# EryiXie/PlaneRecNet

Measured on AMD Instinct MI355X. Metric: img/s fwd+bwd @480×640 ResNet101-DCN, 1/2/4/8 MI355X + roofline %, higher is better.
Workload: dtype f32 (tensors and accumulation fp32; plain GEMMs and the tap-walked 4x4/s2, 1x1/s2 and sub-pixel convolutions >= 300 tiles: 2xfp16-piece split MFMA, fp32 accumulate; fp32-only rate in fp32_only_run)

## Files before the change

### include/prn.h

```cpp
#ifndef PRN_H
#define PRN_H
#include <stdint.h>
#ifdef __cplusplus
extern "C" {
#endif

#define PRN_BN_SPLITS 32

int prn_version(void);
const char* prn_last_error(void);

enum { PRN_IN_ZERO = 0, PRN_IN_REFLECT = 1, PRN_IN_UP2_REFLECT = 2, PRN_IN_DILATED = 3, PRN_IN_UP2_PHASE = 4,
       PRN_IN_EMBED1 = 5  };
enum { PRN_EPI_NONE = 0, PRN_EPI_RELU = 1, PRN_EPI_SIGMOID = 2 };

enum { PRN_SPLIT_OFF = 0, PRN_SPLIT_PLAN = 1, PRN_SPLIT_ALWAYS = 2 };
enum { PRN_PIECES_BF16 = 0, PRN_PIECES_F16 = 16 };
typedef struct prn_gemm_opts {
  int32_t split_mode;
  int32_t split_kind;
  int32_t split_products;
  int32_t split_min_tiles;
  float split_min_gflop;
  int32_t wgrad_wgs;
  int32_t wgrad_target;
  int32_t wgrad_split;
} prn_gemm_opts;
void prn_gemm_opts_default(prn_gemm_opts* o);

typedef struct prn_conv_desc {
  int32_t B, C, H, W;
  int32_t M;
  int32_t KH, KW;
  int32_t stride, pad;
  int32_t Ho, Wo;
  int32_t in_mode;
  int32_t dil;
  int32_t epilogue;
  int32_t ystride;
  int32_t yH, yW;
  int32_t reserved;
  prn_gemm_opts opts;
} prn_conv_desc;

int64_t prn_conv2d_fwd_ws_bytes(const prn_conv_desc* d);
int prn_conv2d_kernel_kind(const prn_conv_desc* d);
int prn_conv2d_fwd_partials(const prn_conv_desc* d, int64_t* offset_bytes);
int prn_gemm_pipe(int M, int K, int B, int HW, int nz, const prn_gemm_opts* opts);
int64_t prn_split_images_bytes(int M, int K, int nz);
int prn_split_prepare(const float* w, void* images, int M, int K, int nz, int kind, void* stream);
int prn_split_prepare_batched(const void* items_dev, int n_items, int64_t total_blocks, int64_t total_row_blocks, int kind, void* stream);
int prn_conv2d_fwd(const prn_conv_desc* d, const float* x, const float* w, const float* bias,
                   const float* addend, float* y, void* ws, void* stream);
#define PRN_TILE_COUNTERS 4096
int prn_conv2d_fwd_counted(const prn_conv_desc* d, const float* x, const float* w, const void* w_images, const float* bias, const float* addend, float* y,
                           void* ws, unsigned* counters, void* stream, int phase);
#define PRN_MAX_SEGMENTS 6
typedef struct prn_ragged {
  int32_t nseg;
  int32_t H[PRN_MAX_SEGMENTS], W[PRN_MAX_SEGMENTS];
} prn_ragged;
int prn_conv2d_fwd_ragged(const prn_conv_desc* d, const prn_ragged* rg, const float* x, const float* w, const float* bias,
                          const float* addend, float* y, void* stream);
int64_t prn_conv2d_wgrad_ragged_ws_bytes(const prn_conv_desc* d, const prn_ragged* rg);
int prn_conv2d_wgrad_ragged(const prn_conv_desc* d, const prn_ragged* rg, const float* x, const float* dy, float* dw, void* ws,
                            void* stream);

int prn_conv2d_fwd_phase(const prn_conv_desc* d, const float* x, const float* w, const float* bias,
                         const float* addend, float* y, void* ws, void* stream, int phase);

int prn_weight_flip_transpose(const float* w, float* wt, int M, int C, int KH, int KW, void* stream);

typedef struct prn_flip_item {
  const float* src;
  float* dst;
  int M, C, KH, KW;
  int64_t first;
} prn_flip_item;
int prn_weight_flip_transpose_batched(const prn_flip_item* items_dev, int n_items, int64_t total_blocks, void* stream);

int64_t prn_winograd_tiles(int B, int H, int W);
typedef struct prn_winograd_item {
  const float* src;
  float* u;
  float* ut;
  int M, C;
  int64_t first;
} prn_winograd_item;
int prn_winograd_weights_batched(const prn_winograd_item* items_dev, int n_items, int64_t total_blocks, void* stream);
int prn_winograd_input(const float* x, float* V, int B, int C, int H, int W, int in_mode, void* stream);
int64_t prn_gemm_batched_ws_bytes(int M, int C, int P, int nb, const prn_gemm_opts* opts);
int prn_gemm_batched(int M, int C, int P, int nb, const float* U, const void* u_images, const float* V, float* Y, void* ws, const prn_gemm_opts* opts,
                     void* stream);
int prn_winograd_output(const float* Y, const float* bias, const float* addend, float* y, int B, int M, int H, int W, int epilogue, void* stream);
int prn_winograd_output_bn_fwd(const float* Yt, float* x_out, float* stats, const float* gamma, const float* beta, float* y, float* running_mean,
                               float* running_var, int B, int M, int H, int W, float eps, float momentum, int relu, void* stream);
int prn_winograd_output_bn_bwd(const float* Yt, const float* x, const float* stats, const float* gamma, const float* beta, float* dx, float* dgamma,
                               float* dbeta, int B, int M, int H, int W, int relu, void* stream);
int64_t prn_winograd_wgrad_ws_bytes(int B, int C, int H, int W, int M, const prn_gemm_opts* opts);
int prn_winograd_dy(const float* dy, float* Y, int B, int M, int H, int W, void* stream);
int prn_gemm_batched_nt_splits(int M, int C, int P, int nb, const prn_gemm_opts* opts);
int prn_gemm_batched_nt_kind(int M, int C, int P, int nb, const prn_gemm_opts* opts);
int prn_gemm_batched_nt(int M, int C, int P, int nb, const float* A, const float* Bm, float* ws, const prn_gemm_opts* opts, void* stream);
int prn_winograd_dw(const float* partials, float* dw, int M, int C, int splits, void* stream);
int prn_conv3x3_winograd_wgrad(const float* x, const float* dy, float* dw, void* ws, int B, int C, int H, int W, int M, int in_mode, const prn_gemm_opts* opts,
                               void* stream, int phase);
int prn_conv3x3_winograd_wgrad_v(const float* V, const float* dy, float* dw, void* ws, int B, int C, int H, int W, int M, const prn_gemm_opts* opts, void* stream);
int64_t prn_winograd_tiles_ragged(const prn_ragged* rg, int B);
int64_t prn_conv3x3_winograd_ragged_ws_bytes(const prn_ragged* rg, int B, int C, int M, const prn_gemm_opts* opts);
int prn_conv3x3_winograd_ragged(const float* x, const float* U, const void* u_images, const float* bias, const float* addend, float* y, void* ws,
                                const prn_ragged* rg, int B, int C, int M, int epilogue, const prn_gemm_opts* opts, void* stream);
int64_t prn_winograd_wgrad_ragged_ws_bytes(const prn_ragged* rg, int B, int C, int M, const prn_gemm_opts* opts);
int prn_conv3x3_winograd_wgrad_ragged(const float* x, const float* dy, float* dw, void* ws, const prn_ragged* rg, int B, int C, int M, const prn_gemm_opts* opts,
                                      void* stream);
// ... 20 lines not shown

int prn_channel_sum(const float* x, float* out, double* ws, int B, int C, int HW, void* stream);

int prn_dcn_sample(const float* x, const float* om, float* cols, int B, int C, int H, int W, int Ho, int Wo,
                   int stride, float max_offset, void* stream);
int64_t prn_dcn_sample_bwd_ws_bytes(int B, int C, int H, int W, int Ho, int Wo);
int prn_dcn_sample_bwd(const float* x, const float* om, const float* dcols, float* dx, float* d_om, void* ws,
                       int B, int C, int H, int W, int Ho, int Wo, int stride, float max_offset, void* stream);

typedef struct prn_dcn_desc {
  int32_t B, C, H, W;
  int32_t M;
  int32_t stride, pad;
  int32_t Ho, Wo;
  int32_t raw;
  float max_offset;
  int32_t epilogue;
  prn_gemm_opts opts;
} prn_dcn_desc;
int64_t prn_dcnv2_table_bytes(const prn_dcn_desc* d);
int prn_dcnv2_table(const prn_dcn_desc* d, const float* offset, const float* mask, void* table, void* stream);
int64_t prn_dcnv2_fwd_ws_bytes(const prn_dcn_desc* d);
int prn_dcnv2_fwd(const prn_dcn_desc* d, const float* x, const void* table, const float* w, const float* bias, float* y, void* ws, void* stream);
int prn_dcnv2_fwd_phase(const prn_dcn_desc* d, const float* x, const void* table, const float* w, const float* bias, float* y, void* ws, void* stream,
                        int phase);
int64_t prn_dcnv2_bwd_weight_ws_bytes(const prn_dcn_desc* d);
int prn_dcnv2_bwd_weight(const prn_dcn_desc* d, const float* x, const void* table, const float* dy, float* dw, void* ws, void* stream);
int prn_dcnv2_bwd_weight_phase(const prn_dcn_desc* d, const float* x, const void* table, const float* dy, float* dw, void* ws, void* stream, int phase);
int64_t prn_dcnv2_bwd_ws_bytes(const prn_dcn_desc* d);
int prn_dcnv2_bwd_input(const prn_dcn_desc* d, const float* dy, const float* wt, const void* wt_images, const float* offset, const float* mask, float* dx,
                        void* ws, void* stream);
int prn_dcnv2_bwd_input_phase(const prn_dcn_desc* d, const float* dy, const float* wt, const void* wt_images, const float* offset, const float* mask,
                              float* dx, void* ws, void* stream, int phase);
int prn_dcnv2_bwd_offset_mask(const prn_dcn_desc* d, const float* x, const float* offset, const float* mask, float* d_offset, float* d_mask,
                              void* ws, void* stream);

int prn_bn_stats(const float* x, float* stats, float* running_mean, float* running_var, double* ws,
                 int B, int C, int HW, float eps, float momentum, void* stream);
int prn_bn_apply(const float* x, const float* stats, const float* gamma, const float* beta, const float* residual,
                 float* y, int B, int C, int HW, int relu, void* stream);
int prn_bn_kernel_kind(int B, int HW);
int prn_bn_train_fwd(const float* x, float* stats, const float* gamma, const float* beta, const float* residual, float* y,
                     float* running_mean, float* running_var, double* ws, int B, int C, int HW, float eps, float momentum,
                     int relu, void* stream);
int prn_bn_bwd(const float* dy, const float* x, const float* y, const float* stats, const float* gamma, const float* beta,
               float* dx, float* dres, float* dgamma, float* dbeta, double* ws,
               int B, int C, int HW, int relu, int frozen, void* stream);
int prn_bn_train_fwd_into(const float* x, float* stats, const float* gamma, const float* beta, const float* residual, float* y,
                          int64_t y_batch_stride, float* running_mean, float* running_var, double* ws, int B, int C, int HW, float eps,
                          float momentum, int relu, void* stream);
int prn_bn_bwd_from(const float* dy, int64_t dy_batch_stride, const float* x, const float* y, const float* stats, const float* gamma,
                    const float* beta, float* dx, float* dres, float* dgamma, float* dbeta, double* ws,
                    int B, int C, int HW, int relu, int frozen, void* stream);

int prn_bn_train_fwd_partials(const float* parts, int nparts, int64_t part_stride, float* x_out, float* stats, const float* gamma, const float* beta,
                              const float* residual, float* y, float* running_mean, float* running_var, int B, int C, int HW, float eps, float momentum,
                              int relu, void* stream);
int prn_bn_bwd_partials(const float* dparts, int nparts, int64_t part_stride, const float* x, const float* y, const float* stats, const float* gamma,
                        const float* beta, float* dx, float* dres, float* dgamma, float* dbeta, int B, int C, int HW, int relu, int frozen, void* stream);
int prn_bn_train_fwd_winograd(const float* parts, int nparts, int64_t part_stride, float* x_out, float* stats, const float* gamma, const float* beta,
                              const float* residual, float* y, float* running_mean, float* running_var, float* V, int B, int C, int H, int W, float eps,
                              float momentum, int relu, void* stream);
int prn_bn_bwd_winograd(const float* dparts, int nparts, int64_t part_stride, const float* x, const float* y, const float* stats, const float* gamma,
                        const float* beta, float* dx, float* dres, float* dgamma, float* dbeta, float* V, int B, int C, int H, int W, int relu, int frozen,
                        void* stream);

int prn_gn_relu_fwd(const float* x, const float* gamma, const float* beta, float* y, float* stats ,
                    int B, int C, int HW, int G, float eps, void* stream);
int prn_gn_relu_bwd(const float* dy, const float* x, const float* beta, const float* stats, const float* gamma,
                    float* dx, float* dgamma_part , float* dbeta_part ,
                    int B, int C, int HW, int G, void* stream);
int prn_gn_relu_fwd_ragged(const float* x, const float* gamma, const float* beta, float* y, float* stats,
                           int B, int C, int nseg, const int* hw, int G, float eps, void* stream);
int prn_gn_relu_bwd_ragged(const float* dy, const float* x, const float* beta, const float* stats, const float* gamma,
                           float* dx, float* dgamma_part, float* dbeta_part, int B, int C, int nseg, const int* hw, int G,
                           void* stream);

int prn_sum_rows(const float* in, float* out, int nb, int R, int N, void* stream);

int prn_debug_skip_launches(int mask);

int prn_resize_bilinear_fwd(const float* x, float* y, int BC, int H, int W, int Ho, int Wo, void* stream);
int prn_resize_bilinear_bwd(const float* dy, float* dx, int BC, int H, int W, int Ho, int Wo, void* stream);
int prn_resize_bilinear_add_fwd(const float* x, const float* addend, float* y, int BC, int H, int W, int Ho, int Wo, void* stream);
int prn_resize_bilinear_bwd_add(const float* dy, const float* addend, float* dx, int BC, int H, int W, int Ho, int Wo, void* stream);
int prn_maxpool3s2_fwd(const float* x, float* y, unsigned char* arg, int BC, int H, int W, int Ho, int Wo, void* stream);
int prn_maxpool3s2_bwd(const unsigned char* arg, const float* dy, float* dx, int BC, int H, int W, int Ho, int Wo, void* stream);

int64_t prn_plane_prior_ws_bytes(int B, int E, int h, int w, int NK, int F, const prn_gemm_opts* opts);
int prn_plane_prior_fwd(const float* seg, const float* kernels, const float* w1, const float* b1, float* pooled, float* out, void* ws, int B, int E,
                        int h, int w, int NK, int F, const prn_gemm_opts* opts, void* stream);
int prn_plane_prior_fwd_phase(const float* seg, const float* kernels, const float* w1, const float* b1, float* pooled, float* out, void* ws, int B, int E,
                        int h, int w, int NK, int F, const prn_gemm_opts* opts, void* stream, int phase);
int64_t prn_plane_prior_wgrad_ws_bytes(int B, int h, int w, int NK, int F, const prn_gemm_opts* opts);
int prn_plane_prior_wgrad(const float* pooled, const float* d_out, float* dw1, void* ws, int B, int h, int w, int NK, int F, const prn_gemm_opts* opts,
                          void* stream);
int64_t prn_fpn_level_ws_bytes(int B, int C, int H, int W, int F, int relu, int has_prev, int have_u, const prn_gemm_opts* opts);
int prn_fpn_level_fwd(const float* x, const float* w_lat, const float* b_lat, const float* prev, int Hp, int Wp, const float* w_out, const float* u_out,
                      const float* b_out, float* lateral, float* p_out, void* ws, int B, int C, int H, int W, int F, int relu, const prn_gemm_opts* opts,
                      void* stream);

enum { PRN_BLK_WINOGRAD = 1,
       PRN_BLK_HANDOVER = 2,
       PRN_BLK_KEEP_V = 4,
       PRN_BLK_SCATTER_ACC = 8 };
enum { PRN_BLK_CONV2_DIRECT = 0, PRN_BLK_CONV2_WINOGRAD = 1, PRN_BLK_CONV2_DCN = 2 };
typedef struct prn_bottleneck_desc {
  int32_t B, C, H, W;
  int32_t planes;
  int32_t stride;
  int32_t dcn;
  int32_t downsample;
  int32_t flags;
  float eps[4], momentum[4];
  float max_offset;
  int32_t reserved;
  prn_gemm_opts opts;
} prn_bottleneck_desc;
typedef struct prn_bottleneck_params {
  const float *w1, *w2, *w3, *wd;
  const float *b2;
  const void *w1_img, *w3_img, *wd_img;
  const float* u2; const void* u2_img;
  const float *w1_t, *w2_t, *w3_t, *wd_t;
  const void *w1_t_img, *w3_t_img, *wd_t_img;
  const float* ut2; const void* ut2_img;
  const float *w27, *b27, *w27_t;
  const float* w2_cols_t; const void* w2_cols_t_img;
  const float *gamma[4], *beta[4];
  float *running_mean[4], *running_var[4];
} prn_bottleneck_params;
enum { PRN_BLK_SAVE_BYTES = 0, PRN_BLK_GSAVE_BYTES, PRN_BLK_FWD_WS_BYTES, PRN_BLK_BWD_WS_BYTES, PRN_BLK_HO, PRN_BLK_WO, PRN_BLK_CONV2_PATH, PRN_BLK_KEEPS_V,
       PRN_BLK_OFF_A1, PRN_BLK_OFF_V, PRN_BLK_OFF_A2, PRN_BLK_OFF_OM, PRN_BLK_OFF_TABLE,
       PRN_BLK_OFF_D1, PRN_BLK_OFF_D2, PRN_BLK_OFF_D3, PRN_BLK_OFF_DD, PRN_BLK_OFF_DOM,
       PRN_BLK_BN_GRAD_FLOATS,
       PRN_BLK_HANDOVERS,
       PRN_BLK_NEEDS_W1_IMG, PRN_BLK_NEEDS_W3_IMG, PRN_BLK_NEEDS_WD_IMG, PRN_BLK_NEEDS_W1T_IMG, PRN_BLK_NEEDS_W3T_IMG, PRN_BLK_NEEDS_WDT_IMG, PRN_BLK_NEEDS_U_IMG,
       PRN_BLK_NEEDS_COLT_IMG, PRN_BLK_INFO_COUNT };
int64_t prn_bottleneck_plan_bytes(void);
int64_t prn_bottleneck_params_bytes(void);
int prn_bottleneck_plan(const prn_bottleneck_desc* d, void* plan);
int prn_bottleneck_plan_info(const void* plan, int64_t* out, int n);
int prn_bottleneck_train_fwd(const void* plan, const prn_bottleneck_params* p, const float* x, float* y, void* save, void* ws, void* stream);
int prn_bottleneck_train_bwd(const void* plan, const prn_bottleneck_params* p, const float* x, const float* y, const float* dy, float* dx, int dx_accumulate,
                             const void* save, void* gsave, float* bn_grads, void* ws, void* stream);

int prn_frame_to_input(const unsigned char* src, int Hs, int Ws, int Hr, int Wr, int Hp, int Wp, const float* mean_bgr, const float* std_bgr, int mode,
                       float* dst, float* frame_bgr, void* stream);

int prn_mask_loss_ws_floats(int P);
int prn_mask_loss_fwd(const float* logits, const unsigned char* labels, const float* adj, const int64_t* img, const float* gsum, const float* npos,
                      float* out2, float* coef, float* ws, int P, int HW, int B, float w_ins, float w_lav, void* stream);
int prn_mask_loss_bwd(const float* logits, const unsigned char* labels, const float* adj, const int64_t* img, const float* coef, const float* g_ins,
                      const float* g_lav, float* dlogits, int P, int HW, void* stream);

int prn_lava_gt_weights(const float* gt, float* out, int B, int H, int W, float depth_resolution, void* stream);

int prn_vnl_triplets(const float* pred, const float* gt, const int* gid, const int64_t* seg, const unsigned char* seg_is_plane, const double* seg_normal,
                     const int64_t* seg_img, const double* fx, const double* fy, double* loss, unsigned char* valid, float* g3, int n, int H, int W,
                     float delta_z, void* stream);
int prn_vnl_scatter(const double* g_loss, const float* g3, const int64_t* order, const int64_t* start, float* d_depth, int npts, int n, void* stream);

int prn_loss_ws_doubles(int B);
int prn_focal_sum_fwd(const float* x, const int64_t* labels, float* out, double* ws, int64_t rows, int C, float alpha, float gamma, void* stream);
int prn_focal_sum_bwd(const float* x, const int64_t* labels, const float* g_out, float* dx, int64_t rows, int C, float alpha, float gamma, void* stream);
int prn_rmse_log_fwd(const float* pred, const float* gt, float* out, float* coef, double* ws, int B, int HW, float min_depth, float clamp, void* stream);
int prn_rmse_log_bwd(const float* pred, const float* gt, const float* coef, const float* g_out, float* dpred, int B, int HW, float min_depth, float clamp,
                     void* stream);

int prn_vnl_trim_key(const double* loss, const unsigned char* valid, const int64_t* seg, double* key, int n, void* stream);
int prn_vnl_trim_fwd(const double* loss, const unsigned char* valid, const int64_t* order, const int64_t* seg_start, const unsigned char* seg_is_plane,
                     const int64_t* seg_img, const double* nplanes, int nseg, int n, int B, double* out, double* seg_sum, int* seg_m, double* seg_coef,
                     void* ws, void* stream);
int64_t prn_vnl_trim_ws_bytes(int nseg);
int prn_vnl_trim_bwd(const double* loss, const int64_t* order, const int64_t* seg_start, const int* seg_m, const double* seg_coef, const int64_t* seg_img,
                     const double* g_out, int nseg, int n, double* dloss, void* stream);

int prn_depth_metrics_ws_doubles(void);
int prn_depth_metrics(const float* pred, const float* gt, double* out, double* ws, int64_t n, float min_depth, float max_depth, void* stream);

int64_t prn_pairwise_iou_ws_bytes(int A, int B, int64_t HW);
int prn_pairwise_iou(const unsigned char* masks_a, const unsigned char* masks_b, const float* boxes_a, const float* boxes_b, int A, int B, int64_t HW,
                     float* mask_iou, float* box_iou, void* ws, void* stream);
int prn_mask_boxes(const unsigned char* masks, int n, int H, int W, float* boxes, void* stream);
int prn_mask_stats(const float* seg, int n, int64_t HW, float thr, float* count, float* msum, void* stream);
int prn_sigmoid_point_nms(const float* x, float* out, int B, int C, int S, int64_t out_batch_stride, void* stream);
int prn_matrix_nms(const float* iou, const int64_t* labels, const float* scores, int n, float sigma, int gaussian, float* out, float* ws, void* stream);
#define PRN_MASK_NMS_MAX 4096
int64_t prn_mask_nms_ws_bytes(int n_total, int n_max, int64_t HW);
int prn_mask_nms(const unsigned char* masks, const int64_t* labels, const float* sum_masks, const int* seg, int n_img, int n_max, int64_t HW, float thr,
                 unsigned char* keep, void* ws, void* stream);
// ... 71 lines not shown
```

### planerecnet_amd/_lib.py

```python
import ctypes
import os

_HERE = os.path.dirname(os.path.abspath(__file__))
LIB_PATH = os.environ.get("PRN_LIB") or os.path.join(_HERE, "libprn_hip.so")

c_int, c_float, c_void_p, c_i64 = ctypes.c_int, ctypes.c_float, ctypes.c_void_p, ctypes.c_int64


class GemmOpts(ctypes.Structure):
    _fields_ = [("split_mode", ctypes.c_int32), ("split_kind", ctypes.c_int32), ("split_products", ctypes.c_int32), ("split_min_tiles", ctypes.c_int32),
                ("split_min_gflop", ctypes.c_float), ("wgrad_wgs", ctypes.c_int32), ("wgrad_target", ctypes.c_int32), ("wgrad_split", ctypes.c_int32)]

    def key(self):
        return (self.split_mode, self.split_kind, self.split_products, self.split_min_tiles, self.split_min_gflop, self.wgrad_wgs, self.wgrad_target, self.wgrad_split)


SPLIT_OFF, SPLIT_PLAN, SPLIT_ALWAYS = 0, 1, 2
PIECES_BF16, PIECES_F16 = 0, 16


class ConvDesc(ctypes.Structure):
    _fields_ = [(n, ctypes.c_int32) for n in
                ("B", "C", "H", "W", "M", "KH", "KW", "stride", "pad", "Ho", "Wo", "in_mode", "dil", "epilogue", "ystride", "yH", "yW", "reserved")] + [
                    ("opts", GemmOpts)]


class Ragged(ctypes.Structure):
    _fields_ = [("nseg", ctypes.c_int32), ("H", ctypes.c_int32 * 6), ("W", ctypes.c_int32 * 6)]


class DcnDesc(ctypes.Structure):
    _fields_ = [(n, ctypes.c_int32) for n in ("B", "C", "H", "W", "M", "stride", "pad", "Ho", "Wo", "raw")] + [("max_offset", ctypes.c_float),
                                                                                                              ("epilogue", ctypes.c_int32),
                                                                                                              ("opts", GemmOpts)]


class BottleneckDesc(ctypes.Structure):
    _fields_ = [(n, ctypes.c_int32) for n in ("B", "C", "H", "W", "planes", "stride", "dcn", "downsample", "flags")] + [
        ("eps", ctypes.c_float * 4), ("momentum", ctypes.c_float * 4), ("max_offset", ctypes.c_float), ("reserved", ctypes.c_int32), ("opts", GemmOpts)]


class BottleneckParams(ctypes.Structure):
    _fields_ = [(n, ctypes.c_void_p) for n in (
        "w1", "w2", "w3", "wd", "b2", "w1_img", "w3_img", "wd_img", "u2", "u2_img", "w1_t", "w2_t", "w3_t", "wd_t", "w1_t_img", "w3_t_img", "wd_t_img", "ut2", "ut2_img",
        "w27", "b27", "w27_t", "w2_cols_t", "w2_cols_t_img")] + [(n, ctypes.c_void_p * 4) for n in ("gamma", "beta", "running_mean", "running_var")]


IN_ZERO, IN_REFLECT, IN_UP2_REFLECT, IN_DILATED, IN_UP2_PHASE, IN_EMBED1 = 0, 1, 2, 3, 4, 5
EPI_NONE, EPI_RELU, EPI_SIGMOID = 0, 1, 2
BN_SPLITS = 32

P = c_void_p
_DP = ctypes.POINTER(ConvDesc)
_OP = ctypes.POINTER(GemmOpts)
SIGNATURES = {
    "prn_version": (c_int, []),
    "prn_last_error": (ctypes.c_char_p, []),
    "prn_conv2d_fwd_ws_bytes": (c_i64, [_DP]),
    "prn_conv2d_kernel_kind": (c_int, [_DP]),
    "prn_conv2d_fwd_partials": (c_int, [_DP, ctypes.POINTER(c_i64)]),
    "prn_gemm_opts_default": (None, [_OP]),
    "prn_gemm_pipe": (c_int, [c_int, c_int, c_int, c_int, c_int, _OP]),
    "prn_split_images_bytes": (c_i64, [c_int, c_int, c_int]),
    "prn_split_prepare": (c_int, [P, P, c_int, c_int, c_int, c_int, P]),
    "prn_split_prepare_batched": (c_int, [P, c_int, c_i64, c_i64, c_int, P]),
    "prn_conv2d_fwd": (c_int, [_DP, P, P, P, P, P, P, P]),
    "prn_conv2d_fwd_ragged": (c_int, [_DP, P, P, P, P, P, P, P]),
    "prn_conv2d_wgrad_ragged_ws_bytes": (c_i64, [_DP, P]),
    "prn_conv2d_wgrad_ragged": (c_int, [_DP, P, P, P, P, P, P]),
    "prn_gn_relu_fwd_ragged": (c_int, [P, P, P, P, P, c_int, c_int, c_int, P, c_int, c_float, P]),
    "prn_gn_relu_bwd_ragged": (c_int, [P, P, P, P, P, P, P, P, c_int, c_int, c_int, P, c_int, P]),
    "prn_conv2d_fwd_phase": (c_int, [_DP, P, P, P, P, P, P, P, c_int]),
    "prn_conv2d_fwd_counted": (c_int, [_DP, P, P, P, P, P, P, P, P, P, c_int]),
    "prn_conv2d_wgrad_phase": (c_int, [_DP, P, P, P, P, P, c_int]),
    "prn_weight_flip_transpose": (c_int, [P, P, c_int, c_int, c_int, c_int, P]),
    "prn_weight_flip_transpose_batched": (c_int, [P, c_int, c_i64, P]),
    "prn_winograd_tiles": (c_i64, [c_int, c_int, c_int]),
    "prn_winograd_weights_batched": (c_int, [P, c_int, c_i64, P]),
    "prn_winograd_input": (c_int, [P, P, c_int, c_int, c_int, c_int, c_int, P]),
    "prn_gemm_batched_ws_bytes": (c_i64, [c_int, c_int, c_int, c_int, _OP]),
    "prn_gemm_batched": (c_int, [c_int, c_int, c_int, c_int, P, P, P, P, P, _OP, P]),
    "prn_winograd_output": (c_int, [P, P, P, P, c_int, c_int, c_int, c_int, c_int, P]),
    "prn_winograd_output_bn_fwd": (c_int, [P] * 8 + [c_int] * 4 + [c_float, c_float, c_int, P]),
    "prn_winograd_output_bn_bwd": (c_int, [P] * 8 + [c_int] * 5 + [P]),
    "prn_winograd_wgrad_ws_bytes": (c_i64, [c_int] * 5 + [_OP]),
    "prn_winograd_dy": (c_int, [P, P, c_int, c_int, c_int, c_int, P]),
    "prn_gemm_batched_nt_splits": (c_int, [c_int] * 4 + [_OP]),
    "prn_gemm_batched_nt_kind": (c_int, [c_int] * 4 + [_OP]),
    "prn_conv2d_wgrad_kernel_kind": (c_int, [_DP, c_int]),
    "prn_gemm_batched_nt": (c_int, [c_int, c_int, c_int, c_int, P, P, P, _OP, P]),
    "prn_winograd_dw": (c_int, [P, P, c_int, c_int, c_int, P]),
    "prn_conv3x3_winograd_wgrad": (c_int, [P, P, P, P, c_int, c_int, c_int, c_int, c_int, c_int, _OP, P, c_int]),
    "prn_winograd_tiles_ragged": (c_i64, [P, c_int]),
    "prn_conv3x3_winograd_ragged_ws_bytes": (c_i64, [P, c_int, c_int, c_int, _OP]),
    "prn_conv3x3_winograd_ragged": (c_int, [P, P, P, P, P, P, P, P, c_int, c_int, c_int, c_int, _OP, P]),
    "prn_winograd_wgrad_ragged_ws_bytes": (c_i64, [P, c_int, c_int, c_int, _OP]),
    "prn_conv3x3_winograd_wgrad_ragged": (c_int, [P, P, P, P, P, c_int, c_int, c_int, _OP, P]),
    "prn_conv3x3_winograd_wgrad_v": (c_int, [P, P, P, P, c_int, c_int, c_int, c_int, c_int, _OP, P]),
    "prn_conv3x3_winograd_ws_bytes": (c_i64, [c_int] * 5 + [_OP]),
    "prn_conv3x3_winograd": (c_int, [P, P, P, P, P, P, P, c_int, c_int, c_int, c_int, c_int, c_int, c_int, _OP, P]),
    "prn_conv2d_wgrad_ws_bytes": (c_i64, [_DP]),
    "prn_conv2d_wgrad_grouped_ws_bytes": (c_i64, [_DP, c_int]),
    "prn_conv2d_wgrad_grouped": (c_int, [_DP, c_int, P, P, P, P, P]),
    "prn_conv2d_wgrad": (c_int, [_DP, P, P, P, P, P]),
    "prn_pad_fold": (c_int, [P, P, c_int, c_int, c_int, c_int, c_int, P]),
    "prn_pad_fold_pitched": (c_int, [P, P, c_int, c_int, c_int, c_int, c_int, P]),
    "prn_up2_phase_weights": (c_int, [P, P, c_int, c_int, P]),
    "prn_up2_dgrad_weights": (c_int, [P, P, c_int, c_int, P]),
    "prn_up2_wgrad_combine": (c_int, [P, P, c_int, c_int, P]),
    "prn_space_to_depth2": (c_int, [P, P, c_int, c_int, c_int, c_int, P]),
    "prn_replicate_fold": (c_int, [P, P, c_int, c_int, c_int, c_int, P]),
    "prn_channel_sum": (c_int, [P, P, P, c_int, c_int, c_int, P]),
    "prn_dcn_sample": (c_int, [P, P, P] + [c_int] * 7 + [c_float, P]),
    "prn_dcn_sample_bwd_ws_bytes": (c_i64, [c_int] * 6),
    "prn_dcn_sample_bwd": (c_int, [P, P, P, P, P, P] + [c_int] * 7 + [c_float, P]),
    "prn_dcnv2_table_bytes": (c_i64, [P]),
    "prn_dcnv2_table": (c_int, [P, P, P, P, P]),
    "prn_dcnv2_fwd_ws_bytes": (c_i64, [P]),
    "prn_dcnv2_fwd": (c_int, [P] * 8),
    "prn_dcnv2_fwd_phase": (c_int, [P] * 8 + [c_int]),
    "prn_dcnv2_bwd_weight_ws_bytes": (c_i64, [P]),
    "prn_dcnv2_bwd_weight": (c_int, [P] * 7),
    "prn_dcnv2_bwd_weight_phase": (c_int, [P] * 7 + [c_int]),
    "prn_dcnv2_bwd_ws_bytes": (c_i64, [P]),
    "prn_dcnv2_bwd_input": (c_int, [P] * 9),
    "prn_dcnv2_bwd_input_phase": (c_int, [P] * 9 + [c_int]),
    "prn_bn_kernel_kind": (c_int, [c_int, c_int]),
    "prn_dcnv2_bwd_offset_mask": (c_int, [P] * 8),
    "prn_plane_prior_ws_bytes": (c_i64, [c_int] * 6 + [_OP]),
    "prn_plane_prior_fwd": (c_int, [P] * 7 + [c_int] * 6 + [_OP, P]),
    "prn_plane_prior_fwd_phase": (c_int, [P] * 7 + [c_int] * 6 + [_OP, P, c_int]),
    "prn_plane_prior_wgrad_ws_bytes": (c_i64, [c_int] * 5 + [_OP]),
    "prn_plane_prior_wgrad": (c_int, [P] * 4 + [c_int] * 5 + [_OP, P]),
    "prn_fpn_level_ws_bytes": (c_i64, [c_int] * 8 + [_OP]),
    "prn_fpn_level_fwd": (c_int, [P, P, P, P, c_int, c_int, P, P, P, P, P, P] + [c_int] * 6 + [_OP, P]),
    "prn_frame_to_input": (c_int, [P] + [c_int] * 6 + [P, P, c_int, P, P, P]),
    "prn_mask_loss_ws_floats": (c_int, [c_int]),
    "prn_mask_loss_fwd": (c_int, [P] * 9 + [c_int, c_int, c_int, c_float, c_float, P]),
    "prn_mask_loss_bwd": (c_int, [P] * 8 + [c_int, c_int, P]),
    "prn_vnl_triplets": (c_int, [P] * 12 + [c_int, c_int, c_int, c_float, P]),
    "prn_vnl_scatter": (c_int, [P] * 5 + [c_int, c_int, P]),
    "prn_depth_metrics_ws_doubles": (c_int, []),
    "prn_depth_metrics": (c_int, [P, P, P, P, c_i64, c_float, c_float, P]),
    "prn_vnl_trim_key": (c_int, [P, P, P, P, c_int, P]),
    "prn_vnl_trim_fwd": (c_int, [P, P, P, P, P, P, P, c_int, c_int, c_int, P, P, P, P, P, P]),
    "prn_vnl_trim_ws_bytes": (c_i64, [c_int]),
    "prn_vnl_trim_bwd": (c_int, [P, P, P, P, P, P, P, c_int, c_int, P, P]),
    "prn_loss_ws_doubles": (c_int, [c_int]),
    "prn_focal_sum_fwd": (c_int, [P, P, P, P, c_i64, c_int, c_float, c_float, P]),
    "prn_focal_sum_bwd": (c_int, [P, P, P, P, c_i64, c_int, c_float, c_float, P]),
    "prn_rmse_log_fwd": (c_int, [P, P, P, P, P, c_int, c_int, c_float, c_float, P]),
    "prn_rmse_log_bwd": (c_int, [P, P, P, P, P, c_int, c_int, c_float, c_float, P]),
    "prn_gt_segments": (c_i64, [c_int, c_int]),
    "prn_gt_mask_stats": (c_int, [P, P, c_int, c_int, c_int, c_int, P, P, P, P]),
    "prn_gt_quarter_masks": (c_int, [P, P, c_int, c_int, c_int, P]),
    "prn_gt_sample_triplets": (c_int, [P, P, c_int, c_int, c_int, c_int, P, P, P, P, P, ctypes.c_uint64, ctypes.c_uint64, c_i64, P, P]),
    "prn_adam_chunk_elems": (c_int, []),
    "prn_adam_step": (c_int, [P, c_int, c_int, P, P, P, P, P, P, P, P, P, ctypes.c_double, ctypes.c_double, c_float, P]),
    "prn_adam_step_masked": (c_int, [P, c_int, c_int, P, P, P, P, P, P, P, P, P, ctypes.c_double, ctypes.c_double, c_float, P, P, P]),
    "prn_pairwise_iou_ws_bytes": (c_i64, [c_int, c_int, c_i64]),
    "prn_pairwise_iou": (c_int, [P, P, P, P, c_int, c_int, c_i64, P, P, P, P]),
    "prn_mask_boxes": (c_int, [P, c_int, c_int, c_int, P, P]),
    "prn_mask_stats": (c_int, [P, c_int, c_i64, c_float, P, P, P]),
    "prn_sigmoid_point_nms": (c_int, [P, P, c_int, c_int, c_int, c_i64, P]),
    "prn_matrix_nms": (c_int, [P, P, P, c_int, c_float, c_int, P, P, P]),
    "prn_mask_nms_ws_bytes": (c_i64, [c_int, c_int, c_i64]),
    "prn_mask_nms": (c_int, [P, P, P, P, c_int, c_int, c_i64, c_float, P, P, P]),
    "prn_bn_stats": (c_int, [P, P, P, P, P, c_int, c_int, c_int, c_float, c_float, P]),
    "prn_bn_apply": (c_int, [P, P, P, P, P, P, c_int, c_int, c_int, c_int, P]),
    "prn_bn_train_fwd": (c_int, [P] * 9 + [c_int, c_int, c_int, c_float, c_float, c_int, P]),
    "prn_bn_bwd": (c_int, [P] * 11 + [c_int] * 5 + [P]),
    "prn_bn_train_fwd_into": (c_int, [P] * 6 + [c_i64] + [P] * 3 + [c_int, c_int, c_int, c_float, c_float, c_int, P]),
    "prn_bn_bwd_from": (c_int, [P, c_i64] + [P] * 10 + [c_int] * 5 + [P]),
    "prn_bn_train_fwd_partials": (c_int, [P, c_int, c_i64] + [P] * 8 + [c_int, c_int, c_int, c_float, c_float, c_int, P]),
    "prn_bn_bwd_partials": (c_int, [P, c_int, c_i64] + [P] * 9 + [c_int] * 5 + [P]),
    "prn_bn_train_fwd_winograd": (c_int, [P, c_int, c_i64] + [P] * 9 + [c_int] * 4 + [c_float, c_float, c_int, P]),
    "prn_bn_bwd_winograd": (c_int, [P, c_int, c_i64] + [P] * 10 + [c_int] * 6 + [P]),
    "prn_gn_relu_fwd": (c_int, [P, P, P, P, P, c_int, c_int, c_int, c_int, c_float, P]),
    "prn_gn_relu_bwd": (c_int, [P] * 8 + [c_int] * 4 + [P]),
    "prn_resize_bilinear_fwd": (c_int, [P, P] + [c_int] * 5 + [P]),
    "prn_resize_bilinear_bwd": (c_int, [P, P] + [c_int] * 5 + [P]),
    "prn_resize_bilinear_add_fwd": (c_int, [P, P, P] + [c_int] * 5 + [P]),
    "prn_resize_bilinear_bwd_add": (c_int, [P, P, P] + [c_int] * 5 + [P]),
    "prn_maxpool3s2_fwd": (c_int, [P, P, P] + [c_int] * 5 + [P]),
    "prn_maxpool3s2_bwd": (c_int, [P, P, P] + [c_int] * 5 + [P]),
    "prn_sum_rows": (c_int, [P, P, c_int, c_int, c_int, P]),
    "prn_lava_gt_weights": (c_int, [P, P, c_int, c_int, c_int, c_float, P]),
    "prn_debug_skip_launches": (c_int, [c_int]),
    "prn_bottleneck_plan_bytes": (c_i64, []),
    "prn_bottleneck_params_bytes": (c_i64, []),
    "prn_bottleneck_plan": (c_int, [ctypes.POINTER(BottleneckDesc), P]),
    "prn_bottleneck_plan_info": (c_int, [P, ctypes.POINTER(c_i64), c_int]),
    "prn_bottleneck_train_fwd": (c_int, [P, ctypes.POINTER(BottleneckParams), P, P, P, P, P]),
    "prn_bottleneck_train_bwd": (c_int, [P, ctypes.POINTER(BottleneckParams), P, P, P, P, c_int, P, P, P, P, P]),
    "prn_planes_ws_bytes": (c_i64, [c_int] * 4),
    "prn_planes_fit": (c_int, [P] * 4 + [c_int] * 4 + [P] * 6),
    "prn_planes_render": (c_int, [P] * 6 + [c_int] * 5 + [c_float, c_float, P, P, P]),
    "prn_planes_ransac_ws_bytes": (c_i64, [c_int] * 5),
    "prn_planes_ransac_fit": (c_int, [P] * 4 + [c_int] * 4 + [ctypes.c_double, c_int, c_int, c_int, ctypes.c_uint64] + [P] * 9),
    "prn_render_overlay": (c_int, [P] * 4 + [c_int] * 3 + [c_float, c_float, c_int, P, P]),
    "prn_render_limits_ws_bytes": (c_i64, []),
    "prn_render_depth_limits": (c_int, [P, c_i64, ctypes.c_double, ctypes.c_double, P, P, P]),
    "prn_render_depth_colors": (c_int, [P, c_i64, P, P, P, P]),
    "prn_render_depth_gray": (c_int, [P, c_i64, c_float, P, P]),
    "prn_rle_ws_bytes": (c_i64, [c_int] * 3),
    "prn_rle_count": (c_int, [P, P] + [c_int] * 4 + [P, P, P]),
    "prn_rle_fill": (c_int, [P, P] + [c_int] * 4 + [P, P, P, P]),
    "prn_rle_string_lengths": (c_int, [P, P] + [c_int] * 3 + [P, P]),
    "prn_rle_strings": (c_int, [P, P, P] + [c_int] * 3 + [P, P]),
    "prn_rle_paint": (c_int, [P, P] + [c_int] * 3 + [P, P]),
    "prn_ccl_ws_bytes": (c_i64, [c_int] * 3),
    "prn_ccl_label": (c_int, [P, P] + [c_int] * 5 + [P, P, P, P]),
    "prn_ccl_clean": (c_int, [P, P] + [c_int] * 8 + [P] * 7),
    "prn_morph_ws_bytes": (c_i64, [c_int] * 4),
    "prn_morph": (c_int, [P, P] + [c_int] * 7 + [P] * 4),
    "prn_boundary_iou_ws_bytes": (c_i64, [c_int] * 4),
    "prn_boundary_iou": (c_int, [P, P] + [c_int] * 5 + [P] * 4),
}


def load():
    if not os.path.exists(LIB_PATH):
        raise ImportError(f"{LIB_PATH} is missing: run `python -c 'import __graft_entry__ as g; g.build()'` "
                          "(hipcc --offload-arch=gfx950). There is no fallback path.")
# ... 17 lines not shown
```

### planerecnet_amd/blocks.py

```python
import ctypes
import os
import sys

import torch

from . import _lib, ops, profiling
from ._lib import lib, check

ENABLED = os.environ.get("PRN_BLOCKS", "1") == "1"
HANDOVER = os.environ.get("PRN_BLOCK_HANDOVER", "1") == "1"
SCATTER_ACCUMULATE = os.environ.get("PRN_SCATTER_ACC", "1") == "1"
STATS = {"fwd": 0, "bwd": 0, "resolved": 0, "vouched": 0, "scatter_acc": 0}

BLK_WINOGRAD, BLK_HANDOVER, BLK_KEEP_V, BLK_SCATTER_ACC = 1, 2, 4, 8
CONV2_DIRECT, CONV2_WINOGRAD, CONV2_DCN = 0, 1, 2
(I_SAVE, I_GSAVE, I_FWD_WS, I_BWD_WS, I_HO, I_WO, I_CONV2, I_KEEPS_V, I_A1, I_V, I_A2, I_OM, I_TABLE, I_D1, I_D2, I_D3, I_DD, I_DOM, I_BN_FLOATS, I_HANDOVERS,
 I_W1_IMG, I_W3_IMG, I_WD_IMG, I_W1T_IMG, I_W3T_IMG, I_WDT_IMG, I_U_IMG, I_COLT_IMG, INFO_COUNT) = range(29)

_SCRATCH = {}
_F32 = torch.float32
_empty = torch.empty


def scratch(nbytes, dev):
    key = (dev.index, ops._raw_stream(dev.index))
    t = _SCRATCH.get(key)
    if t is None or t.numel() * 4 < nbytes:
        t = _SCRATCH[key] = torch.empty((int(nbytes * 1.25) + 1023) // 4, device=dev, dtype=torch.float32)
    return t


class _Ref:
    __slots__ = ("ptr", "shape", "device")

    def __init__(self, ptr, shape, device):
        self.ptr, self.shape, self.device = ptr, shape, device

    def data_ptr(self):
        return self.ptr

    def numel(self):
        n = 1
        for s in self.shape:
            n *= s
        return n


class _State:
    __slots__ = ("plan", "plan_ref", "info", "params", "params_ref", "convw", "wver", "epoch", "batched", "keep", "hb", "bn_sizes", "out_shape", "Ho", "Wo", "conv2",
                 "dims", "wino_wgrad", "g_keys", "max_offset", "ps", "bns", "stat_bufs", "save_n", "gsave_n", "bn_n", "fwd_ws", "bwd_ws", "stride", "dcn", "ds",
                 "shapes")


def _flags():
    f = BLK_SCATTER_ACC if SCATTER_ACCUMULATE else 0
    if ops.WINOGRAD:
        f |= BLK_WINOGRAD
    if ops.WINOGRAD and ops.WINOGRAD_WGRAD:
        f |= BLK_KEEP_V
    if HANDOVER:
        f |= BLK_HANDOVER
    return f


def supported(blk):
    from .dcn import DeformableConv2d
    c2 = blk.conv2
    if blk.downsample is not None:
        dc = blk.downsample[0]
        if dc.kernel_size != (1, 1) or dc.stride[0] != blk.stride or dc.bias is not None:
            return False
    elif blk.stride != 1 or blk.conv1.weight.shape[1] != blk.conv3.weight.shape[0]:
        return False
    if isinstance(c2, DeformableConv2d):
        if c2.stride != blk.stride:
            return False
    elif c2.bias is not None or c2.kernel_size != (3, 3) or c2.padding != (1, 1) or c2.stride[0] != blk.stride:
        return False
    bns = [blk.bn1, blk.bn2, blk.bn3] + ([blk.downsample[1]] if blk.downsample is not None else [])
    return (blk.stride in (1, 2) and ops.WINOGRAD_MIN_TILES == 128 and blk.conv1.bias is None and blk.conv3.bias is None and blk.conv1.kernel_size == (1, 1)
            and blk.conv3.kernel_size == (1, 1) and all(isinstance(m, torch.nn.BatchNorm2d) and m.affine and m.track_running_stats and m.momentum is not None for m in bns))


def _param_list(blk):
    from .dcn import DeformableConv2d
    c2 = blk.conv2
    ps = [blk.conv1.weight, blk.bn1.weight, blk.bn1.bias]
    if isinstance(c2, DeformableConv2d):
        ps += [c2.offset_conv.weight, c2.modulator_conv.weight, c2.offset_conv.bias, c2.modulator_conv.bias, c2.regular_conv.weight, c2.regular_conv.bias]
    else:
        ps += [c2.weight]
    ps += [blk.bn2.weight, blk.bn2.bias, blk.conv3.weight, blk.bn3.weight, blk.bn3.bias]
    if blk.downsample is not None:
        ps += [blk.downsample[0].weight, blk.downsample[1].weight, blk.downsample[1].bias]
    return tuple(ps)


def _state(blk, x, key):
    from .dcn import DeformableConv2d
    oe = ops._opts_entry()
    B, C, H, W = x.shape
    dcn = isinstance(blk.conv2, DeformableConv2d)
    bns = (blk.bn1, blk.bn2, blk.bn3) + ((blk.downsample[1],) if blk.downsample is not None else ())
    eps = [float(m.eps) for m in bns] + [0.0] * (4 - len(bns))
    mom = [float(m.momentum) for m in bns] + [0.0] * (4 - len(bns))
    P = blk.conv1.weight.shape[0]
    d = _lib.BottleneckDesc(B, C, H, W, P, blk.stride, int(dcn), int(blk.downsample is not None), key[2], (ctypes.c_float * 4)(*eps), (ctypes.c_float * 4)(*mom),
                            max(H, W) / 4.0 if dcn else 0.0, 0, oe[0])
    st = _State()
    st.plan = ctypes.create_string_buffer(int(lib.prn_bottleneck_plan_bytes()) + 64)
    st.plan_ref = (ctypes.addressof(st.plan) + 63) & ~63
    check(lib.prn_bottleneck_plan(ctypes.byref(d), st.plan_ref), "prn_bottleneck_plan")
    info = (ctypes.c_int64 * INFO_COUNT)()
    check(lib.prn_bottleneck_plan_info(st.plan_ref, info, INFO_COUNT), "prn_bottleneck_plan_info")
# ... 276 lines not shown
```

### planerecnet_amd/csrc/prn_bottleneck.hip

```cpp
#include "prn_common.h"
#include <string.h>

namespace {

constexpr int32_t PLAN_MAGIC = 0x424c4b36;
constexpr int64_t WINOGRAD_MIN_TILES = 128;

inline int64_t up256(int64_t v) { return (v + 255) & ~255LL; }

struct Plan {
  int32_t magic, pad_;
  prn_bottleneck_desc d;
  int32_t Ho, Wo, P4, conv2_path;
  int32_t small1, small2;
  int32_t lazy1, parts1;
  int32_t v1, lazy2, keep_v;
  int32_t lazy3g, parts3g;
  int32_t v2g, lazy2g;
  int32_t pad2_;
  int64_t parts1_off, parts3g_off;
  prn_conv_desc c1, c2, c3, cd, c27, g1, g2, g3, gd, g27;
  prn_dcn_desc dcn;
  int64_t s_c1, s_a1, s_v, s_c2, s_a2, s_c3, s_cd, s_om, s_table, s_stats[4], save_bytes;
  int64_t q_d3, q_dd, q_d2, q_d1, q_dom, q_bn, gsave_bytes;
  int64_t f_c1, f_bn, f_v, f_yt, f_gemm, f_c2, f_c27, f_dcn, f_c3, f_cd, f_res, fwd_ws_bytes;
  int64_t b_bn, b_dres, b_g3, b_g3ws, b_v, b_yt, b_gemm, b_g2, b_g2ws, b_dcn, b_dx1, b_g27ws, b_g1ws, b_gdtmp, b_gdws, bwd_ws_bytes;
};

prn_conv_desc conv_desc(int B, int C, int H, int W, int M, int K, int stride, int pad, int Ho, int Wo, int mode, int dil, int ystride, int yH, int yW,
                        const prn_gemm_opts& o) {
  prn_conv_desc d;
  d.B = B; d.C = C; d.H = H; d.W = W; d.M = M; d.KH = d.KW = K; d.stride = stride; d.pad = pad; d.Ho = Ho; d.Wo = Wo;
  d.in_mode = mode; d.dil = dil; d.epilogue = PRN_EPI_NONE; d.ystride = ystride; d.yH = yH; d.yW = yW; d.reserved = 0;
  d.opts = o;
  return d;
}

bool winograd_ok(const prn_bottleneck_desc& d, int B, int C, int H, int W, int M) {
  return (d.flags & PRN_BLK_WINOGRAD) && (W % 4) == 0 && H >= 8 && C >= 64 && M >= 64 && (int64_t)B * ((H + 3) / 4) * (W / 4) >= WINOGRAD_MIN_TILES;
}

int make_plan(const prn_bottleneck_desc* dp, Plan& L) {
  PRN_REQUIRE(dp != nullptr, "prn_bottleneck_plan: null descriptor");
  const prn_bottleneck_desc& d = *dp;
  PRN_REQUIRE(d.B > 0 && d.C > 0 && d.H > 0 && d.W > 0 && d.planes > 0, "prn_bottleneck_plan: empty dimension");
  PRN_REQUIRE(d.stride == 1 || d.stride == 2, "prn_bottleneck_plan: stride %d (1 or 2)", d.stride);
  PRN_REQUIRE(d.downsample || (d.stride == 1 && d.C == 4 * d.planes), "prn_bottleneck_plan: without a downsample branch the block must keep its shape (C = 4 * planes, stride 1)");
  PRN_REQUIRE(!d.dcn || d.max_offset > 0.f, "prn_bottleneck_plan: the deformable variant needs max_offset (max(h, w) / 4)");
  memset(&L, 0, sizeof(L));
  L.magic = PLAN_MAGIC;
  L.d = d;
  const int B = d.B, C = d.C, H = d.H, W = d.W, P = d.planes, s = d.stride, Q = 4 * d.planes;
  const int Ho = (H + 2 - 3) / s + 1, Wo = (W + 2 - 3) / s + 1;
  L.Ho = Ho; L.Wo = Wo;
  const prn_gemm_opts& o = d.opts;
  const bool ho = (d.flags & PRN_BLK_HANDOVER) != 0;
  L.small1 = prn_bn_kernel_kind(B, H * W);
  L.small2 = prn_bn_kernel_kind(B, Ho * Wo);
  L.c1 = conv_desc(B, C, H, W, P, 1, 1, 0, H, W, PRN_IN_ZERO, 1, 0, 0, 0, o);
  L.c3 = conv_desc(B, P, Ho, Wo, Q, 1, 1, 0, Ho, Wo, PRN_IN_ZERO, 1, 0, 0, 0, o);
  if (d.downsample) L.cd = conv_desc(B, C, H, W, Q, 1, s, 0, Ho, Wo, PRN_IN_ZERO, 1, 0, 0, 0, o);
  const bool wino = !d.dcn && s == 1 && winograd_ok(d, B, P, H, W, P);
  L.conv2_path = d.dcn ? PRN_BLK_CONV2_DCN : (wino ? PRN_BLK_CONV2_WINOGRAD : PRN_BLK_CONV2_DIRECT);
  if (d.dcn) {
    L.c27 = conv_desc(B, P, H, W, 27, 3, s, 1, Ho, Wo, PRN_IN_ZERO, 1, 0, 0, 0, o);
    prn_dcn_desc& q = L.dcn;
    q.B = B; q.C = P; q.H = H; q.W = W; q.M = P; q.stride = s; q.pad = 1; q.Ho = Ho; q.Wo = Wo; q.raw = 1; q.max_offset = d.max_offset; q.epilogue = PRN_EPI_NONE;
    q.opts = o;
  } else if (!wino) {
    L.c2 = conv_desc(B, P, H, W, P, 3, s, 1, Ho, Wo, PRN_IN_ZERO, 1, 0, 0, 0, o);
  }
  if (wino) L.P4 = (int)prn_winograd_tiles(B, H, W);
  L.g3 = conv_desc(B, Q, Ho, Wo, P, 1, 1, 0, Ho, Wo, PRN_IN_ZERO, 1, 0, 0, 0, o);
  L.g1 = conv_desc(B, P, H, W, C, 1, 1, 0, H, W, PRN_IN_ZERO, 1, 0, 0, 0, o);
  if (!d.dcn && !wino)
    L.g2 = s == 1 ? conv_desc(B, P, Ho, Wo, P, 3, 1, 1, H, W, PRN_IN_ZERO, 1, 0, 0, 0, o) : conv_desc(B, P, Ho, Wo, P, 3, 1, 1, H, W, PRN_IN_DILATED, 2, 0, 0, 0, o);
  if (d.dcn)
    L.g27 = s == 1 ? conv_desc(B, 27, Ho, Wo, P, 3, 1, 1, H, W, PRN_IN_ZERO, 1, 0, 0, 0, o) : conv_desc(B, 27, Ho, Wo, P, 3, 1, 1, H, W, PRN_IN_DILATED, 2, 0, 0, 0, o);
  if (d.downsample)
    L.gd = s == 1 ? conv_desc(B, Q, Ho, Wo, C, 1, 1, 0, H, W, PRN_IN_ZERO, 1, 0, 0, 0, o) : conv_desc(B, Q, Ho, Wo, C, 1, 1, 0, Ho, Wo, PRN_IN_ZERO, 1, 2, H, W, o);
  int64_t off = 0;
  const int p1 = prn_conv2d_fwd_partials(&L.c1, &off);
  if (p1 < 0) return 2;
  L.lazy1 = ho && L.small1 && p1 > 1 && (((int64_t)B * P * H * W) & 3) == 0;
  L.parts1 = L.lazy1 ? p1 : 0; L.parts1_off = L.lazy1 ? off : 0;
  L.v1 = ho && wino && L.small1;
  L.lazy2 = ho && wino && L.small2 && L.P4 <= 768;
  L.keep_v = wino && (d.flags & PRN_BLK_KEEP_V) && 4LL * 36 * P * L.P4 <= (128LL << 20);
  const int p3 = prn_conv2d_fwd_partials(&L.g3, &off);
  if (p3 < 0) return 2;
  L.lazy3g = ho && L.small2 && p3 > 1 && (((int64_t)B * P * Ho * Wo) & 3) == 0;
  L.parts3g = L.lazy3g ? p3 : 0; L.parts3g_off = L.lazy3g ? off : 0;
  L.v2g = ho && wino && L.small2;
  L.lazy2g = ho && wino && L.small1 && L.P4 <= 768;
  const int64_t n1 = (int64_t)B * P * H * W * 4, n2 = (int64_t)B * P * Ho * Wo * 4, n3 = (int64_t)B * Q * Ho * Wo * 4, nx = (int64_t)B * C * H * W * 4;
  const int64_t nv = wino ? 4LL * 36 * P * L.P4 : 0, nom = (int64_t)B * 27 * Ho * Wo * 4;
  const int Cmax = Q > C ? Q : C;
  const int64_t bnws = 2LL * Cmax * PRN_BN_SPLITS * 8;
#define PRN_WS(expr_, name_) const int64_t name_ = (expr_); if (name_ < 0) return 2
  PRN_WS(prn_conv2d_fwd_ws_bytes(&L.c1), w_c1);
  PRN_WS(prn_conv2d_fwd_ws_bytes(&L.c3), w_c3);
  PRN_WS(d.downsample ? prn_conv2d_fwd_ws_bytes(&L.cd) : 0, w_cd);
  PRN_WS(L.conv2_path == PRN_BLK_CONV2_DIRECT ? prn_conv2d_fwd_ws_bytes(&L.c2) : 0, w_c2);
  PRN_WS(d.dcn ? prn_conv2d_fwd_ws_bytes(&L.c27) : 0, w_c27);
  PRN_WS(d.dcn ? prn_dcnv2_fwd_ws_bytes(&L.dcn) : 0, w_dcnf);
  PRN_WS(d.dcn ? prn_dcnv2_table_bytes(&L.dcn) : 0, n_table);
  PRN_WS(d.dcn ? prn_dcnv2_bwd_ws_bytes(&L.dcn) : 0, w_dcnb);
  PRN_WS(wino ? prn_gemm_batched_ws_bytes(P, P, L.P4, 36, &o) : 0, w_gemm);
  PRN_WS(prn_conv2d_fwd_ws_bytes(&L.g3), w_g3);
  PRN_WS(prn_conv2d_fwd_ws_bytes(&L.g1), w_g1);
  PRN_WS(L.conv2_path == PRN_BLK_CONV2_DIRECT ? prn_conv2d_fwd_ws_bytes(&L.g2) : 0, w_g2);
  PRN_WS(d.dcn ? prn_conv2d_fwd_ws_bytes(&L.g27) : 0, w_g27);
  PRN_WS(d.downsample ? prn_conv2d_fwd_ws_bytes(&L.gd) : 0, w_gd);
#undef PRN_WS
  int64_t at = 0;
  auto put = [&at](int64_t& slot, int64_t bytes) { slot = at; at += up256(bytes); };
  put(L.s_c1, n1); put(L.s_a1, n1);
  put(L.s_v, L.keep_v ? nv : 0);
  put(L.s_c2, n2); put(L.s_a2, n2); put(L.s_c3, n3);
  put(L.s_cd, d.downsample ? n3 : 0);
  put(L.s_om, d.dcn ? nom : 0); put(L.s_table, n_table);
  put(L.s_stats[0], 8LL * P); put(L.s_stats[1], 8LL * P); put(L.s_stats[2], 8LL * Q); put(L.s_stats[3], d.downsample ? 8LL * Q : 0);
  L.save_bytes = at;
  at = 0;
  put(L.q_d3, n3); put(L.q_dd, d.downsample ? n3 : 0); put(L.q_d2, n2); put(L.q_d1, n1); put(L.q_dom, d.dcn ? nom : 0);
  L.q_bn = 2 * P + 2 * P + 2 * Q + (d.downsample ? 2 * Q : 0);
  L.gsave_bytes = at;
  at = 0;
  put(L.f_c1, w_c1); put(L.f_bn, bnws);
  put(L.f_v, (wino && !L.keep_v) ? nv : 0); put(L.f_yt, nv); put(L.f_gemm, w_gemm);
  put(L.f_c2, w_c2); put(L.f_c27, w_c27); put(L.f_dcn, w_dcnf); put(L.f_c3, w_c3); put(L.f_cd, w_cd);
  put(L.f_res, d.downsample ? n3 : 0);
  L.fwd_ws_bytes = at;
  at = 0;
  put(L.b_bn, bnws); put(L.b_dres, n3);
  put(L.b_g3, n2); put(L.b_g3ws, w_g3);
  put(L.b_v, nv); put(L.b_yt, nv); put(L.b_gemm, w_gemm);
  put(L.b_g2, n1); put(L.b_g2ws, w_g2);
  put(L.b_dcn, w_dcnb); put(L.b_dx1, d.dcn ? n1 : 0); put(L.b_g27ws, w_g27);
  put(L.b_g1ws, w_g1);
  put(L.b_gdtmp, d.downsample ? nx : 0); put(L.b_gdws, w_gd);
  L.bwd_ws_bytes = at;
  return 0;
}

const Plan* plan_of(const void* plan, const char* who) {
  const Plan* L = (const Plan*)plan;
  if (L == nullptr || L->magic != PLAN_MAGIC) { prn_set_error("%s: not a plan filled by prn_bottleneck_plan", who); return nullptr; }
  return L;
}

inline float* f32(void* base, int64_t off) { return (float*)((char*)base + off); }
inline void* raw(void* base, int64_t off, int64_t used = 1) { return used ? (void*)((char*)base + off) : nullptr; }

#define PRN_TRY(call_) do { if (int e_ = (call_)) return e_; } while (0)

}

extern "C" int64_t prn_bottleneck_plan_bytes(void) { return (int64_t)sizeof(Plan); }
extern "C" int64_t prn_bottleneck_params_bytes(void) { return (int64_t)sizeof(prn_bottleneck_params); }

extern "C" int prn_bottleneck_plan(const prn_bottleneck_desc* d, void* plan) {
  PRN_REQUIRE(plan != nullptr, "prn_bottleneck_plan: null plan buffer (prn_bottleneck_plan_bytes() bytes, caller-owned)");
  Plan L;
  if (int e = make_plan(d, L)) { memset(plan, 0, sizeof(int32_t)); return e; }
  memcpy(plan, &L, sizeof(L));
  return 0;
}

extern "C" int prn_bottleneck_plan_info(const void* plan, int64_t* out, int n) {
  const Plan* L = plan_of(plan, "prn_bottleneck_plan_info");
  if (!L) return 2;
  PRN_REQUIRE(out != nullptr && n >= PRN_BLK_INFO_COUNT, "prn_bottleneck_plan_info: out must hold PRN_BLK_INFO_COUNT (%d) values", PRN_BLK_INFO_COUNT);
  out[PRN_BLK_SAVE_BYTES] = L->save_bytes; out[PRN_BLK_GSAVE_BYTES] = L->gsave_bytes;
  out[PRN_BLK_FWD_WS_BYTES] = L->fwd_ws_bytes; out[PRN_BLK_BWD_WS_BYTES] = L->bwd_ws_bytes;
  out[PRN_BLK_HO] = L->Ho; out[PRN_BLK_WO] = L->Wo; out[PRN_BLK_CONV2_PATH] = L->conv2_path; out[PRN_BLK_KEEPS_V] = L->keep_v;
  out[PRN_BLK_OFF_A1] = L->s_a1; out[PRN_BLK_OFF_V] = L->s_v; out[PRN_BLK_OFF_A2] = L->s_a2; out[PRN_BLK_OFF_OM] = L->s_om; out[PRN_BLK_OFF_TABLE] = L->s_table;
  out[PRN_BLK_OFF_D1] = L->q_d1; out[PRN_BLK_OFF_D2] = L->q_d2; out[PRN_BLK_OFF_D3] = L->q_d3; out[PRN_BLK_OFF_DD] = L->q_dd; out[PRN_BLK_OFF_DOM] = L->q_dom;
  out[PRN_BLK_BN_GRAD_FLOATS] = L->q_bn;
  out[PRN_BLK_HANDOVERS] = L->lazy1 | (L->v1 << 1) | (L->lazy2 << 2) | (L->lazy3g << 3) | (L->v2g << 4) | (L->lazy2g << 5);
  out[PRN_BLK_NEEDS_W1_IMG] = prn_conv2d_kernel_kind(&L->c1) >= 2; out[PRN_BLK_NEEDS_W3_IMG] = prn_conv2d_kernel_kind(&L->c3) >= 2;
  out[PRN_BLK_NEEDS_WD_IMG] = (L->d.downsample && L->d.stride == 1 && prn_conv2d_kernel_kind(&L->cd) >= 2) ? 1 : 0;
  out[PRN_BLK_NEEDS_W1T_IMG] = prn_conv2d_kernel_kind(&L->g1) >= 2; out[PRN_BLK_NEEDS_W3T_IMG] = prn_conv2d_kernel_kind(&L->g3) >= 2;
  out[PRN_BLK_NEEDS_WDT_IMG] = (L->d.downsample && L->d.stride == 1 && prn_conv2d_kernel_kind(&L->gd) >= 2) ? 1 : 0;
  out[PRN_BLK_NEEDS_U_IMG] = (L->conv2_path == PRN_BLK_CONV2_WINOGRAD && prn_gemm_pipe(L->d.planes, L->d.planes, 1, L->P4, 36, &L->d.opts) >= 1) ? 1 : 0;
  out[PRN_BLK_NEEDS_COLT_IMG] = (L->d.dcn && prn_gemm_pipe(9 * L->d.planes, L->d.planes, L->d.B, L->Ho * L->Wo, 1, &L->d.opts) >= 1) ? 1 : 0;
  return 0;
}

extern "C" int prn_bottleneck_train_fwd(const void* plan, const prn_bottleneck_params* p, const float* x, float* y, void* save, void* ws, void* stream) {
  const Plan* Lp = plan_of(plan, "prn_bottleneck_train_fwd");
  if (!Lp) return 2;
  const Plan& L = *Lp;
  const prn_bottleneck_desc& d = L.d;
  PRN_REQUIRE(p && x && y && save && (ws || L.fwd_ws_bytes == 0), "prn_bottleneck_train_fwd: null tensor / buffer");
  PRN_REQUIRE(p->w1 && p->w3 && (p->w2 || L.conv2_path == PRN_BLK_CONV2_WINOGRAD) && (p->u2 || L.conv2_path != PRN_BLK_CONV2_WINOGRAD) && (!d.downsample || p->wd),
              "prn_bottleneck_train_fwd: a weight operand the plan reads is null");
  PRN_REQUIRE(!d.dcn || (p->w27 && p->b27), "prn_bottleneck_train_fwd: the deformable variant needs the merged offset | modulator weights");
  for (int i = 0; i < (d.downsample ? 4 : 3); ++i)
    PRN_REQUIRE(p->gamma[i] && p->beta[i] && p->running_mean[i] && p->running_var[i], "prn_bottleneck_train_fwd: null BatchNorm parameter (layer %d)", i);
  PRN_REQUIRE(((reinterpret_cast<uintptr_t>(save) | reinterpret_cast<uintptr_t>(ws)) & 255) == 0, "prn_bottleneck_train_fwd: save / ws must be 256-byte aligned");
  const int B = d.B, H = d.H, W = d.W, P = d.planes, Q = 4 * P, Ho = L.Ho, Wo = L.Wo;
  float* c1 = f32(save, L.s_c1); float* a1 = f32(save, L.s_a1); float* c2 = f32(save, L.s_c2); float* a2 = f32(save, L.s_a2); float* c3 = f32(save, L.s_c3);
  float* st1 = f32(save, L.s_stats[0]); float* st2 = f32(save, L.s_stats[1]); float* st3 = f32(save, L.s_stats[2]); float* std_ = f32(save, L.s_stats[3]);
  double* bnws = (double*)raw(ws, L.f_bn);
  const int64_t n1 = (int64_t)B * P * H * W;
  const prn_gemm_opts* o = &d.opts;
  PRN_TRY(prn_conv2d_fwd_counted(&L.c1, x, p->w1, p->w1_img, nullptr, nullptr, c1, raw(ws, L.f_c1, L.f_bn - L.f_c1), nullptr, stream, L.lazy1 ? 1 : 0));
  float* V = L.conv2_path == PRN_BLK_CONV2_WINOGRAD ? (L.keep_v ? f32(save, L.s_v) : f32(ws, L.f_v)) : nullptr;
  const float* in1 = L.lazy1 ? f32(ws, L.f_c1 + L.parts1_off) : c1;
  if (L.v1)
    PRN_TRY(prn_bn_train_fwd_winograd(in1, L.lazy1 ? L.parts1 : 1, L.lazy1 ? n1 : 0, L.lazy1 ? c1 : nullptr, st1, p->gamma[0], p->beta[0], nullptr, a1, p->running_mean[0],
                                      p->running_var[0], V, B, P, H, W, d.eps[0], d.momentum[0], 1, stream));
  else if (L.lazy1)
    PRN_TRY(prn_bn_train_fwd_partials(in1, L.parts1, n1, c1, st1, p->gamma[0], p->beta[0], nullptr, a1, p->running_mean[0], p->running_var[0], B, P, H * W, d.eps[0],
                                      d.momentum[0], 1, stream));
  else
    PRN_TRY(prn_bn_train_fwd(c1, st1, p->gamma[0], p->beta[0], nullptr, a1, p->running_mean[0], p->running_var[0], L.small1 ? nullptr : bnws, B, P, H * W, d.eps[0],
                             d.momentum[0], 1, stream));
  float* Yt = f32(ws, L.f_yt);
  if (L.conv2_path == PRN_BLK_CONV2_WINOGRAD) {
    if (!L.v1) PRN_TRY(prn_winograd_input(a1, V, B, P, H, W, PRN_IN_ZERO, stream));
    PRN_TRY(prn_gemm_batched(P, P, L.P4, 36, p->u2, p->u2_img, V, Yt, raw(ws, L.f_gemm, L.f_c2 - L.f_gemm), o, stream));
    if (!L.lazy2) PRN_TRY(prn_winograd_output(Yt, nullptr, nullptr, c2, B, P, H, W, PRN_EPI_NONE, stream));
  } else if (L.conv2_path == PRN_BLK_CONV2_DCN) {
    float* om = f32(save, L.s_om);
    void* table = raw(save, L.s_table);
    PRN_TRY(prn_conv2d_fwd_counted(&L.c27, a1, p->w27, nullptr, p->b27, nullptr, om, raw(ws, L.f_c27, L.f_dcn - L.f_c27), nullptr, stream, 0));
    PRN_TRY(prn_dcnv2_table(&L.dcn, om, nullptr, table, stream));
    PRN_TRY(prn_dcnv2_fwd(&L.dcn, a1, table, p->w2, p->b2, c2, raw(ws, L.f_dcn, L.f_c3 - L.f_dcn), stream));
  } else {
    PRN_TRY(prn_conv2d_fwd_counted(&L.c2, a1, p->w2, nullptr, nullptr, nullptr, c2, raw(ws, L.f_c2, L.f_c27 - L.f_c2), nullptr, stream, 0));
  }
  if (L.conv2_path == PRN_BLK_CONV2_WINOGRAD && L.lazy2)
    PRN_TRY(prn_winograd_output_bn_fwd(Yt, c2, st2, p->gamma[1], p->beta[1], a2, p->running_mean[1], p->running_var[1], B, P, Ho, Wo, d.eps[1], d.momentum[1], 1, stream));
  else
    PRN_TRY(prn_bn_train_fwd(c2, st2, p->gamma[1], p->beta[1], nullptr, a2, p->running_mean[1], p->running_var[1], L.small2 ? nullptr : bnws, B, P, Ho * Wo, d.eps[1],
                             d.momentum[1], 1, stream));
  PRN_TRY(prn_conv2d_fwd_counted(&L.c3, a2, p->w3, p->w3_img, nullptr, nullptr, c3, raw(ws, L.f_c3, L.f_cd - L.f_c3), nullptr, stream, 0));
  const float* res = x;
  if (d.downsample) {
    float* cd = f32(save, L.s_cd);
    float* rd = f32(ws, L.f_res);
    PRN_TRY(prn_conv2d_fwd_counted(&L.cd, x, p->wd, d.stride == 1 ? p->wd_img : nullptr, nullptr, nullptr, cd, raw(ws, L.f_cd, L.f_res - L.f_cd), nullptr, stream, 0));
    PRN_TRY(prn_bn_train_fwd(cd, std_, p->gamma[3], p->beta[3], nullptr, rd, p->running_mean[3], p->running_var[3], L.small2 ? nullptr : bnws, B, Q, Ho * Wo, d.eps[3],
                             d.momentum[3], 0, stream));
    res = rd;
  }
  return prn_bn_train_fwd(c3, st3, p->gamma[2], p->beta[2], res, y, p->running_mean[2], p->running_var[2], L.small2 ? nullptr : bnws, B, Q, Ho * Wo, d.eps[2], d.momentum[2],
                          1, stream);
}

extern "C" int prn_bottleneck_train_bwd(const void* plan, const prn_bottleneck_params* p, const float* x, const float* y, const float* dy, float* dx,
                                        int dx_accumulate, const void* save_, void* gsave, float* bn_grads, void* ws, void* stream) {
  const Plan* Lp = plan_of(plan, "prn_bottleneck_train_bwd");
  if (!Lp) return 2;
  const Plan& L = *Lp;
  const prn_bottleneck_desc& d = L.d;
  PRN_REQUIRE(p && x && y && dy && dx && save_ && gsave && bn_grads && ws, "prn_bottleneck_train_bwd: null tensor / buffer");
  PRN_REQUIRE(p->w1_t && p->w3_t && (!d.downsample || p->wd_t), "prn_bottleneck_train_bwd: an input-gradient weight layout the plan reads is null");
  PRN_REQUIRE(L.conv2_path != PRN_BLK_CONV2_WINOGRAD || p->ut2, "prn_bottleneck_train_bwd: conv2's Winograd-domain input-gradient operand is null");
  PRN_REQUIRE(L.conv2_path != PRN_BLK_CONV2_DIRECT || p->w2_t, "prn_bottleneck_train_bwd: conv2's input-gradient layout is null");
  PRN_REQUIRE(!d.dcn || (p->w27_t && p->w2_cols_t), "prn_bottleneck_train_bwd: the deformable variant needs the input-gradient layouts of both convolutions");
  PRN_REQUIRE(!dx_accumulate || (d.downsample && d.stride == 2 && (d.flags & PRN_BLK_SCATTER_ACC)),
              "prn_bottleneck_train_bwd: dx_accumulate only for stride-2 downsample blocks planned with PRN_BLK_SCATTER_ACC");
  PRN_REQUIRE(((reinterpret_cast<uintptr_t>(save_) | reinterpret_cast<uintptr_t>(gsave) | reinterpret_cast<uintptr_t>(ws)) & 255) == 0,
              "prn_bottleneck_train_bwd: save / gsave / ws must be 256-byte aligned");
  void* save = const_cast<void*>(save_);
  const int B = d.B, C = d.C, H = d.H, W = d.W, P = d.planes, Q = 4 * P, Ho = L.Ho, Wo = L.Wo;
  const float* c1 = f32(save, L.s_c1); const float* a1 = f32(save, L.s_a1); const float* c2 = f32(save, L.s_c2); const float* c3 = f32(save, L.s_c3);
  const float* st1 = f32(save, L.s_stats[0]); const float* st2 = f32(save, L.s_stats[1]); const float* st3 = f32(save, L.s_stats[2]); const float* std_ = f32(save, L.s_stats[3]);
  float* d3 = f32(gsave, L.q_d3); float* d2 = f32(gsave, L.q_d2); float* d1 = f32(gsave, L.q_d1);
  float* dg1 = bn_grads; float* db1 = dg1 + P; float* dg2 = db1 + P; float* db2 = dg2 + P; float* dg3 = db2 + P; float* db3 = dg3 + Q; float* dgd = db3 + Q; float* dbd = dgd + Q;
  double* bnws = (double*)raw(ws, L.b_bn);
  float* dres = f32(ws, L.b_dres);
  const prn_gemm_opts* o = &d.opts;
  hipStream_t st = (hipStream_t)stream;
  PRN_TRY(prn_bn_bwd(dy, c3, y, st3, p->gamma[2], p->beta[2], d3, dres, dg3, db3, L.small2 ? nullptr : bnws, B, Q, Ho * Wo, 1, 0, stream));
  const float* addx = dres;
  if (d.downsample) {
    float* dd = f32(gsave, L.q_dd);
    PRN_TRY(prn_bn_bwd(dres, f32(save, L.s_cd), nullptr, std_, p->gamma[3], p->beta[3], dd, nullptr, dgd, dbd, L.small2 ? nullptr : bnws, B, Q, Ho * Wo, 0, 0, stream));
    void* gws = raw(ws, L.b_gdws, L.bwd_ws_bytes - L.b_gdws);
    if (d.stride == 1) {
      float* tmp = f32(ws, L.b_gdtmp);
      PRN_TRY(prn_conv2d_fwd_counted(&L.gd, dd, p->wd_t, p->wd_t_img, nullptr, nullptr, tmp, gws, nullptr, stream, 0));
      addx = tmp;
    } else if (dx_accumulate) {
      PRN_TRY(prn_conv2d_fwd_counted(&L.gd, dd, p->wd_t, nullptr, nullptr, dx, dx, gws, nullptr, stream, 0));
      addx = dx;
    } else {
      float* tmp = f32(ws, L.b_gdtmp);
      const hipError_t e = hipMemsetAsync(tmp, 0, (size_t)B * C * H * W * 4, st);
      PRN_REQUIRE(e == hipSuccess, "prn_bottleneck_train_bwd: clearing the strided input gradient failed: %s", hipGetErrorString(e));
      PRN_TRY(prn_conv2d_fwd_counted(&L.gd, dd, p->wd_t, nullptr, nullptr, nullptr, tmp, gws, nullptr, stream, 0));
      addx = tmp;
    }
  }
  float* g3 = f32(ws, L.b_g3);
  PRN_TRY(prn_conv2d_fwd_counted(&L.g3, d3, p->w3_t, p->w3_t_img, nullptr, nullptr, g3, raw(ws, L.b_g3ws, L.b_v - L.b_g3ws), nullptr, stream, L.lazy3g ? 1 : 0));
  const float* in2 = L.lazy3g ? f32(ws, L.b_g3ws + L.parts3g_off) : g3;
  const int64_t n2 = (int64_t)B * P * Ho * Wo;
  float* Vg = f32(ws, L.b_v);
  if (L.v2g)
    PRN_TRY(prn_bn_bwd_winograd(in2, L.lazy3g ? L.parts3g : 1, L.lazy3g ? n2 : 0, c2, nullptr, st2, p->gamma[1], p->beta[1], d2, nullptr, dg2, db2, Vg, B, P, Ho, Wo, 1, 0, stream));
  else if (L.lazy3g)
    PRN_TRY(prn_bn_bwd_partials(in2, L.parts3g, n2, c2, nullptr, st2, p->gamma[1], p->beta[1], d2, nullptr, dg2, db2, B, P, Ho * Wo, 1, 0, stream));
  else
    PRN_TRY(prn_bn_bwd(g3, c2, nullptr, st2, p->gamma[1], p->beta[1], d2, nullptr, dg2, db2, L.small2 ? nullptr : bnws, B, P, Ho * Wo, 1, 0, stream));
  float* g2 = f32(ws, L.b_g2);
  float* Ytg = f32(ws, L.b_yt);
  if (L.conv2_path == PRN_BLK_CONV2_WINOGRAD) {
    if (!L.v2g) PRN_TRY(prn_winograd_input(d2, Vg, B, P, H, W, PRN_IN_ZERO, stream));
    PRN_TRY(prn_gemm_batched(P, P, L.P4, 36, p->ut2, p->ut2_img, Vg, Ytg, raw(ws, L.b_gemm, L.b_g2 - L.b_gemm), o, stream));
    if (!L.lazy2g) PRN_TRY(prn_winograd_output(Ytg, nullptr, nullptr, g2, B, P, H, W, PRN_EPI_NONE, stream));
  } else if (L.conv2_path == PRN_BLK_CONV2_DCN) {
    const float* om = f32(save, L.s_om);
    float* dom = f32(gsave, L.q_dom);
    float* dx1 = f32(ws, L.b_dx1);
    void* cws = raw(ws, L.b_dcn);
    PRN_TRY(prn_dcnv2_bwd_input(&L.dcn, d2, p->w2_cols_t, p->w2_cols_t_img, om, nullptr, dx1, cws, stream));
    PRN_TRY(prn_dcnv2_bwd_offset_mask(&L.dcn, a1, om, nullptr, dom, nullptr, cws, stream));
    PRN_TRY(prn_conv2d_fwd_counted(&L.g27, dom, p->w27_t, nullptr, nullptr, dx1, g2, raw(ws, L.b_g27ws, L.b_g1ws - L.b_g27ws), nullptr, stream, 0));
  } else {
    PRN_TRY(prn_conv2d_fwd_counted(&L.g2, d2, p->w2_t, nullptr, nullptr, nullptr, g2, raw(ws, L.b_g2ws, L.b_dcn - L.b_g2ws), nullptr, stream, 0));
  }
  if (L.conv2_path == PRN_BLK_CONV2_WINOGRAD && L.lazy2g)
    PRN_TRY(prn_winograd_output_bn_bwd(Ytg, c1, st1, p->gamma[0], p->beta[0], d1, dg1, db1, B, P, H, W, 1, stream));
  else
    PRN_TRY(prn_bn_bwd(g2, c1, nullptr, st1, p->gamma[0], p->beta[0], d1, nullptr, dg1, db1, L.small1 ? nullptr : bnws, B, P, H * W, 1, 0, stream));
  return prn_conv2d_fwd_counted(&L.g1, d1, p->w1_t, p->w1_t_img, nullptr, addx, dx, raw(ws, L.b_g1ws, L.b_gdtmp - L.b_g1ws), nullptr, stream, 0);
}
```

### planerecnet_amd/csrc/prn_common.h

```cpp
#pragma once
#include <hip/hip_runtime.h>
#include <stdint.h>
#include <stdio.h>
#include "../../include/prn.h"

#define PRN_WAVE 64

void prn_set_error(const char* fmt, ...);

#include <stdlib.h>
static inline int prn_env_int(const char* name, int dflt) {
  const char* e = getenv(name);
  return e ? atoi(e) : dflt;
}
struct prn_env4 { int v[4]; };
static inline prn_env4 prn_env_ints(const char* name) {
  prn_env4 r = {{0, 0, 0, 0}};
  if (const char* e = getenv(name)) sscanf(e, "%d,%d,%d,%d", &r.v[0], &r.v[1], &r.v[2], &r.v[3]);
  return r;
}

extern int prn_skip_mask;
#define PRN_SKIPPED(bit) (__builtin_expect(prn_skip_mask & (bit), 0))
#define PRN_REPS(bit) (__builtin_expect(prn_skip_mask & ((bit) | ((bit) << 8)), 0) ? ((prn_skip_mask & (bit)) ? 0 : 2) : 1)
// ... 37 lines not shown
  const int64_t T_ = (int64_t)gridDim.x * 256, i0_ = (int64_t)blockIdx.x * 256 + threadIdx.x; \
  float v_[PRN_EPT]; \
  _Pragma("unroll") for (int k_ = 0; k_ < PRN_EPT; ++k_) { \
    const int64_t i = (i0_ + k_ * T_ < (total_)) ? i0_ + k_ * T_ : (total_) - 1;
#define PRN_EPT_END(total_, out_) \
  } \
  _Pragma("unroll") for (int k_ = 0; k_ < PRN_EPT; ++k_) if (i0_ + k_ * T_ < (total_)) (out_)[i0_ + k_ * T_] = v_[k_];


__device__ __forceinline__ float wave_sum(float v) {
#pragma unroll
  for (int o = 32; o > 0; o >>= 1) v += __shfl_xor(v, o, 64);
  return v;
}
__device__ __forceinline__ double wave_sum_d(double v) {
#pragma unroll
  for (int o = 32; o > 0; o >>= 1) v += __shfl_xor(v, o, 64);
  return v;
}
__device__ __forceinline__ int wave_sum_i(int v) {
#pragma unroll
  for (int o = 32; o > 0; o >>= 1) v += __shfl_xor(v, o, 64);
  return v;
}

__device__ __forceinline__ void block_sum2(double& a, double& b, double* sm) {
  a = wave_sum_d(a);
  b = wave_sum_d(b);
  const int w = threadIdx.x >> 6, nw = blockDim.x >> 6;
  __syncthreads();
  if ((threadIdx.x & 63) == 0) { sm[w] = a; sm[nw + w] = b; }
  __syncthreads();
  double ra = 0.0, rb = 0.0;
  for (int i = 0; i < nw; ++i) { ra += sm[i]; rb += sm[nw + i]; }
  a = ra; b = rb;
}

__device__ __forceinline__ void bt6(const float* v, float* o) {
  o[0] = 4.f * v[0] - 5.f * v[2] + v[4];
  o[1] = -4.f * (v[1] + v[2]) + v[3] + v[4];
  o[2] = 4.f * (v[1] - v[2]) - v[3] + v[4];
  o[3] = -2.f * v[1] - v[2] + 2.f * v[3] + v[4];
  o[4] = 2.f * v[1] - v[2] - 2.f * v[3] + v[4];
  o[5] = 4.f * v[1] - 5.f * v[3] + v[5];
}
__device__ __forceinline__ void at6(const float* m, float* o) {
  const float s12 = m[1] + m[2], d12 = m[1] - m[2], s34 = m[3] + m[4], d34 = m[3] - m[4];
  o[0] = m[0] + s12 + s34;
  o[1] = d12 + 2.f * d34;
  o[2] = s12 + 4.f * s34;
  o[3] = d12 + 8.f * d34 + m[5];
}

static inline int cdiv(int64_t a, int64_t b) { return (int)((a + b - 1) / b); }
__host__ __device__ inline size_t prn_align256(size_t v) { return (v + 255) & ~(size_t)255; }

int prn_launch_reduce_epilogue(const float* ws, const float* bias, const float* addend, float* y, int64_t total, int M, int HoWo, int splits,
                               int epi, hipStream_t st);
int prn_launch_reduce_splits(const float* ws, float* out, int64_t n, int splits, hipStream_t st);
int prn_quantise_splits(int64_t tiles, int splits);
int prn_gemm_batched_epi(int M, int C, int P, int nb, const float* U, const void* u_images, const float* V, float* Y, void* ws, const prn_gemm_opts* opts, int epi,
                         void* stream);

int prn_split_gemm_plan(int M, int K, int B, int HW, int nz, const prn_gemm_opts* opts);
int64_t prn_split_gemm_image_bytes(int M, int K, int nz);
int64_t prn_split_gemm_partial_bytes(int M, int B, int HW, int nz, int splits);
int prn_split_gemm(const float* w, const void* w_images, const float* x, const float* bias, const float* addend, float* y, void* images_ws, float* partial, int M,
                   int K, int B, int HW, int nz, int64_t zw, int64_t zx, int64_t zy, int epi, int splits, const prn_gemm_opts* opts, hipStream_t st, int phase);
int prn_split_conv_taps(const float* w, const float* x, const float* bias, const float* addend, float* y, void* images_ws, float* partial, int M, int C, int B, int XH,
                        int XW, int Ho, int Wo, int KH, int KW, int stride, int pad, int epi, int splits, const prn_gemm_opts* o, hipStream_t st, int phase);
int prn_split_conv_up2(const float* wp, const float* x, const float* bias, float* y, void* images_ws, int M, int C, int B, int H, int W, int epi, const prn_gemm_opts* o,
                       hipStream_t st);
static inline prn_gemm_opts prn_opts_or_zero(const prn_gemm_opts* o) {
  prn_gemm_opts z;
  if (o) return *o;
  z.split_mode = 0; z.split_kind = 0; z.split_products = 0; z.split_min_tiles = 0; z.split_min_gflop = 0.f; z.wgrad_wgs = 0; z.wgrad_target = 0; z.wgrad_split = 0;
  return z;
}

int prn_wgrad16_plan(int M, int C, int64_t N, int HW, int nz, const prn_gemm_opts* opts);
int prn_wgrad16_launch(const float* dy, const float* x, const float* const* gdy, const float* const* gx, int ngroup, float* out, int M, int C, int B, int HW, int nz,
                       int64_t zdy, int64_t zx, int splits, const prn_gemm_opts* opts, hipStream_t st);
```

### planerecnet_amd/csrc/prn_conv.hip

```cpp
#include <stddef.h>
#include <stdlib.h>
#include <type_traits>
#include "prn_common.h"

typedef float f32x16 __attribute__((ext_vector_type(16)));

namespace {

constexpr int MAX_SEG = 6;
struct Seg {
  int nseg;
  int n0[MAX_SEG + 1];
  int H[MAX_SEG], W[MAX_SEG];
  int x0[MAX_SEG], y0[MAX_SEG];
};
__device__ __forceinline__ int seg_find(const Seg& g, int n) {
  int s = 0;
#pragma unroll
  for (int t = 1; t < MAX_SEG; ++t)
    if (t < g.nseg && n >= g.n0[t]) s = t;
  return s;
}
template <class Args>
__device__ __forceinline__ int seg_read(size_t member_offset, int s) {
// ... 1427 lines not shown
    xo += (int64_t)d->B * d->C * H * W;
    yo += (int64_t)d->B * d->M * H * W;
  }
  PRN_REQUIRE(n % align == 0 && n < (1LL << 31) && xo < (1LL << 29) && yo < (1LL << 29), "%s: ragged batch too large or unaligned", who);
  for (int s = rg->nseg; s <= MAX_SEG; ++s) sg.n0[s] = (int)n;
  sg.nseg = rg->nseg;
  return 0;
}
int64_t seg_pixels(const prn_ragged* rg, int B) {
  int64_t n = 0;
  for (int s = 0; s < rg->nseg; ++s) n += (int64_t)B * rg->H[s] * rg->W[s];
  return n;
}
int conv_fwd_impl(const prn_conv_desc* d, const prn_ragged* rg, const float* x, const float* w, const float* bias, const float* addend, float* y,
                  void* ws, void* stream, int phase, unsigned* counters = nullptr, const void* w_images = nullptr);
int conv_wgrad_impl(const prn_conv_desc* d, const prn_ragged* rg, const float* x, const float* dy, float* dw, void* ws, void* stream, int phase);
}

extern "C" int prn_conv2d_kernel_kind(const prn_conv_desc* d) {
  if (check_desc(d, "prn_conv2d_kernel_kind")) return -1;
  if (direct_small_m(d) || direct_one_c(d)) return 1;
  int ss = split_plan_of(d);
  if (ss == 0) ss = taps_plan_of(d);
  if (ss == 0) ss = up2_plan_of(d);
  return ss == 0 ? 0 : (ss == 1 ? 2 : 3);
}

extern "C" int prn_conv2d_fwd_partials(const prn_conv_desc* d, int64_t* offset_bytes) {
  if (check_desc(d, "prn_conv2d_fwd_partials")) return -1;
  PRN_REQUIRE(offset_bytes != nullptr, "prn_conv2d_fwd_partials: null offset");
  *offset_bytes = 0;
  if (direct_small_m(d) || direct_one_c(d)) return 0;
  if (const int ss = split_plan_of(d)) {
    *offset_bytes = (prn_split_gemm_image_bytes(d->M, d->C, 1) + 255) & ~255LL;
    return ss > 1 ? ss : 0;
  }
  if (taps_plan_of(d) || up2_plan_of(d)) return 0;
  const Geo g = geo_of(d);
  const FwdPlan p = plan_fwd(d->M, (int64_t)d->B * g.gH * g.gW, d->C * d->KH * d->KW, narrow_available(d->KH, d->in_mode), g.phases, g.nosplit,
                             wide_ks(d->KH, d->in_mode));
  return p.splits > 1 ? p.splits : 0;
}

extern "C" int prn_conv2d_fwd_phase(const prn_conv_desc* d, const float* x, const float* w, const float* bias,
                                    const float* addend, float* y, void* ws, void* stream, int phase) {
  return conv_fwd_impl(d, nullptr, x, w, bias, addend, y, ws, stream, phase);
}

extern "C" int prn_conv2d_fwd_counted(const prn_conv_desc* d, const float* x, const float* w, const void* w_images, const float* bias, const float* addend,
                                      float* y, void* ws, unsigned* counters, void* stream, int phase) {
  return conv_fwd_impl(d, nullptr, x, w, bias, addend, y, ws, stream, phase, counters, w_images);
}

extern "C" int prn_conv2d_fwd_ragged(const prn_conv_desc* d, const prn_ragged* rg, const float* x, const float* w, const float* bias,
                                     const float* addend, float* y, void* stream) {
  PRN_REQUIRE(rg != nullptr, "prn_conv2d_fwd_ragged: null segment list");
  return conv_fwd_impl(d, rg, x, w, bias, addend, y, nullptr, stream, 0);
}

namespace {
int conv_fwd_impl(const prn_conv_desc* d0, const prn_ragged* rg, const float* x, const float* w, const float* bias, const float* addend, float* y,
                  void* ws, void* stream, int phase, unsigned* counters, const void* w_images) {
  prn_conv_desc dd;
  const prn_conv_desc* d = d0;
  if (rg && d0) {
    dd = *d0; dd.H = dd.Ho = rg->H[0]; dd.W = dd.Wo = rg->W[0]; d = &dd;
  }
  if (int e = check_desc(d, "prn_conv2d_fwd")) return e;
  PRN_REQUIRE(x && w && y, "prn_conv2d_fwd: null tensor");
  if (rg == nullptr && (direct_small_m(d) || direct_one_c(d))) {
    if (phase == 2) return 0;
    hipStream_t sd = (hipStream_t)stream;
    if (direct_small_m(d)) {
      const dim3 grid(cdiv((int64_t)d->B * d->H * d->W, 256)), block(256);
#define PRN_SMALL_M(MODE_, MM_) hipLaunchKernelGGL((conv3x3_small_m_kernel<MODE_, MM_>), grid, block, 0, sd, x, w, bias, addend, y, d->B, d->C, d->H, d->W, \
                                                   d->pad, d->epilogue)
      if (d->in_mode == PRN_IN_ZERO) { if (d->M == 1) PRN_SMALL_M(PRN_IN_ZERO, 1); else PRN_SMALL_M(PRN_IN_ZERO, 2); }
      else { if (d->M == 1) PRN_SMALL_M(PRN_IN_REFLECT, 1); else PRN_SMALL_M(PRN_IN_REFLECT, 2); }
#undef PRN_SMALL_M
    } else {
      hipLaunchKernelGGL(conv3x3_one_c_kernel, dim3(cdiv((int64_t)d->B * d->Ho * d->Wo, 256)), dim3(256), 0, sd, x, w, bias, addend, y, d->B, d->H, d->W,
                         d->M, d->pad, d->Ho, d->Wo, d->epilogue);
    }
    PRN_CHECK_LAUNCH("prn_conv2d_fwd/direct");
    return 0;
  }
  if (rg == nullptr && ws != nullptr) {
    if (const int ss = split_plan_of(d)) {
      const int64_t ib = (prn_split_gemm_image_bytes(d->M, d->C, 1) + 255) & ~255LL;
      return prn_split_gemm(w, w_images, x, bias, addend, y, ws, (float*)((char*)ws + ib), d->M, d->C, d->B, d->H * d->W, 1, 0, 0, 0, d->epilogue, ss, &d->opts,
                            (hipStream_t)stream, phase);
    }
    if (up2_plan_of(d) && addend == nullptr && (reinterpret_cast<uintptr_t>(y) & 15) == 0) {
      if (phase == 2) return 0;
      return prn_split_conv_up2(w, x, bias, y, ws, d->M, d->C, d->B, d->H, d->W, d->epilogue, &d->opts, (hipStream_t)stream);
    }
    if (const int st = taps_plan_of(d)) {
      const int64_t ib = (prn_split_gemm_image_bytes(d->M, d->C * d->KH * d->KW, 1) + 255) & ~255LL;
      return prn_split_conv_taps(w, x, bias, addend, y, ws, (float*)((char*)ws + ib), d->M, d->C, d->B, d->H, d->W, d->Ho, d->Wo, d->KH, d->KW, d->stride, d->pad, d->epilogue,
                                 st, &d->opts, (hipStream_t)stream, phase);
    }
  }
  ConvArgs a;
  a.x = x; a.w = w; a.bias = bias; a.addend = addend; a.y = y; a.ws = (float*)ws;
  a.B = d->B; a.C = d->C; a.H = d->H; a.W = d->W; a.M = d->M; a.stride = d->stride; a.pad = d->pad;
  const Geo g = geo_of(d);
// ... 370 lines not shown
```

### planerecnet_amd/csrc/prn_gemm_split.hip

```cpp
#include "prn_common.h"
#include <stdlib.h>

namespace {

typedef __attribute__((ext_vector_type(8))) __bf16 bf16x8_t;
typedef __attribute__((ext_vector_type(16))) float f32x16_t;
typedef int i32x4_t __attribute__((ext_vector_type(4)));
typedef float f32x4_t __attribute__((ext_vector_type(4)));

constexpr int BM = 128, BK = 32;
constexpr int IMG_U4 = 1536;

__device__ __forceinline__ void split2(float x0, float x1, unsigned& h, unsigned& m, unsigned& l) {
  const unsigned u0 = __float_as_uint(x0), u1 = __float_as_uint(x1);
  const float r0 = x0 - __uint_as_float(u0 & 0xffff0000u), r1 = x1 - __uint_as_float(u1 & 0xffff0000u);
  const unsigned v0 = __float_as_uint(r0), v1 = __float_as_uint(r1);
  const float s0 = r0 - __uint_as_float(v0 & 0xffff0000u), s1 = r1 - __uint_as_float(v1 & 0xffff0000u);
  h = __builtin_amdgcn_perm(u1, u0, 0x07060302u);
  m = __builtin_amdgcn_perm(v1, v0, 0x07060302u);
  l = __builtin_amdgcn_perm(__float_as_uint(s1), __float_as_uint(s0), 0x07060302u);
}

__global__ void split_prepare_kernel(const float* __restrict__ w, uint4* __restrict__ img, int M, int K, long long zw, int mtiles, int kslices, long long total) {
  const long long i = (long long)blockIdx.x * 256 + threadIdx.x;
// ... 176 lines not shown
}

__global__ void split16_prepare_kernel(const float* __restrict__ w, uint4* __restrict__ img, const int* __restrict__ ex, int M, int K, long long zw, int mtiles, int kslices,
                                       long long total, int taps = 1) {
  const long long i = (long long)blockIdx.x * 256 + threadIdx.x;
  if (i >= total) return;
  const int g = i % 4; const int r = (i / 4) % 128; const long long t = i / 512;
  const int ks = t % kslices; const long long zm = t / kslices; const int mt = zm % mtiles; const long long z = zm / mtiles;
  const int m = mt * 128 + r, k0 = ks * 32 + g * 8;
  const int sh = 14 - ex[z * (mtiles * 128) + m];
  float v[8];
  const int C = K / taps;
#pragma unroll
  for (int j = 0; j < 8; ++j) {
    const int kp = k0 + j;
    const int ksrc = taps > 1 ? (kp % C) * taps + kp / C : kp;
    v[j] = (m < M && kp < K) ? ldexpf(w[z * zw + (long long)m * K + ksrc], sh) : 0.f;
  }
  uint4 h, l;
  split2_f16(v[0], v[1], h.x, l.x); split2_f16(v[2], v[3], h.y, l.y); split2_f16(v[4], v[5], h.z, l.z); split2_f16(v[6], v[7], h.w, l.w);
  uint4* o = img + t * IMG16_U4;
  o[g * 128 + r] = h; o[(4 + g) * 128 + r] = l;
}

#ifdef PRN_S16_TIMING
__device__ long long prn_s16_dbg[8192 * 6];
#define S16_T(slot_) do { if (t == 0 && blockIdx.x + gridDim.x * blockIdx.y < 8192) prn_s16_dbg[(blockIdx.x + gridDim.x * blockIdx.y) * 6 + (slot_)] = (long long)wall_clock64(); } while (0)
__device__ long long prn_s16_it[64 * 4 * 4];
#define S16_IT(slot_) do { if (t == 0 && (blockIdx.x == 0 || blockIdx.x == gridDim.x / 2) && blockIdx.y == 0 && ks - ks0 < 64) { \
    if ((slot_) == 2) asm volatile("s_waitcnt vmcnt(0)" ::: "memory"); \
    prn_s16_it[((blockIdx.x ? 1 : 0) * 64 + (ks - ks0)) * 4 + (slot_)] = (long long)wall_clock64(); } } while (0)
extern "C" int prn_debug_s16_iter(long long* host, int n) { return (int)hipMemcpyFromSymbol(host, HIP_SYMBOL(prn_s16_it), sizeof(long long) * (size_t)n); }
extern "C" int prn_debug_s16_timing(long long* host, int n) { return (int)hipMemcpyFromSymbol(host, HIP_SYMBOL(prn_s16_dbg), sizeof(long long) * (size_t)n); }
#else
#define S16_T(slot_) do { } while (0)
#define S16_IT(slot_) do { } while (0)
#endif

__device__ __forceinline__ void store4_policy(float* p, float4 v, int pol) {
  const f32x4_t q = {v.x, v.y, v.z, v.w};
  if (pol == 0) *reinterpret_cast<float4*>(p) = v;
  else if (pol == 1) asm volatile("global_store_dwordx4 %0, %1, off sc1" ::"v"(p), "v"(q) : "memory");
  else if (pol == 2) asm volatile("global_store_dwordx4 %0, %1, off nt" ::"v"(p), "v"(q) : "memory");
  else if (pol == 3) asm volatile("global_store_dwordx4 %0, %1, off sc0 sc1" ::"v"(p), "v"(q) : "memory");
  else asm volatile("global_store_dwordx4 %0, %1, off sc1 nt" ::"v"(p), "v"(q) : "memory");
}

struct Split16Args {
  const uint4* img; const int* ex; const float* x; const float* bias; const float* addend; float* y; float* partial;
  int M, K, B, HW, epi, mtiles, kslices, ptiles, total, splits;
  int wide;
  int store_policy;
  long long zx, zy, slice;
  int C, XH, XW, Wo, KW, stride, pad;
};

template <int NP, int TAPS = 0>
__global__ __launch_bounds__(256) __attribute__((amdgpu_waves_per_eu(3, 3))) void split16_gemm_kernel(const Split16Args a) {
  __shared__ uint4 lds[2 * IMG16_U4];
  const int t = threadIdx.x, lane = t & 63, wave = __builtin_amdgcn_readfirstlane(t >> 6);
  const int id = prn_xcd_remap(blockIdx.x, a.total);
  const int mt = id % a.mtiles; const int rest = id / a.mtiles;
  const int pt = rest % a.ptiles; const int zb = rest / a.ptiles; const int b = zb % a.B, z = zb / a.B;
  const int sp = blockIdx.y;
  const int ks0 = (int)((long long)a.kslices * sp / a.splits), ks1 = (int)((long long)a.kslices * (sp + 1) / a.splits);
  const int HW = a.HW, M = a.M;
  const int r = lane & 31, gs = lane >> 5;
  S16_T(0);
#ifdef PRN_S16_TIMING
  if (t == 0 && blockIdx.x + gridDim.x * blockIdx.y < 8192) {
    unsigned hw, xcc; asm volatile("s_getreg_b32 %0, hwreg(HW_REG_HW_ID)" : "=s"(hw)); asm volatile("s_getreg_b32 %0, hwreg(HW_REG_XCC_ID)" : "=s"(xcc));
    prn_s16_dbg[(blockIdx.x + gridDim.x * blockIdx.y) * 6 + 4] = ((long long)(xcc & 15) << 32) | hw;
  }
#endif
  const int px = pt * 128 + wave * 32 + r;
  const int pxc = px < HW ? px : HW - 1;
  const int XHW = TAPS ? a.XH * a.XW : HW;
  const int XK = TAPS ? a.C : a.K;
  const float* xb = a.x + (long long)z * a.zx + (long long)b * XK * XHW;
  const __amdgpu_buffer_rsrc_t xrs = __builtin_amdgcn_make_buffer_rsrc(const_cast<float*>(xb), 0, XK * XHW * 4, 0x00020000);
  const int xoff = (pxc + gs * 8 * HW) * 4;
  int choff[16];
#pragma unroll
  for (int j = 0; j < 16; ++j) choff[j] = __builtin_amdgcn_readfirstlane(min(((j >> 3) * 16 + (j & 7)) * XHW * 4, XK * XHW * 4));
  const int t_oi = TAPS ? pxc / a.Wo : 0, t_oj = TAPS ? pxc - t_oi * a.Wo : 0;
  const int t_iy0 = t_oi * a.stride - a.pad, t_ix0 = t_oj * a.stride - a.pad;
  auto tap_vo = [&](int ks_) -> int {
    const int k0 = ks_ * BK, tp = __builtin_amdgcn_readfirstlane(k0 / a.C), c0 = __builtin_amdgcn_readfirstlane(k0 - tp * a.C);
    const int ty = __builtin_amdgcn_readfirstlane(tp / a.KW), tx = __builtin_amdgcn_readfirstlane(tp - ty * a.KW);
    int iy = t_iy0 + ty, ix = t_ix0 + tx;
    bool ok = (unsigned)iy < (unsigned)a.XH && (unsigned)ix < (unsigned)a.XW && k0 < a.K;
    if (TAPS == 2) {
      iy = min(max(t_oi + (z >> 1) - 1 + ty, 0), a.XH - 1); ix = min(max(t_oj + (z & 1) - 1 + tx, 0), a.XW - 1);
      ok = k0 < a.K;
    }
    return ok ? (iy * a.XW + ix + (c0 + gs * 8) * XHW) * 4 : (int)0x80000000u;
  };
  const uint4* ag = a.img + ((long long)(z * a.mtiles + mt) * a.kslices) * IMG16_U4;
  const i32x4_t adesc = make_desc(ag, (unsigned)a.kslices * IMG16_U4 * 16u);
  const unsigned lds0 = (unsigned)(unsigned long long)(void*)lds;
  float rn[16];
  f16x8_t bp[2][2];
  int erun = -1000, de = 0;
  const unsigned podd = (unsigned)__builtin_popcount((unsigned)px) & 1u;
  const unsigned sflip16 = podd ? 0x80008000u : 0u, sflip32 = podd ? 0x80000000u : 0u;
#define S16_DMA(ks_, st_) do { \
// ... 74 lines not shown
    __builtin_amdgcn_sched_barrier(0);
    S16_STEP(1);
    S16_IT(1);
    S16_IT(2);
    if (more) S16_PIECES(); else de = 0;
    __builtin_amdgcn_sched_barrier(0);
    S16_LOADB(ks + 2);
    S16_IT(3);
  }
#undef S16_DMA
#undef S16_LOADB
#undef S16_PIECES
#undef S16_STEP
  S16_T(2);
  const bool cok = px < HW;
  const int* exm = a.ex + (long long)z * a.mtiles * 128 + mt * 128;
  float* yb = a.y + (long long)z * a.zy + (long long)b * M * HW;
  const float* ab = a.addend ? a.addend + (long long)z * a.zy + (long long)b * M * HW : nullptr;
  float* pb = a.splits > 1 ? a.partial + (long long)sp * a.slice + ((long long)z * a.B + b) * (long long)M * HW : nullptr;
  if (a.wide) {
    __syncthreads();
    float* cw = reinterpret_cast<float*>(lds) + wave * (32 * 36);
    int* exl = reinterpret_cast<int*>(lds) + 4 * (32 * 36);
    if (t < 128) exl[t] = exm[t];
    __syncthreads();
    const int crow = lane >> 3, ccol = (lane & 7) * 4;
    const int px4 = pt * 128 + wave * 32 + ccol;
    const bool pok = px4 < HW;
    const bool fin = a.splits == 1;
#pragma unroll
    for (int i = 0; i < 4; ++i) {
#pragma unroll
      for (int e = 0; e < 16; ++e) {
        const int ro = (e >> 2) * 8 + (e & 3) + gs * 4;
        cw[ro * 36 + r] = __uint_as_float(__float_as_uint(ldexpf(acc[i][e], erun + exl[i * 32 + ro] - 28)) ^ sflip32);
      }
      __builtin_amdgcn_wave_barrier();
#pragma unroll
      for (int q = 0; q < 4; ++q) {
        const int rl = crow + 8 * q, row = mt * BM + i * 32 + rl;
        float4 v = *reinterpret_cast<const float4*>(&cw[rl * 36 + ccol]);
        if (!pok || row >= M) continue;
        const long long idx = (long long)row * HW + px4;
        if (TAPS == 2) {
          if (a.bias) { const float bm = a.bias[row]; v.x += bm; v.y += bm; v.z += bm; v.w += bm; }
          if (a.epi == PRN_EPI_RELU) { v.x = fmaxf(v.x, 0.f); v.y = fmaxf(v.y, 0.f); v.z = fmaxf(v.z, 0.f); v.w = fmaxf(v.w, 0.f); }
          const int oi4 = px4 / a.Wo, oj4 = px4 - oi4 * a.Wo;
          float* yp = a.y + (((long long)b * M + row) * (2 * a.XH) + 2 * oi4 + (z >> 1)) * (2 * a.XW) + 2 * oj4 + (z & 1);
          yp[0] = v.x; yp[2] = v.y; yp[4] = v.z; yp[6] = v.w;
          continue;
        }
        if (fin) {
          if (a.bias) { const float bm = a.bias[row]; v.x += bm; v.y += bm; v.z += bm; v.w += bm; }
          if (ab) { const float4 t4 = *reinterpret_cast<const float4*>(ab + idx); v.x += t4.x; v.y += t4.y; v.z += t4.z; v.w += t4.w; }
          if (a.epi == PRN_EPI_RELU) { v.x = fmaxf(v.x, 0.f); v.y = fmaxf(v.y, 0.f); v.z = fmaxf(v.z, 0.f); v.w = fmaxf(v.w, 0.f); }
          else if (a.epi == PRN_EPI_SIGMOID) { v.x = 1.f / (1.f + expf(-v.x)); v.y = 1.f / (1.f + expf(-v.y)); v.z = 1.f / (1.f + expf(-v.z)); v.w = 1.f / (1.f + expf(-v.w)); }
          store4_policy(yb + idx, v, a.store_policy);
        } else {
          store4_policy(pb + idx, v, a.store_policy);
        }
      }
      __builtin_amdgcn_wave_barrier();
    }
#ifdef PRN_S16_TIMING
    asm volatile("s_waitcnt vmcnt(0)" ::: "memory");
#endif
    S16_T(3);
    return;
  }
  if (a.splits > 1) {
#pragma unroll
    for (int i = 0; i < 4; ++i)
#pragma unroll
      for (int e = 0; e < 16; ++e) {
        const int rl = i * 32 + gs * 4 + (e >> 2) * 8 + (e & 3), row = mt * BM + rl;
        if (cok && row < M) pb[(long long)row * HW + px] = __uint_as_float(__float_as_uint(ldexpf(acc[i][e], erun + exm[rl] - 28)) ^ sflip32);
      }
    return;
  }
#pragma unroll
  for (int i = 0; i < 4; ++i) {
    const int rl0 = i * 32 + gs * 4, rbase = mt * BM + rl0;
    float bv[16], av[16]; int ev[16];
#pragma unroll
    for (int e = 0; e < 16; ++e) {
      const int ro = (e >> 2) * 8 + (e & 3), row = rbase + ro; const int rc = row < M ? row : M - 1;
      bv[e] = a.bias ? a.bias[rc] : 0.f; av[e] = ab ? ab[(long long)rc * HW + pxc] : 0.f; ev[e] = exm[rl0 + ro];
    }
#pragma unroll
    for (int e = 0; e < 16; ++e) {
      const int row = rbase + (e >> 2) * 8 + (e & 3);
      float v = __uint_as_float(__float_as_uint(ldexpf(acc[i][e], erun + ev[e] - 28)) ^ sflip32) + bv[e] + av[e];
      if (a.epi == PRN_EPI_RELU) v = fmaxf(v, 0.f);
      else if (a.epi == PRN_EPI_SIGMOID) v = 1.f / (1.f + expf(-v));
      if (cok && row < M) yb[(long long)row * HW + px] = v;
    }
  }
}

struct PrepItem { const float* src; uint4* dst; int M, K, nz, pad; long long zw; long long first; };
__global__ void split_prepare_batched_kernel(const PrepItem* __restrict__ items, int n) {
  int lo = 0, hi = n - 1;
  const long long blk = blockIdx.x;
  while (lo < hi) { const int mid = (lo + hi + 1) >> 1; if (items[mid].first <= blk) lo = mid; else hi = mid - 1; }
  const PrepItem it = items[lo];
  const int mtiles = (it.M + 127) / 128, kslices = (it.K + 31) / 32;
  const long long total = (long long)it.nz * mtiles * kslices * 512;
// ... 93 lines not shown
}
extern "C" void prn_gemm_opts_default(prn_gemm_opts* o) {
  if (!o) return;
  o->split_mode = PRN_SPLIT_PLAN; o->split_kind = PRN_PIECES_F16; o->split_products = 3; o->split_min_tiles = 300; o->split_min_gflop = 4.0f;
  o->wgrad_wgs = 0; o->wgrad_target = 0; o->wgrad_split = PRN_SPLIT_PLAN;
}
extern "C" int64_t prn_split_images_bytes(int M, int K, int nz) {
  if (M <= 0 || K <= 0 || nz <= 0) return -1;
  return prn_split_gemm_image_bytes(M, K, nz);
}
extern "C" int prn_split_prepare_batched(const void* items_dev, int n_items, int64_t total_blocks, int64_t total_row_blocks, int kind, void* stream) {
  PRN_REQUIRE(items_dev && n_items > 0 && total_blocks > 0 && total_blocks < (1LL << 31), "prn_split_prepare_batched: bad arguments");
  PRN_REQUIRE(kind == PRN_PIECES_F16 || kind == PRN_PIECES_BF16, "prn_split_prepare_batched: kind is PRN_PIECES_F16 or PRN_PIECES_BF16");
  if (kind == PRN_PIECES_F16) {
    PRN_REQUIRE(total_row_blocks > 0 && total_row_blocks < (1LL << 31), "prn_split_prepare_batched: the fp16 piece format needs the row-block count");
    hipLaunchKernelGGL(split16_rowmax_batched_kernel, dim3((unsigned)total_row_blocks), dim3(256), 0, (hipStream_t)stream, (const PrepItem*)items_dev, n_items);
    hipLaunchKernelGGL(split16_prepare_batched_kernel, dim3((unsigned)total_blocks), dim3(256), 0, (hipStream_t)stream, (const PrepItem*)items_dev, n_items);
    PRN_CHECK_LAUNCH("prn_split_prepare_batched/f16");
    return 0;
  }
  hipLaunchKernelGGL(split_prepare_batched_kernel, dim3((unsigned)total_blocks), dim3(256), 0, (hipStream_t)stream, (const PrepItem*)items_dev, n_items);
  PRN_CHECK_LAUNCH("prn_split_prepare_batched");
  return 0;
}
namespace {
int cut_weight(const float* w, void* images, int M, int K, int nz, long long zw, int kind, hipStream_t st, const char* who, int taps = 1) {
  const int mtiles = cdiv(M, 128), kslices = cdiv(K, 32);
  const long long ptotal = (long long)nz * mtiles * kslices * 512;
  if (kind == PRN_PIECES_F16) {
    int* ex = (int*)((char*)images + (int64_t)nz * mtiles * kslices * IMG16_U4 * 16);
    const long long rows = (long long)nz * mtiles * 128;
    hipLaunchKernelGGL(split16_rowmax_kernel, dim3(cdiv(rows, 4)), dim3(256), 0, st, w, ex, M, K, zw, mtiles * 128, rows);
    hipLaunchKernelGGL(split16_prepare_kernel, dim3(cdiv(ptotal, 256)), dim3(256), 0, st, w, (uint4*)images, (const int*)ex, M, K, zw, mtiles, kslices, ptotal, taps);
  } else {
    hipLaunchKernelGGL(split_prepare_kernel, dim3(cdiv(ptotal, 256)), dim3(256), 0, st, w, (uint4*)images, M, K, zw, mtiles, kslices, ptotal);
  }
  PRN_CHECK_LAUNCH(who);
  return 0;
}
}
extern "C" int prn_split_prepare(const float* w, void* images, int M, int K, int nz, int kind, void* stream) {
  PRN_REQUIRE(w && images && M > 0 && K > 0 && nz > 0 && (reinterpret_cast<uintptr_t>(images) & 15) == 0, "prn_split_prepare: bad arguments");
  PRN_REQUIRE(kind == PRN_PIECES_F16 || kind == PRN_PIECES_BF16, "prn_split_prepare: kind is PRN_PIECES_F16 or PRN_PIECES_BF16");
  return cut_weight(w, images, M, K, nz, (long long)M * K, kind, (hipStream_t)stream, "prn_split_prepare");
}
extern "C" int prn_gemm_pipe(int M, int K, int B, int HW, int nz, const prn_gemm_opts* opts) {
  return prn_split_gemm_plan(M, K, B, HW, nz, opts);
}
int64_t prn_split_gemm_image_bytes(int M, int K, int nz) { return (int64_t)nz * cdiv(M, 128) * cdiv(K, 32) * IMG_U4 * 16 + (int64_t)nz * cdiv(M, 128) * 128 * 4; }
int64_t prn_split_gemm_partial_bytes(int M, int B, int HW, int nz, int splits) { return splits > 1 ? (int64_t)splits * nz * B * M * HW * 4 : 0; }

int prn_split_gemm(const float* w, const void* w_images, const float* x, const float* bias, const float* addend, float* y, void* images_ws, float* partial, int M,
                   int K, int B, int HW, int nz, int64_t zw, int64_t zx, int64_t zy, int epi, int splits, const prn_gemm_opts* o, hipStream_t st, int phase) {
  PRN_REQUIRE(o != nullptr && w && x && y && (splits == 1 || partial), "prn_split_gemm: null operand");
  const int mtiles = cdiv(M, 128), kslices = cdiv(K, 32), ptiles = cdiv(HW, 128);
  PRN_REQUIRE((int64_t)kslices * IMG_U4 * 16 < (1LL << 31) && (int64_t)K * HW < (1LL << 29), "prn_split_gemm: operand larger than a buffer descriptor");
  const int kind = o->split_kind;
  PRN_REQUIRE(kind == PRN_PIECES_F16 || kind == PRN_PIECES_BF16, "prn_split_gemm: unknown piece format %d", kind);
  {
    static const int dbg = prn_env_int("PRN_SPLIT_DEBUG", 0);
    if (dbg) fprintf(stderr, "prn_split_gemm M=%d K=%d B=%d HW=%d nz=%d splits=%d epi=%d addend=%d\n", M, K, B, HW, nz, splits, epi, addend != nullptr);
  }
  if (phase != 2) {
    const void* images = w_images;
    if (images == nullptr) {
      PRN_REQUIRE(images_ws != nullptr, "prn_split_gemm: no workspace for the weight images");
      if (int e = cut_weight(w, images_ws, M, K, nz, (long long)zw, kind, st, "prn_split_gemm/prepare")) return e;
      images = images_ws;
    }
    PRN_REQUIRE((reinterpret_cast<uintptr_t>(images) & 15) == 0, "prn_split_gemm: images must be 16-byte aligned");
    if (kind == PRN_PIECES_F16) {
      Split16Args a;
      a.img = (const uint4*)images; a.ex = (const int*)((const char*)images + (int64_t)nz * mtiles * kslices * IMG16_U4 * 16);
      a.x = x; a.bias = bias; a.addend = addend; a.y = y; a.partial = partial;
      a.M = M; a.K = K; a.B = B; a.HW = HW; a.epi = epi; a.mtiles = mtiles; a.kslices = kslices; a.ptiles = ptiles;
      a.total = mtiles * ptiles * B * nz; a.splits = splits; a.zx = zx; a.zy = zy; a.slice = (long long)nz * B * M * HW;
      a.C = K; a.XH = 1; a.XW = HW; a.Wo = HW; a.KW = 1; a.stride = 1; a.pad = 0;
      {
        auto al16 = [](const void* q) { return (reinterpret_cast<uintptr_t>(q) & 15) == 0; };
        static const int wide_on = prn_env_int("PRN_SPLIT_WIDE_STORE", 1);
        a.wide = wide_on && (HW & 3) == 0 && ((int64_t)M * HW & 3) == 0 && (zy & 3) == 0 && al16(y) && al16(addend) && al16(partial);
        static const int policy = prn_env_int("PRN_SPLIT_STORE_POLICY", 1);
        a.store_policy = policy;
      }
      if (o->split_products >= 4) hipLaunchKernelGGL(split16_gemm_kernel<4>, dim3(a.total, splits), dim3(256), 0, st, a);
      else hipLaunchKernelGGL(split16_gemm_kernel<3>, dim3(a.total, splits), dim3(256), 0, st, a);
      PRN_CHECK_LAUNCH("prn_split_gemm/f16");
    } else {
      SplitArgs a;
      a.img = (const uint4*)images; a.x = x; a.bias = bias; a.addend = addend; a.y = y; a.partial = partial;
      a.M = M; a.K = K; a.B = B; a.HW = HW; a.epi = epi; a.mtiles = mtiles; a.kslices = kslices; a.ptiles = ptiles;
      a.total = mtiles * ptiles * B * nz; a.splits = splits; a.zx = zx; a.zy = zy; a.slice = (long long)nz * B * M * HW;
      hipLaunchKernelGGL(split_gemm_kernel, dim3(a.total, splits), dim3(256), 0, st, a);
      PRN_CHECK_LAUNCH("prn_split_gemm");
    }
  }
  if (splits > 1 && phase != 1) {
    PRN_REQUIRE(nz == 1 || (zy == (int64_t)B * M * HW), "prn_split_gemm: K splits need a dense output");
    return prn_launch_reduce_epilogue(partial, bias, addend, y, (int64_t)nz * B * M * HW, M, HW, splits, epi, st);
  }
  return 0;
}

int prn_split_conv_taps(const float* w, const float* x, const float* bias, const float* addend, float* y, void* images_ws, float* partial, int M, int C, int B, int XH,
                        int XW, int Ho, int Wo, int KH, int KW, int stride, int pad, int epi, int splits, const prn_gemm_opts* o, hipStream_t st, int phase) {
  PRN_REQUIRE(o != nullptr && w && x && y && images_ws && (splits == 1 || partial), "prn_split_conv_taps: null operand");
  PRN_REQUIRE(o->split_kind == PRN_PIECES_F16 && (C & 31) == 0 && KH > 0 && KW > 0, "prn_split_conv_taps: fp16 pieces and C %% 32 == 0 only");
  const int K = KH * KW * C, HW = Ho * Wo;
  const int mtiles = cdiv(M, 128), kslices = K / 32, ptiles = cdiv(HW, 128);
  PRN_REQUIRE((int64_t)kslices * IMG_U4 * 16 < (1LL << 31) && (int64_t)C * XH * XW < (1LL << 29) && (int64_t)M * HW < (1LL << 29),
              "prn_split_conv_taps: operand larger than a buffer descriptor");
  if (phase != 2) {
    if (int e = cut_weight(w, images_ws, M, K, 1, (long long)M * K, PRN_PIECES_F16, st, "prn_split_conv_taps/prepare", KH * KW)) return e;
    Split16Args a;
    a.img = (const uint4*)images_ws; a.ex = (const int*)((const char*)images_ws + (int64_t)mtiles * kslices * IMG16_U4 * 16);
    a.x = x; a.bias = bias; a.addend = addend; a.y = y; a.partial = partial;
    a.M = M; a.K = K; a.B = B; a.HW = HW; a.epi = epi; a.mtiles = mtiles; a.kslices = kslices; a.ptiles = ptiles;
    a.total = mtiles * ptiles * B; a.splits = splits; a.zx = 0; a.zy = 0; a.slice = (long long)B * M * HW;
    a.C = C; a.XH = XH; a.XW = XW; a.Wo = Wo; a.KW = KW; a.stride = stride; a.pad = pad;
    auto al16 = [](const void* q) { return (reinterpret_cast<uintptr_t>(q) & 15) == 0; };
    a.wide = (HW & 3) == 0 && ((int64_t)M * HW & 3) == 0 && al16(y) && al16(addend) && al16(partial);
    a.store_policy = 1;
    if (o->split_products >= 4) hipLaunchKernelGGL((split16_gemm_kernel<4, 1>), dim3(a.total, splits), dim3(256), 0, st, a);
    else hipLaunchKernelGGL((split16_gemm_kernel<3, 1>), dim3(a.total, splits), dim3(256), 0, st, a);
    PRN_CHECK_LAUNCH("prn_split_conv_taps");
  }
  if (splits > 1 && phase != 1) return prn_launch_reduce_epilogue(partial, bias, addend, y, (int64_t)B * M * HW, M, HW, splits, epi, st);
  return 0;
}

int prn_split_conv_up2(const float* wp, const float* x, const float* bias, float* y, void* images_ws, int M, int C, int B, int H, int W, int epi, const prn_gemm_opts* o,
                       hipStream_t st) {
  PRN_REQUIRE(o != nullptr && wp && x && y && images_ws, "prn_split_conv_up2: null operand");
  PRN_REQUIRE(o->split_kind == PRN_PIECES_F16 && (C & 31) == 0 && (W & 3) == 0 && (reinterpret_cast<uintptr_t>(y) & 15) == 0, "prn_split_conv_up2: fp16 pieces, C %% 32 == 0, W %% 4 == 0");
  const int K = 4 * C, HW = H * W;
  const int mtiles = cdiv(M, 128), kslices = K / 32, ptiles = cdiv(HW, 128);
  PRN_REQUIRE((int64_t)kslices * IMG_U4 * 16 < (1LL << 31) && (int64_t)C * HW < (1LL << 29) && (int64_t)B * M * HW * 4 < (1LL << 31), "prn_split_conv_up2: operand too large");
  if (int e = cut_weight(wp, images_ws, M, K, 4, (long long)M * K, PRN_PIECES_F16, st, "prn_split_conv_up2/prepare", 4)) return e;
  Split16Args a;
  a.img = (const uint4*)images_ws; a.ex = (const int*)((const char*)images_ws + (int64_t)4 * mtiles * kslices * IMG16_U4 * 16);
  a.x = x; a.bias = bias; a.addend = nullptr; a.y = y; a.partial = nullptr;
  a.M = M; a.K = K; a.B = B; a.HW = HW; a.epi = epi; a.mtiles = mtiles; a.kslices = kslices; a.ptiles = ptiles;
  a.total = mtiles * ptiles * B * 4; a.splits = 1; a.zx = 0; a.zy = 0; a.slice = 0;
  a.C = C; a.XH = H; a.XW = W; a.Wo = W; a.KW = 2; a.stride = 1; a.pad = 0;
  a.wide = 1; a.store_policy = 1;
  if (o->split_products >= 4) hipLaunchKernelGGL((split16_gemm_kernel<4, 2>), dim3(a.total, 1), dim3(256), 0, st, a);
  else hipLaunchKernelGGL((split16_gemm_kernel<3, 2>), dim3(a.total, 1), dim3(256), 0, st, a);
  PRN_CHECK_LAUNCH("prn_split_conv_up2");
  return 0;
}
```

### planerecnet_amd/csrc/prn_norm.hip

```cpp
#include <stdlib.h>
#include "prn_common.h"

namespace {


__device__ __forceinline__ void slice_bounds(int HW, int s, int S, bool vec, int& beg, int& end) {
  if (vec) {
    const int n4 = HW >> 2;
    beg = (int)((int64_t)n4 * s / S) * 4;
    end = (int)((int64_t)n4 * (s + 1) / S) * 4;
  } else {
    beg = (int)((int64_t)HW * s / S);
    end = (int)((int64_t)HW * (s + 1) / S);
  }
}

__global__ __launch_bounds__(256) void bn_partial_kernel(const float* __restrict__ x, double* __restrict__ ws, int B, int C, int HW) {
  const int c = blockIdx.x, s = blockIdx.y, S = gridDim.y;
  const bool vec = (HW & 3) == 0;
  int beg, end;
  slice_bounds(HW, s, S, vec, beg, end);
  float s1 = 0.f, s2 = 0.f;
  for (int b = 0; b < B; ++b) {
    const float* xp = x + ((size_t)b * C + c) * HW;
    if (vec) {
      for (int p = beg + threadIdx.x * 4; p < end; p += 1024) {
        const float4 v = *reinterpret_cast<const float4*>(xp + p);
        s1 += (v.x + v.y) + (v.z + v.w);
        s2 += (v.x * v.x + v.y * v.y) + (v.z * v.z + v.w * v.w);
      }
    } else {
      for (int p = beg + threadIdx.x; p < end; p += 256) {
        const float v = xp[p];
        s1 += v; s2 += v * v;
      }
    }
  }
  __shared__ double sm[16];
  double d1 = s1, d2 = s2;
  block_sum2(d1, d2, sm);
  if (threadIdx.x == 0) { ws[((size_t)c * S + s) * 2] = d1; ws[((size_t)c * S + s) * 2 + 1] = d2; }
}

__global__ void bn_finalize_kernel(const double* __restrict__ ws, float* __restrict__ stats, float* __restrict__ rmean,
                                   float* __restrict__ rvar, int C, int S, double count, float eps, float momentum) {
  const int c = blockIdx.x * blockDim.x + threadIdx.x;
  if (c >= C) return;
  double s1 = 0.0, s2 = 0.0;
  for (int s = 0; s < S; ++s) { s1 += ws[((size_t)c * S + s) * 2]; s2 += ws[((size_t)c * S + s) * 2 + 1]; }
  const double mean = s1 / count;
  double var = s2 / count - mean * mean;
  if (var < 0.0) var = 0.0;
  stats[c] = (float)mean;
  stats[C + c] = (float)(1.0 / sqrt(var + (double)eps));
  if (rmean) {
    const double unbiased = count > 1.0 ? var * count / (count - 1.0) : var;
    rmean[c] = (1.f - momentum) * rmean[c] + momentum * (float)mean;
    rvar[c] = (1.f - momentum) * rvar[c] + momentum * (float)unbiased;
  }
}

template <bool FIN>
__global__ __launch_bounds__(256) void bn_apply_kernel(const float* __restrict__ x, float* __restrict__ stats,
                                                       const float* __restrict__ gamma, const float* __restrict__ beta,
                                                       const float* __restrict__ res, float* __restrict__ y, int C, int HW, int relu,
                                                       const double* __restrict__ ws, float* __restrict__ rmean, float* __restrict__ rvar,
                                                       int S, double count, float eps, float momentum, int64_t ybs) {
  const int bc = blockIdx.y, c = bc % C;
  float mean_f, istd_f;
  if (FIN) {
    double s1 = 0.0, s2 = 0.0;
    for (int s = 0; s < S; ++s) { s1 += ws[((size_t)c * S + s) * 2]; s2 += ws[((size_t)c * S + s) * 2 + 1]; }
    const double mean = s1 / count;
    double var = s2 / count - mean * mean;
    if (var < 0.0) var = 0.0;
    mean_f = (float)mean;
    istd_f = (float)(1.0 / sqrt(var + (double)eps));
    if (blockIdx.x == 0 && bc == c && threadIdx.x == 0) {
      stats[c] = mean_f;
      stats[C + c] = istd_f;
      if (rmean) {
        const double unbiased = count > 1.0 ? var * count / (count - 1.0) : var;
        rmean[c] = (1.f - momentum) * rmean[c] + momentum * mean_f;
        rvar[c] = (1.f - momentum) * rvar[c] + momentum * (float)unbiased;
      }
    }
  } else {
    mean_f = stats[c];
    istd_f = stats[C + c];
  }
  const float sc = istd_f * gamma[c], sh = beta[c] - mean_f * sc;
  const size_t base = (size_t)bc * HW;
  y += (size_t)(bc / C) * ybs + (size_t)c * HW - base;
  if ((HW & 3) == 0) {
    const int n4 = HW >> 2;
    const float4* xp = reinterpret_cast<const float4*>(x + base);
    const float4* rp = res ? reinterpret_cast<const float4*>(res + base) : nullptr;
    float4* yp = reinterpret_cast<float4*>(y + base);
    for (int i = blockIdx.x * 256 + threadIdx.x; i < n4; i += gridDim.x * 256) {
      float4 v = xp[i];
      v.x = fmaf(v.x, sc, sh); v.y = fmaf(v.y, sc, sh); v.z = fmaf(v.z, sc, sh); v.w = fmaf(v.w, sc, sh);
      if (rp) { const float4 r = rp[i]; v.x += r.x; v.y += r.y; v.z += r.z; v.w += r.w; }
      if (relu) { v.x = fmaxf(v.x, 0.f); v.y = fmaxf(v.y, 0.f); v.z = fmaxf(v.z, 0.f); v.w = fmaxf(v.w, 0.f); }
      yp[i] = v;
    }
  } else {
    for (int i = blockIdx.x * 256 + threadIdx.x; i < HW; i += gridDim.x * 256) {
      float v = fmaf(x[base + i], sc, sh);
      if (res) v += res[base + i];
      if (relu) v = fmaxf(v, 0.f);
      y[base + i] = v;
    }
  }
}

__global__ __launch_bounds__(256) void bn_bwd_partial_kernel(const float* __restrict__ dy, const float* __restrict__ x,
                                                             const float* __restrict__ y, const float* __restrict__ stats,
                                                             double* __restrict__ ws, int B, int C, int HW, int relu, const float* __restrict__ gamma,
                                                             const float* __restrict__ beta, int64_t dbs) {
  const int c = blockIdx.x, s = blockIdx.y, S = gridDim.y;
  const bool vec = (HW & 3) == 0;
  int beg, end;
  slice_bounds(HW, s, S, vec, beg, end);
  const float mean = stats[c], istd = stats[C + c];
  const float sc = relu == 2 ? istd * gamma[c] : 0.f, sh = relu == 2 ? beta[c] - mean * sc : 0.f;
  float s1 = 0.f, s2 = 0.f;
  for (int b = 0; b < B; ++b) {
    const size_t base = ((size_t)b * C + c) * HW;
    const float* dyb = dy + (size_t)b * dbs + (size_t)c * HW;
    if (vec) {
      for (int p = beg + threadIdx.x * 4; p < end; p += 1024) {
        float4 g = *reinterpret_cast<const float4*>(dyb + p);
        const float4 xv = *reinterpret_cast<const float4*>(x + base + p);
        if (relu == 1) {
          const float4 yv = *reinterpret_cast<const float4*>(y + base + p);
          g.x = yv.x > 0.f ? g.x : 0.f; g.y = yv.y > 0.f ? g.y : 0.f; g.z = yv.z > 0.f ? g.z : 0.f; g.w = yv.w > 0.f ? g.w : 0.f;
        } else if (relu == 2) {
          g.x = fmaf(xv.x, sc, sh) > 0.f ? g.x : 0.f; g.y = fmaf(xv.y, sc, sh) > 0.f ? g.y : 0.f;
          g.z = fmaf(xv.z, sc, sh) > 0.f ? g.z : 0.f; g.w = fmaf(xv.w, sc, sh) > 0.f ? g.w : 0.f;
        }
        s1 += (g.x + g.y) + (g.z + g.w);
        s2 += (g.x * (xv.x - mean) + g.y * (xv.y - mean)) + (g.z * (xv.z - mean) + g.w * (xv.w - mean));
      }
    } else {
      for (int p = beg + threadIdx.x; p < end; p += 256) {
        float g = dyb[p];
        if (relu == 1 && !(y[base + p] > 0.f)) g = 0.f;
        if (relu == 2 && !(fmaf(x[base + p], sc, sh) > 0.f)) g = 0.f;
        s1 += g; s2 += g * (x[base + p] - mean);
      }
    }
  }
  s2 *= istd;
  __shared__ double sm[16];
  double d1 = s1, d2 = s2;
  block_sum2(d1, d2, sm);
  if (threadIdx.x == 0) { ws[((size_t)c * S + s) * 2] = d1; ws[((size_t)c * S + s) * 2 + 1] = d2; }
}

__global__ __launch_bounds__(256) void bn_bwd_apply_kernel(const float* __restrict__ dy, const float* __restrict__ x,
                                                           const float* __restrict__ y, const float* __restrict__ stats,
                                                           const float* __restrict__ gamma, const double* __restrict__ ws,
                                                           float* __restrict__ dx, float* __restrict__ dres, int C, int HW,
                                                           int S, float inv_count, int relu, int frozen, int have_partials,
                                                           float* __restrict__ dgamma, float* __restrict__ dbeta,
                                                           const float* __restrict__ beta, int64_t dbs) {
  const int bc = blockIdx.y, c = bc % C;
  const float mean = stats[c], istd = stats[C + c], gi = gamma[c] * istd;
  const float sc = relu == 2 ? gi : 0.f, sh = relu == 2 ? beta[c] - mean * sc : 0.f;
  double t1 = 0.0, t2 = 0.0;
  if (have_partials)
    for (int s = 0; s < S; ++s) { t1 += ws[((size_t)c * S + s) * 2]; t2 += ws[((size_t)c * S + s) * 2 + 1]; }
  if (have_partials && blockIdx.x == 0 && bc == c && threadIdx.x == 0) {
    if (dbeta) dbeta[c] = (float)t1;
    if (dgamma) dgamma[c] = (float)t2;
  }
  const float m1 = frozen ? 0.f : (float)t1 * inv_count;
  const float m2 = frozen ? 0.f : (float)t2 * inv_count;
  const size_t base = (size_t)bc * HW;
  dy += (size_t)(bc / C) * dbs + (size_t)c * HW - base;
  if ((HW & 3) == 0) {
    const int n4 = HW >> 2;
    for (int i = blockIdx.x * 256 + threadIdx.x; i < n4; i += gridDim.x * 256) {
      float4 g = reinterpret_cast<const float4*>(dy + base)[i];
      const float4 xv = reinterpret_cast<const float4*>(x + base)[i];
      if (relu == 1) {
        const float4 yv = reinterpret_cast<const float4*>(y + base)[i];
        g.x = yv.x > 0.f ? g.x : 0.f; g.y = yv.y > 0.f ? g.y : 0.f; g.z = yv.z > 0.f ? g.z : 0.f; g.w = yv.w > 0.f ? g.w : 0.f;
      } else if (relu == 2) {
        g.x = fmaf(xv.x, sc, sh) > 0.f ? g.x : 0.f; g.y = fmaf(xv.y, sc, sh) > 0.f ? g.y : 0.f;
        g.z = fmaf(xv.z, sc, sh) > 0.f ? g.z : 0.f; g.w = fmaf(xv.w, sc, sh) > 0.f ? g.w : 0.f;
      }
      if (dres) reinterpret_cast<float4*>(dres + base)[i] = g;
      float4 o;
      o.x = gi * (g.x - m1 - (xv.x - mean) * istd * m2); o.y = gi * (g.y - m1 - (xv.y - mean) * istd * m2);
      o.z = gi * (g.z - m1 - (xv.z - mean) * istd * m2); o.w = gi * (g.w - m1 - (xv.w - mean) * istd * m2);
      reinterpret_cast<float4*>(dx + base)[i] = o;
    }
    return;
  }
  for (int i = blockIdx.x * 256 + threadIdx.x; i < HW; i += gridDim.x * 256) {
    float g = dy[base + i];
    if (relu == 1 && !(y[base + i] > 0.f)) g = 0.f;
    if (relu == 2 && !(fmaf(x[base + i], sc, sh) > 0.f)) g = 0.f;
    if (dres) dres[base + i] = g;
    const float xh = (x[base + i] - mean) * istd;
    dx[base + i] = gi * (g - m1 - xh * m2);
  }
}

constexpr int BN_SMALL_MAX = 12288;

__device__ __forceinline__ void plane_to_winograd_v(const float* __restrict__ plane, float* __restrict__ V, int c, int C, int B, int H, int W) {
  const int TW = W >> 2, TH = (H + 3) >> 2, P = B * TH * TW, P4 = (P + 3) & ~3, HW = H * W;
  const size_t zs = (size_t)C * P4;
  for (int p = threadIdx.x; p < P; p += 256) {
    const int tx = p % TW, ty = (p / TW) % TH, b = p / (TW * TH);
    const float* pb = plane + b * HW;
    const int w0 = 4 * tx;
    float d[6][6];
#pragma unroll
    for (int i = 0; i < 6; ++i) {
      const int ih = 4 * ty - 1 + i;
      const bool ok = (unsigned)ih < (unsigned)H;
      const float* row = pb + (ok ? ih : 0) * W;
      const float4 q = *reinterpret_cast<const float4*>(row + w0);
      const bool okl = w0 > 0, okr = w0 + 4 < W;
      const float l = row[okl ? w0 - 1 : 0], r = row[okr ? w0 + 4 : 0];
      d[i][0] = (ok && okl) ? l : 0.f;
      d[i][1] = ok ? q.x : 0.f; d[i][2] = ok ? q.y : 0.f; d[i][3] = ok ? q.z : 0.f; d[i][4] = ok ? q.w : 0.f;
      d[i][5] = (ok && okr) ? r : 0.f;
    }
    float t[6][6];
#pragma unroll
    for (int j = 0; j < 6; ++j) {
      float v[6], o[6];
#pragma unroll
      for (int i = 0; i < 6; ++i) v[i] = d[i][j];
      bt6(v, o);
#pragma unroll
      for (int i = 0; i < 6; ++i) t[i][j] = o[i];
    }
    float* out = V + (size_t)c * P4 + p;
#pragma unroll
    for (int i = 0; i < 6; ++i) {
      float o[6];
      bt6(t[i], o);
#pragma unroll
      for (int j = 0; j < 6; ++j) out[(size_t)(i * 6 + j) * zs] = o[j];
    }
  }
}

template <int NV, bool WINO = false>
__global__ __launch_bounds__(256) void bn_small_fwd_kernel(const float* __restrict__ x, float* __restrict__ stats, const float* __restrict__ gamma,
                                                           const float* __restrict__ beta, const float* __restrict__ res, float* __restrict__ y,
                                                           float* __restrict__ rmean, float* __restrict__ rvar, int B, int C, int HW, float eps,
                                                           float momentum, int relu, int64_t ybs, int nparts, int64_t pstride, float* __restrict__ xsum,
                                                           float* __restrict__ V = nullptr, int H = 0, int W = 0) {
  __shared__ float wino_plane[WINO ? BN_SMALL_MAX : 4];
  const int c = blockIdx.x, n4 = (B * HW) >> 2;
  const int64_t ydelta = ybs - (int64_t)C * HW;
  float4 v[NV];
  size_t off[NV];
  float s1 = 0.f, s2 = 0.f;
#pragma unroll
  for (int i = 0; i < NV; ++i) {
    const int q = threadIdx.x + i * 256;
    const int e = q < n4 ? q * 4 : 0, b = e / HW, p = e - b * HW;
    off[i] = ((size_t)b * C + c) * HW + p;
  }
#pragma unroll
  for (int i = 0; i < NV; ++i) v[i] = *reinterpret_cast<const float4*>(x + off[i]);
  __builtin_amdgcn_sched_barrier(0);
  for (int s = 1; s < nparts; ++s) {
    float4 t[NV];
#pragma unroll
    for (int i = 0; i < NV; ++i) t[i] = *reinterpret_cast<const float4*>(x + (size_t)s * pstride + off[i]);
    __builtin_amdgcn_sched_barrier(0);
#pragma unroll
    for (int i = 0; i < NV; ++i) { v[i].x += t[i].x; v[i].y += t[i].y; v[i].z += t[i].z; v[i].w += t[i].w; }
  }
  if (xsum) {
#pragma unroll
    for (int i = 0; i < NV; ++i)
      if (threadIdx.x + i * 256 < n4) *reinterpret_cast<float4*>(xsum + off[i]) = v[i];
  }
#pragma unroll
  for (int i = 0; i < NV; ++i) {
    if (threadIdx.x + i * 256 >= n4) v[i] = make_float4(0.f, 0.f, 0.f, 0.f);
    s1 += (v[i].x + v[i].y) + (v[i].z + v[i].w);
    s2 += (v[i].x * v[i].x + v[i].y * v[i].y) + (v[i].z * v[i].z + v[i].w * v[i].w);
  }
  __shared__ double sm[16];
  double d1 = s1, d2 = s2;
  block_sum2(d1, d2, sm);
  const double count = (double)B * HW, mean = d1 / count;
  double var = d2 / count - mean * mean;
  if (var < 0.0) var = 0.0;
  const float mean_f = (float)mean, istd_f = (float)(1.0 / sqrt(var + (double)eps));
  if (threadIdx.x == 0) {
    stats[c] = mean_f;
    stats[C + c] = istd_f;
    if (rmean) {
      const double unbiased = count > 1.0 ? var * count / (count - 1.0) : var;
      rmean[c] = (1.f - momentum) * rmean[c] + momentum * mean_f;
      rvar[c] = (1.f - momentum) * rvar[c] + momentum * (float)unbiased;
    }
  }
  const float sc = istd_f * gamma[c], sh = beta[c] - mean_f * sc;
  float4 r[NV];
  if (res) {
#pragma unroll
    for (int i = 0; i < NV; ++i) r[i] = *reinterpret_cast<const float4*>(res + off[i]);
    __builtin_amdgcn_sched_barrier(0);
  } else {
#pragma unroll
    for (int i = 0; i < NV; ++i) r[i] = make_float4(0.f, 0.f, 0.f, 0.f);
  }
#pragma unroll
  for (int i = 0; i < NV; ++i) {
    if (threadIdx.x + i * 256 >= n4) continue;
    float4 o = v[i];
    o.x = fmaf(o.x, sc, sh) + r[i].x; o.y = fmaf(o.y, sc, sh) + r[i].y; o.z = fmaf(o.z, sc, sh) + r[i].z; o.w = fmaf(o.w, sc, sh) + r[i].w;
    if (relu) { o.x = fmaxf(o.x, 0.f); o.y = fmaxf(o.y, 0.f); o.z = fmaxf(o.z, 0.f); o.w = fmaxf(o.w, 0.f); }
    size_t oy = off[i];
    if (ydelta) oy += (size_t)(((threadIdx.x + i * 256) * 4) / HW) * ydelta;
    *reinterpret_cast<float4*>(y + oy) = o;
    if constexpr (WINO) *reinterpret_cast<float4*>(&wino_plane[(threadIdx.x + i * 256) * 4]) = o;
  }
  if constexpr (WINO) {
    __syncthreads();
    plane_to_winograd_v(wino_plane, V, c, C, B, H, W);
  }
}

template <int NV, bool WINO = false>
__global__ __launch_bounds__(256) void bn_small_bwd_kernel(const float* __restrict__ dy, const float* __restrict__ x, const float* __restrict__ y,
                                                           const float* __restrict__ stats, const float* __restrict__ gamma,
                                                           const float* __restrict__ beta, float* __restrict__ dx, float* __restrict__ dres,
                                                           float* __restrict__ dgamma, float* __restrict__ dbeta, int B, int C, int HW, int relu,
                                                           int frozen, int64_t dbs, int nparts, int64_t pstride, float* __restrict__ V = nullptr, int H = 0,
                                                           int W = 0) {
  __shared__ float wino_plane[WINO ? BN_SMALL_MAX : 4];
  const int c = blockIdx.x, n4 = (B * HW) >> 2;
  const int64_t ddelta = dbs - (int64_t)C * HW;
  const float mean = stats[c], istd = stats[C + c], gi = gamma[c] * istd;
  const float sc = relu == 2 ? gi : 0.f, sh = relu == 2 ? beta[c] - mean * sc : 0.f;
  float4 g[NV], xv[NV];
  size_t off[NV];
  float s1 = 0.f, s2 = 0.f;
#pragma unroll
  for (int i = 0; i < NV; ++i) {
    const int q = threadIdx.x + i * 256;
    const int e = q < n4 ? q * 4 : 0, b = e / HW, p = e - b * HW;
    off[i] = ((size_t)b * C + c) * HW + p;
  }
#pragma unroll
  for (int i = 0; i < NV; ++i) {
    const int q = threadIdx.x + i * 256;
    g[i] = *reinterpret_cast<const float4*>(dy + off[i] + (ddelta ? (size_t)((q < n4 ? q * 4 : 0) / HW) * ddelta : 0));
    xv[i] = *reinterpret_cast<const float4*>(x + off[i]);
  }
  __builtin_amdgcn_sched_barrier(0);
  for (int s = 1; s < nparts; ++s) {
    float4 t[NV];
#pragma unroll
    for (int i = 0; i < NV; ++i) t[i] = *reinterpret_cast<const float4*>(dy + (size_t)s * pstride + off[i]);
    __builtin_amdgcn_sched_barrier(0);
#pragma unroll
    for (int i = 0; i < NV; ++i) { g[i].x += t[i].x; g[i].y += t[i].y; g[i].z += t[i].z; g[i].w += t[i].w; }
  }
  if (relu == 1) {
    float4 yv[NV];
#pragma unroll
    for (int i = 0; i < NV; ++i) yv[i] = *reinterpret_cast<const float4*>(y + off[i]);
    __builtin_amdgcn_sched_barrier(0);
#pragma unroll
    for (int i = 0; i < NV; ++i) {
      g[i].x = yv[i].x > 0.f ? g[i].x : 0.f; g[i].y = yv[i].y > 0.f ? g[i].y : 0.f;
      g[i].z = yv[i].z > 0.f ? g[i].z : 0.f; g[i].w = yv[i].w > 0.f ? g[i].w : 0.f;
    }
  } else if (relu == 2) {
#pragma unroll
    for (int i = 0; i < NV; ++i) {
      g[i].x = fmaf(xv[i].x, sc, sh) > 0.f ? g[i].x : 0.f; g[i].y = fmaf(xv[i].y, sc, sh) > 0.f ? g[i].y : 0.f;
      g[i].z = fmaf(xv[i].z, sc, sh) > 0.f ? g[i].z : 0.f; g[i].w = fmaf(xv[i].w, sc, sh) > 0.f ? g[i].w : 0.f;
    }
  }
#pragma unroll
  for (int i = 0; i < NV; ++i) {
    if (threadIdx.x + i * 256 >= n4) { g[i] = make_float4(0.f, 0.f, 0.f, 0.f); xv[i] = g[i]; }
    s1 += (g[i].x + g[i].y) + (g[i].z + g[i].w);
    s2 += (g[i].x * (xv[i].x - mean) + g[i].y * (xv[i].y - mean)) + (g[i].z * (xv[i].z - mean) + g[i].w * (xv[i].w - mean));
  }
  s2 *= istd;
  __shared__ double sm[16];
  double t1 = s1, t2 = s2;
  block_sum2(t1, t2, sm);
  if (threadIdx.x == 0) {
    if (dbeta) dbeta[c] = (float)t1;
    if (dgamma) dgamma[c] = (float)t2;
  }
  const float inv_count = 1.f / ((float)B * HW);
  const float m1 = frozen ? 0.f : (float)t1 * inv_count, m2 = frozen ? 0.f : (float)t2 * inv_count;
#pragma unroll
  for (int i = 0; i < NV; ++i) {
    if (threadIdx.x + i * 256 >= n4) continue;
    if (dres) *reinterpret_cast<float4*>(dres + off[i]) = g[i];
    float4 o;
    o.x = gi * (g[i].x - m1 - (xv[i].x - mean) * istd * m2); o.y = gi * (g[i].y - m1 - (xv[i].y - mean) * istd * m2);
    o.z = gi * (g[i].z - m1 - (xv[i].z - mean) * istd * m2); o.w = gi * (g[i].w - m1 - (xv[i].w - mean) * istd * m2);
    *reinterpret_cast<float4*>(dx + off[i]) = o;
    if constexpr (WINO) *reinterpret_cast<float4*>(&wino_plane[(threadIdx.x + i * 256) * 4]) = o;
  }
  if constexpr (WINO) {
    __syncthreads();
    plane_to_winograd_v(wino_plane, V, c, C, B, H, W);
  }
}

bool bn_small_ok(int B, int HW) {
  static const int on = prn_env_int("PRN_BN_SMALL", 1);
  return on && (HW & 3) == 0 && (int64_t)B * HW <= BN_SMALL_MAX;
}
}

extern "C" int prn_bn_kernel_kind(int B, int HW) { return bn_small_ok(B, HW) ? 1 : 0; }

namespace {

struct GnSeg { int nseg; int hw[6]; int off[6]; };
__device__ __forceinline__ int gn_seg_get(const int (&v)[6], int s) {
  int r = v[0];
#pragma unroll
  for (int t = 1; t < 6; ++t)
    if (s == t) r = v[t];
  return r;
}

// ... 125 lines not shown
    return;
  }
  for (int i = threadIdx.x; i < n; i += blockDim.x) {
    const int c = g * cpg + i / HW;
    float gg = dy[base + i];
    const float xh = (x[base + i] - mu) * istd;
    if (!(xh * gamma[c] + beta[c] > 0.f)) gg = 0.f;
    dx[base + i] = istd * (gamma[c] * gg - m1 - xh * m2);
  }
  (void)tot;
}

int bn_splits(int B, int HW) {
  int s = (int)(((int64_t)B * HW + 8191) / 8192);
  if (s > PRN_BN_SPLITS) s = PRN_BN_SPLITS;
  if (s < 1) s = 1;
  if (s > HW / 4 && HW >= 4) s = HW / 4;
  return s < 1 ? 1 : s;
}

}

extern "C" int prn_bn_stats(const float* x, float* stats, float* running_mean, float* running_var, double* ws,
                            int B, int C, int HW, float eps, float momentum, void* stream) {
  PRN_REQUIRE(x && stats && ws && B > 0 && C > 0 && HW > 0, "prn_bn_stats: bad arguments");
  hipStream_t st = (hipStream_t)stream;
  const int S = bn_splits(B, HW);
  hipLaunchKernelGGL(bn_partial_kernel, dim3(C, S), dim3(256), 0, st, x, ws, B, C, HW);
  PRN_CHECK_LAUNCH("prn_bn_stats/partial");
  hipLaunchKernelGGL(bn_finalize_kernel, dim3(cdiv(C, 128)), dim3(128), 0, st, (const double*)ws, stats, running_mean, running_var, C,
                     S, (double)B * HW, eps, momentum);
  PRN_CHECK_LAUNCH("prn_bn_stats/finalize");
  return 0;
}

extern "C" int prn_bn_apply(const float* x, const float* stats, const float* gamma, const float* beta, const float* residual,
                            float* y, int B, int C, int HW, int relu, void* stream) {
  PRN_REQUIRE(x && stats && gamma && beta && y && B > 0 && C > 0 && HW > 0, "prn_bn_apply: bad arguments");
  int gx = cdiv(HW, 256 * 8);
  if (gx < 1) gx = 1;
  PRN_REQUIRE((int64_t)B * C <= 65535, "prn_bn_apply: B*C too large for grid.y");
  hipLaunchKernelGGL((bn_apply_kernel<false>), dim3(gx, B * C), dim3(256), 0, (hipStream_t)stream, x, const_cast<float*>(stats), gamma, beta,
                     residual, y, C, HW, relu, (const double*)nullptr, (float*)nullptr, (float*)nullptr, 0, 0.0, 0.f, 0.f, (int64_t)C * HW);
  PRN_CHECK_LAUNCH("prn_bn_apply");
  return 0;
}

extern "C" int prn_bn_train_fwd(const float* x, float* stats, const float* gamma, const float* beta, const float* residual, float* y,
                                float* running_mean, float* running_var, double* ws, int B, int C, int HW, float eps, float momentum,
                                int relu, void* stream) {
  return prn_bn_train_fwd_into(x, stats, gamma, beta, residual, y, (int64_t)C * HW, running_mean, running_var, ws, B, C, HW, eps, momentum, relu, stream);
}

extern "C" int prn_bn_train_fwd_into(const float* x, float* stats, const float* gamma, const float* beta, const float* residual, float* y,
                                     int64_t y_batch_stride, float* running_mean, float* running_var, double* ws, int B, int C, int HW, float eps,
                                     float momentum, int relu, void* stream) {
  PRN_REQUIRE(x && stats && gamma && beta && y && B > 0 && C > 0 && HW > 0, "prn_bn_train_fwd: bad arguments");
  PRN_REQUIRE(ws || bn_small_ok(B, HW), "prn_bn_train_fwd: the two-launch path needs its workspace (prn_bn_kernel_kind(B, HW) == 0)");
  PRN_REQUIRE(y_batch_stride >= (int64_t)C * HW && ((HW & 3) || ((y_batch_stride & 3) == 0 && (reinterpret_cast<uintptr_t>(y) & 15) == 0)),
              "prn_bn_train_fwd_into: bad output batch stride / alignment");
  const int64_t ybs = y_batch_stride;
  PRN_REQUIRE((int64_t)B * C <= 65535, "prn_bn_train_fwd: B*C too large for grid.y");
  hipStream_t st = (hipStream_t)stream;
  if (bn_small_ok(B, HW)) {
    const int nv = cdiv(B * HW / 4, 256);
#define PRN_BN_SMALL_FWD(NV_) hipLaunchKernelGGL((bn_small_fwd_kernel<NV_>), dim3(C), dim3(256), 0, st, x, stats, gamma, beta, residual, y, \
                                                 running_mean, running_var, B, C, HW, eps, momentum, relu, ybs, 1, (int64_t)0, (float*)nullptr)
    if (nv <= 3) PRN_BN_SMALL_FWD(3); else if (nv <= 6) PRN_BN_SMALL_FWD(6); else if (nv <= 10) PRN_BN_SMALL_FWD(10); else PRN_BN_SMALL_FWD(12);
#undef PRN_BN_SMALL_FWD
    PRN_CHECK_LAUNCH("prn_bn_train_fwd/small");
    return 0;
  }
  const int S = bn_splits(B, HW);
  for (int r = PRN_REPS(1); r > 0; --r) hipLaunchKernelGGL(bn_partial_kernel, dim3(C, S), dim3(256), 0, st, x, ws, B, C, HW);
  PRN_CHECK_LAUNCH("prn_bn_train_fwd/partial");
  int gx = cdiv(HW, 256 * 8);
  if (gx < 1) gx = 1;
  hipLaunchKernelGGL((bn_apply_kernel<true>), dim3(gx, B * C), dim3(256), 0, st, x, stats, gamma, beta, residual, y, C, HW, relu,
                     (const double*)ws, running_mean, running_var, S, (double)B * HW, eps, momentum, ybs);
  PRN_CHECK_LAUNCH("prn_bn_train_fwd/apply");
  return 0;
}

extern "C" int prn_bn_bwd(const float* dy, const float* x, const float* y, const float* stats, const float* gamma, const float* beta,
                          float* dx, float* dres, float* dgamma, float* dbeta, double* ws,
                          int B, int C, int HW, int relu, int frozen, void* stream) {
  return prn_bn_bwd_from(dy, (int64_t)C * HW, x, y, stats, gamma, beta, dx, dres, dgamma, dbeta, ws, B, C, HW, relu, frozen, stream);
}

extern "C" int prn_bn_bwd_from(const float* dy, int64_t dy_batch_stride, const float* x, const float* y, const float* stats, const float* gamma,
                               const float* beta, float* dx, float* dres, float* dgamma, float* dbeta, double* ws,
                               int B, int C, int HW, int relu, int frozen, void* stream) {
  PRN_REQUIRE(dy && x && stats && gamma && dx && B > 0 && C > 0 && HW > 0, "prn_bn_bwd: bad arguments");
  PRN_REQUIRE(ws || bn_small_ok(B, HW), "prn_bn_bwd: the two-launch path needs its workspace (prn_bn_kernel_kind(B, HW) == 0)");
  PRN_REQUIRE(dy_batch_stride >= (int64_t)C * HW && ((HW & 3) || ((dy_batch_stride & 3) == 0 && (reinterpret_cast<uintptr_t>(dy) & 15) == 0)),
              "prn_bn_bwd_from: bad gradient batch stride / alignment");
  const int64_t dbs = dy_batch_stride;
  PRN_REQUIRE(!relu || y || (beta && !dres), "prn_bn_bwd: relu needs the forward output, or beta (and no residual) to recompute its sign");
  if (relu) relu = y ? 1 : 2;
  PRN_REQUIRE((int64_t)B * C <= 65535, "prn_bn_bwd: B*C too large for grid.y");
  hipStream_t st = (hipStream_t)stream;
  if (bn_small_ok(B, HW)) {
    const int nv = cdiv(B * HW / 4, 256);
#define PRN_BN_SMALL_BWD(NV_) hipLaunchKernelGGL((bn_small_bwd_kernel<NV_>), dim3(C), dim3(256), 0, st, dy, x, y, stats, gamma, beta, dx, dres, dgamma, \
                                                 dbeta, B, C, HW, relu, frozen, dbs, 1, (int64_t)0)
    if (nv <= 3) PRN_BN_SMALL_BWD(3); else if (nv <= 6) PRN_BN_SMALL_BWD(6); else if (nv <= 10) PRN_BN_SMALL_BWD(10); else PRN_BN_SMALL_BWD(12);
#undef PRN_BN_SMALL_BWD
    PRN_CHECK_LAUNCH("prn_bn_bwd/small");
    return 0;
  }
  const int S = bn_splits(B, HW);
  const int have = (!frozen || dgamma || dbeta) ? 1 : 0;
  if (have) {
    for (int r = PRN_REPS(2); r > 0; --r) hipLaunchKernelGGL(bn_bwd_partial_kernel, dim3(C, S), dim3(256), 0, st, dy, x, y, stats, ws, B, C, HW, relu, gamma, beta, dbs);
    PRN_CHECK_LAUNCH("prn_bn_bwd/partial");
  }
  int gx = cdiv(HW, 256 * 8);
  if (gx < 1) gx = 1;
  hipLaunchKernelGGL(bn_bwd_apply_kernel, dim3(gx, B * C), dim3(256), 0, st, dy, x, y, stats, gamma, (const double*)ws, dx, dres, C, HW,
                     S, 1.f / ((float)B * HW), relu, frozen, have, dgamma, dbeta, beta, dbs);
  PRN_CHECK_LAUNCH("prn_bn_bwd/apply");
  return 0;
}

extern "C" int prn_bn_train_fwd_partials(const float* parts, int nparts, int64_t part_stride, float* x_out, float* stats, const float* gamma, const float* beta,
                                         const float* residual, float* y, float* running_mean, float* running_var, int B, int C, int HW, float eps,
                                         float momentum, int relu, void* stream) {
  PRN_REQUIRE(parts && x_out && stats && gamma && beta && y && B > 0 && C > 0 && HW > 0, "prn_bn_train_fwd_partials: bad arguments");
  PRN_REQUIRE(nparts >= 1 && nparts <= 64 && (nparts == 1 || part_stride >= (int64_t)B * C * HW) && (part_stride & 3) == 0,
              "prn_bn_train_fwd_partials: 1..64 partial sums, a multiple of four elements and at least B*C*HW apart");
  PRN_REQUIRE(bn_small_ok(B, HW), "prn_bn_train_fwd_partials: only for maps the one-pass kernel takes (prn_bn_kernel_kind(B, HW) == 1)");
  PRN_REQUIRE(((reinterpret_cast<uintptr_t>(parts) | reinterpret_cast<uintptr_t>(x_out) | reinterpret_cast<uintptr_t>(y)) & 15) == 0,
              "prn_bn_train_fwd_partials: tensors must be 16-byte aligned");
  hipStream_t st = (hipStream_t)stream;
  const int nv = cdiv(B * HW / 4, 256);
  const int64_t ybs = (int64_t)C * HW;
#define PRN_BN_SMALL_FWD(NV_) hipLaunchKernelGGL((bn_small_fwd_kernel<NV_>), dim3(C), dim3(256), 0, st, parts, stats, gamma, beta, residual, y, \
                                                 running_mean, running_var, B, C, HW, eps, momentum, relu, ybs, nparts, part_stride, x_out)
  if (nv <= 3) PRN_BN_SMALL_FWD(3); else if (nv <= 6) PRN_BN_SMALL_FWD(6); else if (nv <= 10) PRN_BN_SMALL_FWD(10); else PRN_BN_SMALL_FWD(12);
#undef PRN_BN_SMALL_FWD
  PRN_CHECK_LAUNCH("prn_bn_train_fwd_partials");
  return 0;
}

extern "C" int prn_bn_bwd_partials(const float* dparts, int nparts, int64_t part_stride, const float* x, const float* y, const float* stats, const float* gamma,
                                   const float* beta, float* dx, float* dres, float* dgamma, float* dbeta, int B, int C, int HW, int relu, int frozen,
                                   void* stream) {
  PRN_REQUIRE(dparts && x && stats && gamma && dx && B > 0 && C > 0 && HW > 0, "prn_bn_bwd_partials: bad arguments");
  PRN_REQUIRE(nparts >= 1 && nparts <= 64 && (nparts == 1 || part_stride >= (int64_t)B * C * HW) && (part_stride & 3) == 0,
              "prn_bn_bwd_partials: 1..64 partial sums, a multiple of four elements and at least B*C*HW apart");
  PRN_REQUIRE(bn_small_ok(B, HW), "prn_bn_bwd_partials: only for maps the one-pass kernel takes (prn_bn_kernel_kind(B, HW) == 1)");
  PRN_REQUIRE((reinterpret_cast<uintptr_t>(dparts) & 15) == 0, "prn_bn_bwd_partials: partial sums must be 16-byte aligned");
  PRN_REQUIRE(!relu || y || (beta && !dres), "prn_bn_bwd_partials: relu needs the forward output, or beta (and no residual) to recompute its sign");
  if (relu) relu = y ? 1 : 2;
  hipStream_t st = (hipStream_t)stream;
  const int nv = cdiv(B * HW / 4, 256);
  const int64_t dbs = (int64_t)C * HW;
#define PRN_BN_SMALL_BWD(NV_) hipLaunchKernelGGL((bn_small_bwd_kernel<NV_>), dim3(C), dim3(256), 0, st, dparts, x, y, stats, gamma, beta, dx, dres, dgamma, \
                                                 dbeta, B, C, HW, relu, frozen, dbs, nparts, part_stride)
  if (nv <= 3) PRN_BN_SMALL_BWD(3); else if (nv <= 6) PRN_BN_SMALL_BWD(6); else if (nv <= 10) PRN_BN_SMALL_BWD(10); else PRN_BN_SMALL_BWD(12);
#undef PRN_BN_SMALL_BWD
  PRN_CHECK_LAUNCH("prn_bn_bwd_partials");
  return 0;
}

extern "C" int prn_bn_train_fwd_winograd(const float* parts, int nparts, int64_t part_stride, float* x_out, float* stats, const float* gamma, const float* beta,
                                         const float* residual, float* y, float* running_mean, float* running_var, float* V, int B, int C, int H, int W,
                                         float eps, float momentum, int relu, void* stream) {
  const int HW = H * W;
  PRN_REQUIRE(parts && stats && gamma && beta && y && V && B > 0 && C > 0 && H >= 5 && W >= 4 && (W & 3) == 0, "prn_bn_train_fwd_winograd: bad arguments");
  PRN_REQUIRE(nparts >= 1 && nparts <= 64 && (nparts == 1 || (x_out && part_stride >= (int64_t)B * C * HW)) && (part_stride & 3) == 0,
              "prn_bn_train_fwd_winograd: 1..64 partial sums (x_out required beyond one), a multiple of four elements and at least B*C*HW apart");
  PRN_REQUIRE(bn_small_ok(B, HW), "prn_bn_train_fwd_winograd: only for maps the one-pass kernel takes (prn_bn_kernel_kind(B, HW) == 1)");
  PRN_REQUIRE(((reinterpret_cast<uintptr_t>(parts) | reinterpret_cast<uintptr_t>(x_out) | reinterpret_cast<uintptr_t>(y)) & 15) == 0,
              "prn_bn_train_fwd_winograd: tensors must be 16-byte aligned");
// ... 108 lines not shown
```

Before: 194.3.

## Save packed ReLU sign bitmask in bottleneck BN and gate residual gradient in conv1 epilogue

The final BN+ReLU of each bottleneck now writes a packed 1-bit-per-element ReLU gate into the saved activations. The backward BN reads this gate instead of the full forward output to mask the gradient. For non-downsampling blocks whose conv1 backward uses the split GEMM path, the residual gradient is no longer materialized. Instead the GEMM epilogue applies the gate to dy directly while adding it as the addend. This cuts saved-activation memory and backward traffic (a full-size y read and a dres write/read), at the cost of gate pack/unpack logic and a new gated GEMM path.

```diff
diff --git a/include/prn.h b/include/prn.h
--- a/include/prn.h
+++ b/include/prn.h
@@ -60,6 +60,9 @@
   int32_t nseg;
   int32_t H[PRN_MAX_SEGMENTS], W[PRN_MAX_SEGMENTS];
 } prn_ragged;
+int prn_conv2d_gated_addend_ok(const prn_conv_desc* d);
+int prn_conv2d_fwd_gated(const prn_conv_desc* d, const float* x, const float* w, const void* w_images, const float* bias, const float* addend,
+                         const uint32_t* addend_gate, float* y, void* ws, void* stream);
 int prn_conv2d_fwd_ragged(const prn_conv_desc* d, const prn_ragged* rg, const float* x, const float* w, const float* bias,
                           const float* addend, float* y, void* stream);
 int64_t prn_conv2d_wgrad_ragged_ws_bytes(const prn_conv_desc* d, const prn_ragged* rg);
@@ -186,6 +189,12 @@
 int prn_bn_bwd_from(const float* dy, int64_t dy_batch_stride, const float* x, const float* y, const float* stats, const float* gamma,
                     const float* beta, float* dx, float* dres, float* dgamma, float* dbeta, double* ws,
                     int B, int C, int HW, int relu, int frozen, void* stream);
+int64_t prn_bn_gate_words(int B, int C, int HW);
+int prn_bn_train_fwd_gate(const float* x, float* stats, const float* gamma, const float* beta, const float* residual, float* y, uint32_t* gate,
+                          float* running_mean, float* running_var, double* ws, int B, int C, int HW, float eps, float momentum, int relu,
+                          void* stream);
+int prn_bn_bwd_gate(const float* dy, const float* x, const uint32_t* gate, const float* stats, const float* gamma, const float* beta, float* dx,
+                    float* dres, float* dgamma, float* dbeta, double* ws, int B, int C, int HW, void* stream);
 
 int prn_bn_train_fwd_partials(const float* parts, int nparts, int64_t part_stride, float* x_out, float* stats, const float* gamma, const float* beta,
                               const float* residual, float* y, float* running_mean, float* running_var, int B, int C, int HW, float eps, float momentum,
@@ -237,7 +246,9 @@
 enum { PRN_BLK_WINOGRAD = 1,
        PRN_BLK_HANDOVER = 2,
        PRN_BLK_KEEP_V = 4,
-       PRN_BLK_SCATTER_ACC = 8 };
+       PRN_BLK_SCATTER_ACC = 8,
+       PRN_BLK_RELU_GATE = 16,
+       PRN_BLK_GATE_ADDEND = 32 };
 enum { PRN_BLK_CONV2_DIRECT = 0, PRN_BLK_CONV2_WINOGRAD = 1, PRN_BLK_CONV2_DCN = 2 };
 typedef struct prn_bottleneck_desc {
   int32_t B, C, H, W;
@@ -270,7 +281,11 @@
        PRN_BLK_BN_GRAD_FLOATS,
        PRN_BLK_HANDOVERS,
        PRN_BLK_NEEDS_W1_IMG, PRN_BLK_NEEDS_W3_IMG, PRN_BLK_NEEDS_WD_IMG, PRN_BLK_NEEDS_W1T_IMG, PRN_BLK_NEEDS_W3T_IMG, PRN_BLK_NEEDS_WDT_IMG, PRN_BLK_NEEDS_U_IMG,
-       PRN_BLK_NEEDS_COLT_IMG, PRN_BLK_INFO_COUNT };
+       PRN_BLK_NEEDS_COLT_IMG,
+       PRN_BLK_RELU_GATED,
+       PRN_BLK_OFF_GATE,
+       PRN_BLK_GATED_ADDEND,
+       PRN_BLK_INFO_COUNT };
 int64_t prn_bottleneck_plan_bytes(void);
 int64_t prn_bottleneck_params_bytes(void);
 int prn_bottleneck_plan(const prn_bottleneck_desc* d, void* plan);
diff --git a/planerecnet_amd/_lib.py b/planerecnet_amd/_lib.py
--- a/planerecnet_amd/_lib.py
+++ b/planerecnet_amd/_lib.py
@@ -72,6 +72,8 @@
     "prn_gn_relu_bwd_ragged": (c_int, [P, P, P, P, P, P, P, P, c_int, c_int, c_int, P, c_int, P]),
     "prn_conv2d_fwd_phase": (c_int, [_DP, P, P, P, P, P, P, P, c_int]),
     "prn_conv2d_fwd_counted": (c_int, [_DP, P, P, P, P, P, P, P, P, P, c_int]),
+    "prn_conv2d_gated_addend_ok": (c_int, [_DP]),
+    "prn_conv2d_fwd_gated": (c_int, [_DP, P, P, P, P, P, P, P, P, P]),
     "prn_conv2d_wgrad_phase": (c_int, [_DP, P, P, P, P, P, c_int]),
     "prn_weight_flip_transpose": (c_int, [P, P, c_int, c_int, c_int, c_int, P]),
     "prn_weight_flip_transpose_batched": (c_int, [P, c_int, c_i64, P]),
@@ -170,6 +172,9 @@
     "prn_bn_apply": (c_int, [P, P, P, P, P, P, c_int, c_int, c_int, c_int, P]),
     "prn_bn_train_fwd": (c_int, [P] * 9 + [c_int, c_int, c_int, c_float, c_float, c_int, P]),
     "prn_bn_bwd": (c_int, [P] * 11 + [c_int] * 5 + [P]),
+    "prn_bn_gate_words": (c_i64, [c_int, c_int, c_int]),
+    "prn_bn_train_fwd_gate": (c_int, [P] * 10 + [c_int, c_int, c_int, c_float, c_float, c_int, P]),
+    "prn_bn_bwd_gate": (c_int, [P] * 11 + [c_int] * 3 + [P]),
     "prn_bn_train_fwd_into": (c_int, [P] * 6 + [c_i64] + [P] * 3 + [c_int, c_int, c_int, c_float, c_float, c_int, P]),
     "prn_bn_bwd_from": (c_int, [P, c_i64] + [P] * 10 + [c_int] * 5 + [P]),
     "prn_bn_train_fwd_partials": (c_int, [P, c_int, c_i64] + [P] * 8 + [c_int, c_int, c_int, c_float, c_float, c_int, P]),
diff --git a/planerecnet_amd/blocks.py b/planerecnet_amd/blocks.py
--- a/planerecnet_amd/blocks.py
+++ b/planerecnet_amd/blocks.py
@@ -10,12 +10,14 @@
 ENABLED = os.environ.get("PRN_BLOCKS", "1") == "1"
 HANDOVER = os.environ.get("PRN_BLOCK_HANDOVER", "1") == "1"
 SCATTER_ACCUMULATE = os.environ.get("PRN_SCATTER_ACC", "1") == "1"
+RELU_GATE = os.environ.get("PRN_RELU_GATE", "1") == "1"
+GATE_ADDEND = os.environ.get("PRN_GATE_ADDEND", "1") == "1"
 STATS = {"fwd": 0, "bwd": 0, "resolved": 0, "vouched": 0, "scatter_acc": 0}
 
-BLK_WINOGRAD, BLK_HANDOVER, BLK_KEEP_V, BLK_SCATTER_ACC = 1, 2, 4, 8
+BLK_WINOGRAD, BLK_HANDOVER, BLK_KEEP_V, BLK_SCATTER_ACC, BLK_RELU_GATE, BLK_GATE_ADDEND = 1, 2, 4, 8, 16, 32
 CONV2_DIRECT, CONV2_WINOGRAD, CONV2_DCN = 0, 1, 2
 (I_SAVE, I_GSAVE, I_FWD_WS, I_BWD_WS, I_HO, I_WO, I_CONV2, I_KEEPS_V, I_A1, I_V, I_A2, I_OM, I_TABLE, I_D1, I_D2, I_D3, I_DD, I_DOM, I_BN_FLOATS, I_HANDOVERS,
- I_W1_IMG, I_W3_IMG, I_WD_IMG, I_W1T_IMG, I_W3T_IMG, I_WDT_IMG, I_U_IMG, I_COLT_IMG, INFO_COUNT) = range(29)
+ I_W1_IMG, I_W3_IMG, I_WD_IMG, I_W1T_IMG, I_W3T_IMG, I_WDT_IMG, I_U_IMG, I_COLT_IMG, I_RELU_GATED, I_GATE, I_GATED_ADDEND, INFO_COUNT) = range(32)
 
 _SCRATCH = {}
 _F32 = torch.float32
@@ -60,6 +62,10 @@
         f |= BLK_KEEP_V
     if HANDOVER:
         f |= BLK_HANDOVER
+    if RELU_GATE:
+        f |= BLK_RELU_GATE
+        if GATE_ADDEND:
+            f |= BLK_GATE_ADDEND
     return f
 
 
diff --git a/planerecnet_amd/csrc/prn_bottleneck.hip b/planerecnet_amd/csrc/prn_bottleneck.hip
--- a/planerecnet_amd/csrc/prn_bottleneck.hip
+++ b/planerecnet_amd/csrc/prn_bottleneck.hip
@@ -3,7 +3,7 @@
 
 namespace {
 
-constexpr int32_t PLAN_MAGIC = 0x424c4b36;
+constexpr int32_t PLAN_MAGIC = 0x424c4b37;
 constexpr int64_t WINOGRAD_MIN_TILES = 128;
 
 inline int64_t up256(int64_t v) { return (v + 255) & ~255LL; }
@@ -16,12 +16,13 @@
   int32_t lazy1, parts1;
   int32_t v1, lazy2, keep_v;
   int32_t lazy3g, parts3g;
+  int32_t gate_addend;
   int32_t v2g, lazy2g;
-  int32_t pad2_;
+  int32_t gate;
   int64_t parts1_off, parts3g_off;
   prn_conv_desc c1, c2, c3, cd, c27, g1, g2, g3, gd, g27;
   prn_dcn_desc dcn;
-  int64_t s_c1, s_a1, s_v, s_c2, s_a2, s_c3, s_cd, s_om, s_table, s_stats[4], save_bytes;
+  int64_t s_c1, s_a1, s_v, s_c2, s_a2, s_c3, s_cd, s_om, s_table, s_stats[4], s_gate, save_bytes;
   int64_t q_d3, q_dd, q_d2, q_d1, q_dom, q_bn, gsave_bytes;
   int64_t f_c1, f_bn, f_v, f_yt, f_gemm, f_c2, f_c27, f_dcn, f_c3, f_cd, f_res, fwd_ws_bytes;
   int64_t b_bn, b_dres, b_g3, b_g3ws, b_v, b_yt, b_gemm, b_g2, b_g2ws, b_dcn, b_dx1, b_g27ws, b_g1ws, b_gdtmp, b_gdws, bwd_ws_bytes;
@@ -93,6 +94,9 @@
   L.parts3g = L.lazy3g ? p3 : 0; L.parts3g_off = L.lazy3g ? off : 0;
   L.v2g = ho && wino && L.small2;
   L.lazy2g = ho && wino && L.small1 && L.P4 <= 768;
+  const int64_t gate_words = (d.flags & PRN_BLK_RELU_GATE) ? prn_bn_gate_words(B, Q, Ho * Wo) : 0;
+  L.gate = gate_words > 0;
+  L.gate_addend = L.gate && (d.flags & PRN_BLK_GATE_ADDEND) && !d.downsample && prn_conv2d_gated_addend_ok(&L.g1) == 1;
   const int64_t n1 = (int64_t)B * P * H * W * 4, n2 = (int64_t)B * P * Ho * Wo * 4, n3 = (int64_t)B * Q * Ho * Wo * 4, nx = (int64_t)B * C * H * W * 4;
   const int64_t nv = wino ? 4LL * 36 * P * L.P4 : 0, nom = (int64_t)B * 27 * Ho * Wo * 4;
   const int Cmax = Q > C ? Q : C;
@@ -121,6 +125,7 @@
   put(L.s_cd, d.downsample ? n3 : 0);
   put(L.s_om, d.dcn ? nom : 0); put(L.s_table, n_table);
   put(L.s_stats[0], 8LL * P); put(L.s_stats[1], 8LL * P); put(L.s_stats[2], 8LL * Q); put(L.s_stats[3], d.downsample ? 8LL * Q : 0);
+  put(L.s_gate, 4 * gate_words);
   L.save_bytes = at;
   at = 0;
   put(L.q_d3, n3); put(L.q_dd, d.downsample ? n3 : 0); put(L.q_d2, n2); put(L.q_d1, n1); put(L.q_dom, d.dcn ? nom : 0);
@@ -184,6 +189,7 @@
   out[PRN_BLK_NEEDS_W1T_IMG] = prn_conv2d_kernel_kind(&L->g1) >= 2; out[PRN_BLK_NEEDS_W3T_IMG] = prn_conv2d_kernel_kind(&L->g3) >= 2;
   out[PRN_BLK_NEEDS_WDT_IMG] = (L->d.downsample && L->d.stride == 1 && prn_conv2d_kernel_kind(&L->gd) >= 2) ? 1 : 0;
   out[PRN_BLK_NEEDS_U_IMG] = (L->conv2_path == PRN_BLK_CONV2_WINOGRAD && prn_gemm_pipe(L->d.planes, L->d.planes, 1, L->P4, 36, &L->d.opts) >= 1) ? 1 : 0;
+  out[PRN_BLK_RELU_GATED] = L->gate; out[PRN_BLK_OFF_GATE] = L->s_gate; out[PRN_BLK_GATED_ADDEND] = L->gate_addend;
   out[PRN_BLK_NEEDS_COLT_IMG] = (L->d.dcn && prn_gemm_pipe(9 * L->d.planes, L->d.planes, L->d.B, L->Ho * L->Wo, 1, &L->d.opts) >= 1) ? 1 : 0;
   return 0;
 }
@@ -247,8 +253,8 @@
                              d.momentum[3], 0, stream));
     res = rd;
   }
-  return prn_bn_train_fwd(c3, st3, p->gamma[2], p->beta[2], res, y, p->running_mean[2], p->running_var[2], L.small2 ? nullptr : bnws, B, Q, Ho * Wo, d.eps[2], d.momentum[2],
-                          1, stream);
+  return prn_bn_train_fwd_gate(c3, st3, p->gamma[2], p->beta[2], res, y, L.gate ? (uint32_t*)raw(save, L.s_gate) : nullptr, p->running_mean[2], p->running_var[2],
+                               L.small2 ? nullptr : bnws, B, Q, Ho * Wo, d.eps[2], d.momentum[2], 1, stream);
 }
 
 extern "C" int prn_bottleneck_train_bwd(const void* plan, const prn_bottleneck_params* p, const float* x, const float* y, const float* dy, float* dx,
@@ -276,7 +282,12 @@
   float* dres = f32(ws, L.b_dres);
   const prn_gemm_opts* o = &d.opts;
   hipStream_t st = (hipStream_t)stream;
-  PRN_TRY(prn_bn_bwd(dy, c3, y, st3, p->gamma[2], p->beta[2], d3, dres, dg3, db3, L.small2 ? nullptr : bnws, B, Q, Ho * Wo, 1, 0, stream));
+  const uint32_t* gate = L.gate ? (const uint32_t*)raw(save, L.s_gate) : nullptr;
+  const bool gadd = L.gate_addend && ((reinterpret_cast<uintptr_t>(dy) | reinterpret_cast<uintptr_t>(dx)) & 15) == 0;
+  if (L.gate)
+    PRN_TRY(prn_bn_bwd_gate(dy, c3, gate, st3, p->gamma[2], p->beta[2], d3, gadd ? nullptr : dres, dg3, db3, L.small2 ? nullptr : bnws, B, Q, Ho * Wo, stream));
+  else
+    PRN_TRY(prn_bn_bwd(dy, c3, y, st3, p->gamma[2], p->beta[2], d3, dres, dg3, db3, L.small2 ? nullptr : bnws, B, Q, Ho * Wo, 1, 0, stream));
   const float* addx = dres;
   if (d.downsample) {
     float* dd = f32(gsave, L.q_dd);
@@ -329,5 +340,6 @@
     PRN_TRY(prn_winograd_output_bn_bwd(Ytg, c1, st1, p->gamma[0], p->beta[0], d1, dg1, db1, B, P, H, W, 1, stream));
   else
     PRN_TRY(prn_bn_bwd(g2, c1, nullptr, st1, p->gamma[0], p->beta[0], d1, nullptr, dg1, db1, L.small1 ? nullptr : bnws, B, P, H * W, 1, 0, stream));
+  if (gadd) return prn_conv2d_fwd_gated(&L.g1, d1, p->w1_t, p->w1_t_img, nullptr, dy, gate, dx, raw(ws, L.b_g1ws, L.b_gdtmp - L.b_g1ws), stream);
   return prn_conv2d_fwd_counted(&L.g1, d1, p->w1_t, p->w1_t_img, nullptr, addx, dx, raw(ws, L.b_g1ws, L.b_gdtmp - L.b_g1ws), nullptr, stream, 0);
 }
diff --git a/planerecnet_amd/csrc/prn_common.h b/planerecnet_amd/csrc/prn_common.h
--- a/planerecnet_amd/csrc/prn_common.h
+++ b/planerecnet_amd/csrc/prn_common.h
@@ -113,6 +113,17 @@
   o[3] = d12 + 8.f * d34 + m[5];
 }
 
+__host__ __device__ inline int prn_gate_wpp(int HW) { return (HW + 31) >> 5; }
+__device__ __forceinline__ unsigned prn_gate_nibble_of(const float4& v) {
+  return (v.x > 0.f ? 1u : 0u) | (v.y > 0.f ? 2u : 0u) | (v.z > 0.f ? 4u : 0u) | (v.w > 0.f ? 8u : 0u);
+}
+__device__ __forceinline__ unsigned prn_gate_nibble(const uint32_t* __restrict__ plane_words, int p) {
+  return (plane_words[p >> 5] >> (((p >> 2) & 7) * 4)) & 15u;
+}
+__device__ __forceinline__ void prn_gate_apply(float4& g, unsigned nib) {
+  g.x = (nib & 1u) ? g.x : 0.f; g.y = (nib & 2u) ? g.y : 0.f; g.z = (nib & 4u) ? g.z : 0.f; g.w = (nib & 8u) ? g.w : 0.f;
+}
+
 static inline int cdiv(int64_t a, int64_t b) { return (int)((a + b - 1) / b); }
 __host__ __device__ inline size_t prn_align256(size_t v) { return (v + 255) & ~(size_t)255; }
 
@@ -128,6 +139,10 @@
 int64_t prn_split_gemm_partial_bytes(int M, int B, int HW, int nz, int splits);
 int prn_split_gemm(const float* w, const void* w_images, const float* x, const float* bias, const float* addend, float* y, void* images_ws, float* partial, int M,
                    int K, int B, int HW, int nz, int64_t zw, int64_t zx, int64_t zy, int epi, int splits, const prn_gemm_opts* opts, hipStream_t st, int phase);
+int prn_split_gemm_gate_ok(int M, int K, int B, int HW, const prn_gemm_opts* opts);
+int prn_split_gemm_gated(const float* w, const void* w_images, const float* x, const float* bias, const float* addend, const uint32_t* addend_gate, float* y,
+                         void* images_ws, float* partial, int M, int K, int B, int HW, int nz, int64_t zw, int64_t zx, int64_t zy, int epi, int splits,
+                         const prn_gemm_opts* opts, hipStream_t st, int phase);
 int prn_split_conv_taps(const float* w, const float* x, const float* bias, const float* addend, float* y, void* images_ws, float* partial, int M, int C, int B, int XH,
                         int XW, int Ho, int Wo, int KH, int KW, int stride, int pad, int epi, int splits, const prn_gemm_opts* o, hipStream_t st, int phase);
 int prn_split_conv_up2(const float* wp, const float* x, const float* bias, float* y, void* images_ws, int M, int C, int B, int H, int W, int epi, const prn_gemm_opts* o,
diff --git a/planerecnet_amd/csrc/prn_conv.hip b/planerecnet_amd/csrc/prn_conv.hip
--- a/planerecnet_amd/csrc/prn_conv.hip
+++ b/planerecnet_amd/csrc/prn_conv.hip
@@ -1503,6 +1503,22 @@
   return conv_fwd_impl(d, nullptr, x, w, bias, addend, y, ws, stream, phase, counters, w_images);
 }
 
+extern "C" int prn_conv2d_gated_addend_ok(const prn_conv_desc* d) {
+  if (check_desc(d, "prn_conv2d_gated_addend_ok")) return -1;
+  if (direct_small_m(d) || direct_one_c(d)) return 0;
+  return (split_plan_of(d) == 1 && prn_split_gemm_gate_ok(d->M, d->C, d->B, d->H * d->W, &d->opts)) ? 1 : 0;
+}
+
+extern "C" int prn_conv2d_fwd_gated(const prn_conv_desc* d, const float* x, const float* w, const void* w_images, const float* bias, const float* addend,
+                                    const uint32_t* addend_gate, float* y, void* ws, void* stream) {
+  if (int e = check_desc(d, "prn_conv2d_fwd_gated")) return e;
+  PRN_REQUIRE(x && w && y && addend && addend_gate && ws, "prn_conv2d_fwd_gated: null tensor / workspace");
+  PRN_REQUIRE(prn_conv2d_gated_addend_ok(d) == 1, "prn_conv2d_fwd_gated: this launch has no gated addend (prn_conv2d_gated_addend_ok)");
+  const int64_t ib = (prn_split_gemm_image_bytes(d->M, d->C, 1) + 255) & ~255LL;
+  return prn_split_gemm_gated(w, w_images, x, bias, addend, addend_gate, y, ws, (float*)((char*)ws + ib), d->M, d->C, d->B, d->H * d->W, 1, 0, 0, 0, d->epilogue, 1,
+                              &d->opts, (hipStream_t)stream, 0);
+}
+
 extern "C" int prn_conv2d_fwd_ragged(const prn_conv_desc* d, const prn_ragged* rg, const float* x, const float* w, const float* bias,
                                      const float* addend, float* y, void* stream) {
   PRN_REQUIRE(rg != nullptr, "prn_conv2d_fwd_ragged: null segment list");
diff --git a/planerecnet_amd/csrc/prn_gemm_split.hip b/planerecnet_amd/csrc/prn_gemm_split.hip
--- a/planerecnet_amd/csrc/prn_gemm_split.hip
+++ b/planerecnet_amd/csrc/prn_gemm_split.hip
@@ -252,6 +252,7 @@
   int wide;
   int store_policy;
   long long zx, zy, slice;
+  const uint32_t* gate;
   int C, XH, XW, Wo, KW, stride, pad;
 };
 
@@ -432,7 +433,13 @@
         }
         if (fin) {
           if (a.bias) { const float bm = a.bias[row]; v.x += bm; v.y += bm; v.z += bm; v.w += bm; }
-          if (ab) { const float4 t4 = *reinterpret_cast<const float4*>(ab + idx); v.x += t4.x; v.y += t4.y; v.z += t4.z; v.w += t4.w; }
+          if (ab) {
+            float4 t4 = *reinterpret_cast<const float4*>(ab + idx);
+            if constexpr (TAPS == 0) {
+              if (a.gate) prn_gate_apply(t4, prn_gate_nibble(a.gate + ((long long)b * M + row) * prn_gate_wpp(HW), px4));
+            }
+            v.x += t4.x; v.y += t4.y; v.z += t4.z; v.w += t4.w;
+          }
           if (a.epi == PRN_EPI_RELU) { v.x = fmaxf(v.x, 0.f); v.y = fmaxf(v.y, 0.f); v.z = fmaxf(v.z, 0.f); v.w = fmaxf(v.w, 0.f); }
           else if (a.epi == PRN_EPI_SIGMOID) { v.x = 1.f / (1.f + expf(-v.x)); v.y = 1.f / (1.f + expf(-v.y)); v.z = 1.f / (1.f + expf(-v.z)); v.w = 1.f / (1.f + expf(-v.w)); }
           store4_policy(yb + idx, v, a.store_policy);
@@ -632,7 +639,27 @@
 
 int prn_split_gemm(const float* w, const void* w_images, const float* x, const float* bias, const float* addend, float* y, void* images_ws, float* partial, int M,
                    int K, int B, int HW, int nz, int64_t zw, int64_t zx, int64_t zy, int epi, int splits, const prn_gemm_opts* o, hipStream_t st, int phase) {
+  return prn_split_gemm_gated(w, w_images, x, bias, addend, nullptr, y, images_ws, partial, M, K, B, HW, nz, zw, zx, zy, epi, splits, o, st, phase);
+}
+
+namespace {
+bool split_wide_store_on() {
+  static const int wide_on = prn_env_int("PRN_SPLIT_WIDE_STORE", 1);
+  return wide_on != 0;
+}
+}
+
+int prn_split_gemm_gate_ok(int M, int K, int B, int HW, const prn_gemm_opts* o) {
+  return o != nullptr && o->split_kind == PRN_PIECES_F16 && prn_split_gemm_plan(M, K, B, HW, 1, o) == 1 && split_wide_store_on() && (HW & 3) == 0;
+}
+
+int prn_split_gemm_gated(const float* w, const void* w_images, const float* x, const float* bias, const float* addend, const uint32_t* addend_gate, float* y,
+                         void* images_ws, float* partial, int M, int K, int B, int HW, int nz, int64_t zw, int64_t zx, int64_t zy, int epi, int splits,
+                         const prn_gemm_opts* o, hipStream_t st, int phase) {
   PRN_REQUIRE(o != nullptr && w && x && y && (splits == 1 || partial), "prn_split_gemm: null operand");
+  PRN_REQUIRE(!addend_gate || (addend && nz == 1 && splits == 1 && phase == 0 && prn_split_gemm_gate_ok(M, K, B, HW, o) &&
+                               ((reinterpret_cast<uintptr_t>(y) | reinterpret_cast<uintptr_t>(addend)) & 15) == 0),
+              "prn_split_gemm: a gated addend needs the fp16-piece kernel's float4 epilogue in one launch (no K split) and 16-byte aligned y / addend");
   const int mtiles = cdiv(M, 128), kslices = cdiv(K, 32), ptiles = cdiv(HW, 128);
   PRN_REQUIRE((int64_t)kslices * IMG_U4 * 16 < (1LL << 31) && (int64_t)K * HW < (1LL << 29), "prn_split_gemm: operand larger than a buffer descriptor");
   const int kind = o->split_kind;
@@ -652,14 +679,15 @@
     if (kind == PRN_PIECES_F16) {
       Split16Args a;
       a.img = (const uint4*)images; a.ex = (const int*)((const char*)images + (int64_t)nz * mtiles * kslices * IMG16_U4 * 16);
-      a.x = x; a.bias = bias; a.addend = addend; a.y = y; a.partial = partial;
+      a.x = x; a.bias = bias; a.addend = addend; a.y = y; a.partial = partial; a.gate = addend_gate;
       a.M = M; a.K = K; a.B = B; a.HW = HW; a.epi = epi; a.mtiles = mtiles; a.kslices = kslices; a.ptiles = ptiles;
       a.total = mtiles * ptiles * B * nz; a.splits = splits; a.zx = zx; a.zy = zy; a.slice = (long long)nz * B * M * HW;
       a.C = K; a.XH = 1; a.XW = HW; a.Wo = HW; a.KW = 1; a.stride = 1; a.pad = 0;
       {
         auto al16 = [](const void* q) { return (reinterpret_cast<uintptr_t>(q) & 15) == 0; };
-        static const int wide_on = prn_env_int("PRN_SPLIT_WIDE_STORE", 1);
+        const bool wide_on = split_wide_store_on();
         a.wide = wide_on && (HW & 3) == 0 && ((int64_t)M * HW & 3) == 0 && (zy & 3) == 0 && al16(y) && al16(addend) && al16(partial);
+        PRN_REQUIRE(!addend_gate || a.wide, "prn_split_gemm: a gated addend needs the float4 epilogue (16-byte aligned workspace)");
         static const int policy = prn_env_int("PRN_SPLIT_STORE_POLICY", 1);
         a.store_policy = policy;
       }
@@ -694,7 +722,7 @@
     if (int e = cut_weight(w, images_ws, M, K, 1, (long long)M * K, PRN_PIECES_F16, st, "prn_split_conv_taps/prepare", KH * KW)) return e;
     Split16Args a;
     a.img = (const uint4*)images_ws; a.ex = (const int*)((const char*)images_ws + (int64_t)mtiles * kslices * IMG16_U4 * 16);
-    a.x = x; a.bias = bias; a.addend = addend; a.y = y; a.partial = partial;
+    a.x = x; a.bias = bias; a.addend = addend; a.y = y; a.partial = partial; a.gate = nullptr;
     a.M = M; a.K = K; a.B = B; a.HW = HW; a.epi = epi; a.mtiles = mtiles; a.kslices = kslices; a.ptiles = ptiles;
     a.total = mtiles * ptiles * B; a.splits = splits; a.zx = 0; a.zy = 0; a.slice = (long long)B * M * HW;
     a.C = C; a.XH = XH; a.XW = XW; a.Wo = Wo; a.KW = KW; a.stride = stride; a.pad = pad;
@@ -719,7 +747,7 @@
   if (int e = cut_weight(wp, images_ws, M, K, 4, (long long)M * K, PRN_PIECES_F16, st, "prn_split_conv_up2/prepare", 4)) return e;
   Split16Args a;
   a.img = (const uint4*)images_ws; a.ex = (const int*)((const char*)images_ws + (int64_t)4 * mtiles * kslices * IMG16_U4 * 16);
-  a.x = x; a.bias = bias; a.addend = nullptr; a.y = y; a.partial = nullptr;
+  a.x = x; a.bias = bias; a.addend = nullptr; a.y = y; a.partial = nullptr; a.gate = nullptr;
   a.M = M; a.K = K; a.B = B; a.HW = HW; a.epi = epi; a.mtiles = mtiles; a.kslices = kslices; a.ptiles = ptiles;
   a.total = mtiles * ptiles * B * 4; a.splits = 1; a.zx = 0; a.zy = 0; a.slice = 0;
   a.C = C; a.XH = H; a.XW = W; a.Wo = W; a.KW = 2; a.stride = 1; a.pad = 0;
diff --git a/planerecnet_amd/csrc/prn_norm.hip b/planerecnet_amd/csrc/prn_norm.hip
--- a/planerecnet_amd/csrc/prn_norm.hip
+++ b/planerecnet_amd/csrc/prn_norm.hip
@@ -60,12 +60,13 @@
   }
 }
 
-template <bool FIN>
+template <bool FIN, bool GATE = false>
 __global__ __launch_bounds__(256) void bn_apply_kernel(const float* __restrict__ x, float* __restrict__ stats,
                                                        const float* __restrict__ gamma, const float* __restrict__ beta,
                                                        const float* __restrict__ res, float* __restrict__ y, int C, int HW, int relu,
                                                        const double* __restrict__ ws, float* __restrict__ rmean, float* __restrict__ rvar,
-                                                       int S, double count, float eps, float momentum, int64_t ybs) {
+                                                       int S, double count, float eps, float momentum, int64_t ybs,
+                                                       uint32_t* __restrict__ gate = nullptr) {
   const int bc = blockIdx.y, c = bc % C;
   float mean_f, istd_f;
   if (FIN) {
@@ -92,6 +93,26 @@
   const float sc = istd_f * gamma[c], sh = beta[c] - mean_f * sc;
   const size_t base = (size_t)bc * HW;
   y += (size_t)(bc / C) * ybs + (size_t)c * HW - base;
+  if constexpr (GATE) {
+    const int n4 = HW >> 2;
+    const float4* xp = reinterpret_cast<const float4*>(x + base);
+    const float4* rp = res ? reinterpret_cast<const float4*>(res + base) : nullptr;
+    float4* yp = reinterpret_cast<float4*>(y + base);
+    uint32_t* gp = gate + (size_t)bc * prn_gate_wpp(HW);
+    for (int i0 = blockIdx.x * 256 + threadIdx.x; (i0 & ~7) < n4; i0 += gridDim.x * 256) {
+      const bool ok = i0 < n4;
+      const int i = ok ? i0 : n4 - 1;
+      float4 v = xp[i];
+      v.x = fmaf(v.x, sc, sh); v.y = fmaf(v.y, sc, sh); v.z = fmaf(v.z, sc, sh); v.w = fmaf(v.w, sc, sh);
+      if (rp) { const float4 r = rp[i]; v.x += r.x; v.y += r.y; v.z += r.z; v.w += r.w; }
+      if (relu) { v.x = fmaxf(v.x, 0.f); v.y = fmaxf(v.y, 0.f); v.z = fmaxf(v.z, 0.f); v.w = fmaxf(v.w, 0.f); }
+      if (ok) yp[i] = v;
+      unsigned w = ok ? prn_gate_nibble_of(v) << ((threadIdx.x & 7) * 4) : 0u;
+      w |= (unsigned)__shfl_xor((int)w, 1, 64); w |= (unsigned)__shfl_xor((int)w, 2, 64); w |= (unsigned)__shfl_xor((int)w, 4, 64);
+      if ((threadIdx.x & 7) == 0) gp[i0 >> 3] = w;
+    }
+    return;
+  }
   if ((HW & 3) == 0) {
     const int n4 = HW >> 2;
     const float4* xp = reinterpret_cast<const float4*>(x + base);
@@ -117,7 +138,8 @@
 __global__ __launch_bounds__(256) void bn_bwd_partial_kernel(const float* __restrict__ dy, const float* __restrict__ x,
                                                              const float* __restrict__ y, const float* __restrict__ stats,
                                                              double* __restrict__ ws, int B, int C, int HW, int relu, const float* __restrict__ gamma,
-                                                             const float* __restrict__ beta, int64_t dbs) {
+                                                             const float* __restrict__ beta, int64_t dbs,
+                                                             const uint32_t* __restrict__ gate = nullptr, float* __restrict__ gout = nullptr) {
   const int c = blockIdx.x, s = blockIdx.y, S = gridDim.y;
   const bool vec = (HW & 3) == 0;
   int beg, end;
@@ -138,6 +160,9 @@
         } else if (relu == 2) {
           g.x = fmaf(xv.x, sc, sh) > 0.f ? g.x : 0.f; g.y = fmaf(xv.y, sc, sh) > 0.f ? g.y : 0.f;
           g.z = fmaf(xv.z, sc, sh) > 0.f ? g.z : 0.f; g.w = fmaf(xv.w, sc, sh) > 0.f ? g.w : 0.f;
+        } else if (relu == 3) {
+          prn_gate_apply(g, prn_gate_nibble(gate + ((size_t)b * C + c) * prn_gate_wpp(HW), p));
+          if (gout) *reinterpret_cast<float4*>(gout + base + p) = g;
         }
         s1 += (g.x + g.y) + (g.z + g.w);
         s2 += (g.x * (xv.x - mean) + g.y * (xv.y - mean)) + (g.z * (xv.z - mean) + g.w * (xv.w - mean));
@@ -164,7 +189,8 @@
                                                            float* __restrict__ dx, float* __restrict__ dres, int C, int HW,
                                                            int S, float inv_count, int relu, int frozen, int have_partials,
                                                            float* __restrict__ dgamma, float* __restrict__ dbeta,
-                                                           const float* __restrict__ beta, int64_t dbs) {
+                                                           const float* __restrict__ beta, int64_t dbs,
+                                                           const uint32_t* __restrict__ gate = nullptr) {
   const int bc = blockIdx.y, c = bc % C;
   const float mean = stats[c], istd = stats[C + c], gi = gamma[c] * istd;
   const float sc = relu == 2 ? gi : 0.f, sh = relu == 2 ? beta[c] - mean * sc : 0.f;
@@ -181,6 +207,24 @@
   dy += (size_t)(bc / C) * dbs + (size_t)c * HW - base;
   if ((HW & 3) == 0) {
     const int n4 = HW >> 2;
+    if (relu == 3) {
+      const uint32_t* gp = gate + (size_t)bc * prn_gate_wpp(HW);
+      for (int i = blockIdx.x * 256 + threadIdx.x; i < n4; i += gridDim.x * 256) {
+        float4 g;
+        if (dres) {
+          g = reinterpret_cast<const float4*>(dres + base)[i];
+        } else {
+          g = reinterpret_cast<const float4*>(dy + base)[i];
+          prn_gate_apply(g, prn_gate_nibble(gp, i * 4));
+        }
+        const float4 xv = reinterpret_cast<const float4*>(x + base)[i];
+        float4 o;
+        o.x = gi * (g.x - m1 - (xv.x - mean) * istd * m2); o.y = gi * (g.y - m1 - (xv.y - mean) * istd * m2);
+        o.z = gi * (g.z - m1 - (xv.z - mean) * istd * m2); o.w = gi * (g.w - m1 - (xv.w - mean) * istd * m2);
+        reinterpret_cast<float4*>(dx + base)[i] = o;
+      }
+      return;
+    }
     for (int i = blockIdx.x * 256 + threadIdx.x; i < n4; i += gridDim.x * 256) {
       float4 g = reinterpret_cast<const float4*>(dy + base)[i];
       const float4 xv = reinterpret_cast<const float4*>(x + base)[i];
@@ -252,13 +296,20 @@
   }
 }
 
-template <int NV, bool WINO = false>
+constexpr int BN_GATE_LDS_WORDS = BN_SMALL_MAX / 32 + 128;
+
+template <int NV, bool WINO = false, bool GATE = false>
 __global__ __launch_bounds__(256) void bn_small_fwd_kernel(const float* __restrict__ x, float* __restrict__ stats, const float* __restrict__ gamma,
                                                            const float* __restrict__ beta, const float* __restrict__ res, float* __restrict__ y,
                                                            float* __restrict__ rmean, float* __restrict__ rvar, int B, int C, int HW, float eps,
                                                            float momentum, int relu, int64_t ybs, int nparts, int64_t pstride, float* __restrict__ xsum,
-                                                           float* __restrict__ V = nullptr, int H = 0, int W = 0) {
+                                                           float* __restrict__ V = nullptr, int H = 0, int W = 0, uint32_t* __restrict__ gate = nullptr) {
   __shared__ float wino_plane[WINO ? BN_SMALL_MAX : 4];
+  __shared__ uint32_t gate_words[GATE ? BN_GATE_LDS_WORDS : 1];
+  const int wpp = prn_gate_wpp(HW);
+  if constexpr (GATE) {
+    for (int k = threadIdx.x; k < B * wpp; k += 256) gate_words[k] = 0u;
+  }
   const int c = blockIdx.x, n4 = (B * HW) >> 2;
   const int64_t ydelta = ybs - (int64_t)C * HW;
   float4 v[NV];
@@ -328,10 +379,21 @@
     if (ydelta) oy += (size_t)(((threadIdx.x + i * 256) * 4) / HW) * ydelta;
     *reinterpret_cast<float4*>(y + oy) = o;
     if constexpr (WINO) *reinterpret_cast<float4*>(&wino_plane[(threadIdx.x + i * 256) * 4]) = o;
+    if constexpr (GATE) {
+      const int e = (threadIdx.x + i * 256) * 4, b = e / HW, p = e - b * HW;
+      atomicOr(&gate_words[b * wpp + (p >> 5)], prn_gate_nibble_of(o) << (((p >> 2) & 7) * 4));
+    }
   }
   if constexpr (WINO) {
     __syncthreads();
     plane_to_winograd_v(wino_plane, V, c, C, B, H, W);
+  }
+  if constexpr (GATE) {
+    __syncthreads();
+    for (int k = threadIdx.x; k < B * wpp; k += 256) {
+      const int b = k / wpp;
+      gate[((size_t)b * C + c) * wpp + (k - b * wpp)] = gate_words[k];
+    }
   }
 }
 
@@ -341,7 +403,7 @@
                                                            const float* __restrict__ beta, float* __restrict__ dx, float* __restrict__ dres,
                                                            float* __restrict__ dgamma, float* __restrict__ dbeta, int B, int C, int HW, int relu,
                                                            int frozen, int64_t dbs, int nparts, int64_t pstride, float* __restrict__ V = nullptr, int H = 0,
-                                                           int W = 0) {
+                                                           int W = 0, const uint32_t* __restrict__ gate = nullptr) {
   __shared__ float wino_plane[WINO ? BN_SMALL_MAX : 4];
   const int c = blockIdx.x, n4 = (B * HW) >> 2;
   const int64_t ddelta = dbs - (int64_t)C * HW;
@@ -386,6 +448,22 @@
     for (int i = 0; i < NV; ++i) {
       g[i].x = fmaf(xv[i].x, sc, sh) > 0.f ? g[i].x : 0.f; g[i].y = fmaf(xv[i].y, sc, sh) > 0.f ? g[i].y : 0.f;
       g[i].z = fmaf(xv[i].z, sc, sh) > 0.f ? g[i].z : 0.f; g[i].w = fmaf(xv[i].w, sc, sh) > 0.f ? g[i].w : 0.f;
+    }
+  } else if (relu == 3) {
+    const int wpp = prn_gate_wpp(HW);
+    uint32_t gw[NV];
+#pragma unroll
+    for (int i = 0; i < NV; ++i) {
+      const int q = threadIdx.x + i * 256;
+      const int e = q < n4 ? q * 4 : 0, b = e / HW, p = e - b * HW;
+      gw[i] = gate[((size_t)b * C + c) * wpp + (p >> 5)];
+    }
+    __builtin_amdgcn_sched_barrier(0);
+#pragma unroll
+    for (int i = 0; i < NV; ++i) {
+      const int q = threadIdx.x + i * 256;
+      const int e = q < n4 ? q * 4 : 0, p = e % HW;
+      prn_gate_apply(g[i], (gw[i] >> (((p >> 2) & 7) * 4)) & 15u);
     }
   }
 #pragma unroll
@@ -617,9 +695,46 @@
   return prn_bn_train_fwd_into(x, stats, gamma, beta, residual, y, (int64_t)C * HW, running_mean, running_var, ws, B, C, HW, eps, momentum, relu, stream);
 }
 
+namespace {
+bool bn_gate_ok(int B, int HW) {
+  return (HW & 3) == 0 && (!bn_small_ok(B, HW) || (int64_t)B * prn_gate_wpp(HW) <= BN_GATE_LDS_WORDS);
+}
+int bn_train_fwd_impl(const float* x, float* stats, const float* gamma, const float* beta, const float* residual, float* y, int64_t y_batch_stride,
+                      float* running_mean, float* running_var, double* ws, int B, int C, int HW, float eps, float momentum, int relu, uint32_t* gate,
+                      void* stream);
+int bn_bwd_impl(const float* dy, int64_t dy_batch_stride, const float* x, const float* y, const uint32_t* gate, const float* stats, const float* gamma,
+                const float* beta, float* dx, float* dres, float* dgamma, float* dbeta, double* ws, int B, int C, int HW, int relu, int frozen, void* stream);
+}
+
+extern "C" int64_t prn_bn_gate_words(int B, int C, int HW) {
+  return (B > 0 && C > 0 && HW > 0 && bn_gate_ok(B, HW)) ? (int64_t)B * C * prn_gate_wpp(HW) : 0;
+}
+
 extern "C" int prn_bn_train_fwd_into(const float* x, float* stats, const float* gamma, const float* beta, const float* residual, float* y,
                                      int64_t y_batch_stride, float* running_mean, float* running_var, double* ws, int B, int C, int HW, float eps,
                                      float momentum, int relu, void* stream) {
+  return bn_train_fwd_impl(x, stats, gamma, beta, residual, y, y_batch_stride, running_mean, running_var, ws, B, C, HW, eps, momentum, relu, nullptr, stream);
+}
+
+extern "C" int prn_bn_train_fwd_gate(const float* x, float* stats, const float* gamma, const float* beta, const float* residual, float* y, uint32_t* gate,
+                                     float* running_mean, float* running_var, double* ws, int B, int C, int HW, float eps, float momentum, int relu,
+                                     void* stream) {
+  PRN_REQUIRE(!gate || (B > 0 && HW > 0 && bn_gate_ok(B, HW)), "prn_bn_train_fwd_gate: no packed gate for this shape (prn_bn_gate_words(B, C, HW) == 0)");
+  PRN_REQUIRE((reinterpret_cast<uintptr_t>(gate) & 3) == 0, "prn_bn_train_fwd_gate: the gate must be 4-byte aligned");
+  return bn_train_fwd_impl(x, stats, gamma, beta, residual, y, (int64_t)C * HW, running_mean, running_var, ws, B, C, HW, eps, momentum, relu, gate, stream);
+}
+
+extern "C" int prn_bn_bwd_gate(const float* dy, const float* x, const uint32_t* gate, const float* stats, const float* gamma, const float* beta, float* dx,
+                               float* dres, float* dgamma, float* dbeta, double* ws, int B, int C, int HW, void* stream) {
+  PRN_REQUIRE(gate && B > 0 && HW > 0 && bn_gate_ok(B, HW), "prn_bn_bwd_gate: needs the gate, for a shape that has one (prn_bn_gate_words(B, C, HW) != 0)");
+  PRN_REQUIRE((reinterpret_cast<uintptr_t>(gate) & 3) == 0, "prn_bn_bwd_gate: the gate must be 4-byte aligned");
+  return bn_bwd_impl(dy, (int64_t)C * HW, x, nullptr, gate, stats, gamma, beta, dx, dres, dgamma, dbeta, ws, B, C, HW, 3, 0, stream);
+}
+
+namespace {
+int bn_train_fwd_impl(const float* x, float* stats, const float* gamma, const float* beta, const float* residual, float* y, int64_t y_batch_stride,
+                      float* running_mean, float* running_var, double* ws, int B, int C, int HW, float eps, float momentum, int relu, uint32_t* gate,
+                      void* stream) {
   PRN_REQUIRE(x && stats && gamma && beta && y && B > 0 && C > 0 && HW > 0, "prn_bn_train_fwd: bad arguments");
   PRN_REQUIRE(ws || bn_small_ok(B, HW), "prn_bn_train_fwd: the two-launch path needs its workspace (prn_bn_kernel_kind(B, HW) == 0)");
   PRN_REQUIRE(y_batch_stride >= (int64_t)C * HW && ((HW & 3) || ((y_batch_stride & 3) == 0 && (reinterpret_cast<uintptr_t>(y) & 15) == 0)),
@@ -631,7 +746,15 @@
     const int nv = cdiv(B * HW / 4, 256);
 #define PRN_BN_SMALL_FWD(NV_) hipLaunchKernelGGL((bn_small_fwd_kernel<NV_>), dim3(C), dim3(256), 0, st, x, stats, gamma, beta, residual, y, \
                                                  running_mean, running_var, B, C, HW, eps, momentum, relu, ybs, 1, (int64_t)0, (float*)nullptr)
-    if (nv <= 3) PRN_BN_SMALL_FWD(3); else if (nv <= 6) PRN_BN_SMALL_FWD(6); else if (nv <= 10) PRN_BN_SMALL_FWD(10); else PRN_BN_SMALL_FWD(12);
+#define PRN_BN_SMALL_FWD_GATE(NV_) hipLaunchKernelGGL((bn_small_fwd_kernel<NV_, false, true>), dim3(C), dim3(256), 0, st, x, stats, gamma, beta, residual, y, \
+                                                      running_mean, running_var, B, C, HW, eps, momentum, relu, ybs, 1, (int64_t)0, (float*)nullptr,      \
+                                                      (float*)nullptr, 0, 0, gate)
+    if (gate) {
+      if (nv <= 3) PRN_BN_SMALL_FWD_GATE(3); else if (nv <= 6) PRN_BN_SMALL_FWD_GATE(6); else if (nv <= 10) PRN_BN_SMALL_FWD_GATE(10); else PRN_BN_SMALL_FWD_GATE(12);
+    } else {
+      if (nv <= 3) PRN_BN_SMALL_FWD(3); else if (nv <= 6) PRN_BN_SMALL_FWD(6); else if (nv <= 10) PRN_BN_SMALL_FWD(10); else PRN_BN_SMALL_FWD(12);
+    }
+#undef PRN_BN_SMALL_FWD_GATE
 #undef PRN_BN_SMALL_FWD
     PRN_CHECK_LAUNCH("prn_bn_train_fwd/small");
     return 0;
@@ -641,10 +764,15 @@
   PRN_CHECK_LAUNCH("prn_bn_train_fwd/partial");
   int gx = cdiv(HW, 256 * 8);
   if (gx < 1) gx = 1;
-  hipLaunchKernelGGL((bn_apply_kernel<true>), dim3(gx, B * C), dim3(256), 0, st, x, stats, gamma, beta, residual, y, C, HW, relu,
-                     (const double*)ws, running_mean, running_var, S, (double)B * HW, eps, momentum, ybs);
+  if (gate)
+    hipLaunchKernelGGL((bn_apply_kernel<true, true>), dim3(gx, B * C), dim3(256), 0, st, x, stats, gamma, beta, residual, y, C, HW, relu,
+                       (const double*)ws, running_mean, running_var, S, (double)B * HW, eps, momentum, ybs, gate);
+  else
+    hipLaunchKernelGGL((bn_apply_kernel<true>), dim3(gx, B * C), dim3(256), 0, st, x, stats, gamma, beta, residual, y, C, HW, relu,
+                       (const double*)ws, running_mean, running_var, S, (double)B * HW, eps, momentum, ybs, (uint32_t*)nullptr);
   PRN_CHECK_LAUNCH("prn_bn_train_fwd/apply");
   return 0;
+}
 }
 
 extern "C" int prn_bn_bwd(const float* dy, const float* x, const float* y, const float* stats, const float* gamma, const float* beta,
@@ -656,36 +784,48 @@
 extern "C" int prn_bn_bwd_from(const float* dy, int64_t dy_batch_stride, const float* x, const float* y, const float* stats, const float* gamma,
                                const float* beta, float* dx, float* dres, float* dgamma, float* dbeta, double* ws,
                                int B, int C, int HW, int relu, int frozen, void* stream) {
+  return bn_bwd_impl(dy, dy_batch_stride, x, y, nullptr, stats, gamma, beta, dx, dres, dgamma, dbeta, ws, B, C, HW, relu, frozen, stream);
+}
+
+namespace {
+int bn_bwd_impl(const float* dy, int64_t dy_batch_stride, const float* x, const float* y, const uint32_t* gate, const float* stats, const float* gamma,
+                const float* beta, float* dx, float* dres, float* dgamma, float* dbeta, double* ws, int B, int C, int HW, int relu, int frozen, void* stream) {
   PRN_REQUIRE(dy && x && stats && gamma && dx && B > 0 && C > 0 && HW > 0, "prn_bn_bwd: bad arguments");
   PRN_REQUIRE(ws || bn_small_ok(B, HW), "prn_bn_bwd: the two-launch path needs its workspace (prn_bn_kernel_kind(B, HW) == 0)");
   PRN_REQUIRE(dy_batch_stride >= (int64_t)C * HW && ((HW & 3) || ((dy_batch_stride & 3) == 0 && (reinterpret_cast<uintptr_t>(dy) & 15) == 0)),
               "prn_bn_bwd_from: bad gradient batch stride / alignment");
   const int64_t dbs = dy_batch_stride;
-  PRN_REQUIRE(!relu || y || (beta && !dres), "prn_bn_bwd: relu needs the forward output, or beta (and no residual) to recompute its sign");
-  if (relu) relu = y ? 1 : 2;
+  if (gate) {
+    relu = 3;
+  } else {
+    PRN_REQUIRE(!relu || y || (beta && !dres), "prn_bn_bwd: relu needs the forward output, or beta (and no residual) to recompute its sign");
+    if (relu) relu = y ? 1 : 2;
+  }
   PRN_REQUIRE((int64_t)B * C <= 65535, "prn_bn_bwd: B*C too large for grid.y");
   hipStream_t st = (hipStream_t)stream;
   if (bn_small_ok(B, HW)) {
     const int nv = cdiv(B * HW / 4, 256);
 #define PRN_BN_SMALL_BWD(NV_) hipLaunchKernelGGL((bn_small_bwd_kernel<NV_>), dim3(C), dim3(256), 0, st, dy, x, y, stats, gamma, beta, dx, dres, dgamma, \
-                                                 dbeta, B, C, HW, relu, frozen, dbs, 1, (int64_t)0)
+                                                 dbeta, B, C, HW, relu, frozen, dbs, 1, (int64_t)0, (float*)nullptr, 0, 0, gate)
     if (nv <= 3) PRN_BN_SMALL_BWD(3); else if (nv <= 6) PRN_BN_SMALL_BWD(6); else if (nv <= 10) PRN_BN_SMALL_BWD(10); else PRN_BN_SMALL_BWD(12);
 #undef PRN_BN_SMALL_BWD
     PRN_CHECK_LAUNCH("prn_bn_bwd/small");
     return 0;
   }
   const int S = bn_splits(B, HW);
-  const int have = (!frozen || dgamma || dbeta) ? 1 : 0;
+  const int have = (relu == 3 || !frozen || dgamma || dbeta) ? 1 : 0;
   if (have) {
-    for (int r = PRN_REPS(2); r > 0; --r) hipLaunchKernelGGL(bn_bwd_partial_kernel, dim3(C, S), dim3(256), 0, st, dy, x, y, stats, ws, B, C, HW, relu, gamma, beta, dbs);
+    for (int r = PRN_REPS(2); r > 0; --r)
+      hipLaunchKernelGGL(bn_bwd_partial_kernel, dim3(C, S), dim3(256), 0, st, dy, x, y, stats, ws, B, C, HW, relu, gamma, beta, dbs, gate, relu == 3 ? dres : (float*)nullptr);
     PRN_CHECK_LAUNCH("prn_bn_bwd/partial");
   }
   int gx = cdiv(HW, 256 * 8);
   if (gx < 1) gx = 1;
   hipLaunchKernelGGL(bn_bwd_apply_kernel, dim3(gx, B * C), dim3(256), 0, st, dy, x, y, stats, gamma, (const double*)ws, dx, dres, C, HW,
-                     S, 1.f / ((float)B * HW), relu, frozen, have, dgamma, dbeta, beta, dbs);
+                     S, 1.f / ((float)B * HW), relu, frozen, have, dgamma, dbeta, beta, dbs, gate);
   PRN_CHECK_LAUNCH("prn_bn_bwd/apply");
   return 0;
+}
 }
 
 extern "C" int prn_bn_train_fwd_partials(const float* parts, int nparts, int64_t part_stride, float* x_out, float* stats, const float* gamma, const float* beta,
```

After: 195.2 (median of 6 runs). No clear change (+0.5%).
